# olasanni1/ETOL

Hardware: AMD Instinct MI355X
Metric: collocation-node constraint+Jacobian evals/sec, 6-state VGP N=1024 (higher is better)
Workload: dtype f64

## Files before the change

### etol_amd/_lib.py

```python
import ctypes as C
import os

import torch

_HERE = os.path.dirname(os.path.abspath(__file__))
LIB_PATH = os.path.join(_HERE, "lib", "libemi355x.so")

EMI_OK = 0
STATUS = {0: "EMI_OK", 1: "EMI_ERR_ARG", 2: "EMI_ERR_STATE", 3: "EMI_ERR_HIP",
          4: "EMI_ERR_NO_DEVICE", 5: "EMI_ERR_UNSUPPORTED", 6: "EMI_ERR_COMM"}

MODEL_POINTMASS2D, MODEL_QUADROTOR2D, MODEL_FIXEDWING12 = 0, 1, 2
MODEL_SOURCE = 100
PATH_ELLIPSE, PATH_DISC, PATH_TRACK = 0, 1, 2
PATH_REC = 8
EVAL_NODES, EVAL_DEFECT, EVAL_ALL, EVAL_NOJAC = 1, 2, 3, 4
EVAL_KEEP_INVARIANT = 8


class EmiError(RuntimeError):
    pass


class Layout(C.Structure):
# ... 41 lines not shown

class IpmRung(C.Structure):
    _fields_ = [("M", C.c_int), ("bd", IpmBounds), ("recs", _D), ("opt", IpmOptions), ("repair", C.c_int)]


class IpmRefine(C.Structure):
    _fields_ = [("ode_tol", C.c_double), ("first_check", C.c_int), ("ul", _D), ("uu", _D)]


class IpmRefineResult(C.Structure):
    _fields_ = [("rung", C.c_int), ("verdict", C.c_int), ("rungs_solved", C.c_int), ("err", C.c_double)]


class Start(C.Structure):
    _fields_ = [("kind", C.c_int), ("nsets", C.c_int), ("xa", _D), ("xb", _D), ("box", _D), ("bend", C.c_double), ("clearance", C.c_double),
                ("grid", C.c_int), ("repair", C.c_int)]


class IpmRestart(C.Structure):
    _fields_ = [("nstarts", C.c_int), ("starts", C.POINTER(Start)), ("patience", _I), ("retry_mask", C.c_int), ("flags", C.c_int)]


class IpmRestartResult(C.Structure):
    _fields_ = [("attempt", C.c_int), ("attempts", C.c_int), ("level", C.c_int), ("refine", IpmRefineResult)]


START_LINE, START_BEND, START_PLANNED = range(3)
RESTART_DROP_FAILED = 1
REFINE_MET, REFINE_NOT_MET, REFINE_FELL_BACK, REFINE_FAILED = range(4)
IPM_RULE_RESIDUAL = 1
IPM_CONVERGED, IPM_ACCEPTABLE, IPM_MAX_ITER, IPM_LINE_SEARCH, IPM_INFEASIBLE, IPM_FACTOR, IPM_NOT_FINITE = range(7)

_PT, _DU, _ST, _EL, _BD = (C.POINTER(t) for t in (IpmPoint, IpmDuals, IpmStep, IpmElim, IpmBounds))

SYMBOLS = {
    "emi_abi_version": (C.c_int, []),
    "emi_status_string": (C.c_char_p, [C.c_int]),
    "emi_device_count": (C.c_int, [_I]),
    "emi_lgl": (C.c_int, [C.c_int, _D, _D, _D]),
    "emi_model_dims": (C.c_int, [C.c_int, _I, _I, _I]),
    "emi_edge_ellipse": (C.c_int, [C.c_double] * 4 + [_D]),
    "emi_track_centres": (C.c_int, [C.c_int, _D, _D, _D, C.c_int, _D, _D, _D]),
    "emi_create": (C.c_int, [C.c_int, C.POINTER(_P)]),
    "emi_create_f32": (C.c_int, [C.c_int, C.POINTER(_P)]),
    "emi_destroy": (C.c_int, [_P]),
    "emi_last_error": (C.c_char_p, [_P]),
    "emi_set_stream": (C.c_int, [_P, _P]),
    "emi_get_stream": (C.c_int, [_P, C.POINTER(_P)]),
    "emi_synchronize": (C.c_int, [_P]),
    "emi_set_mesh": (C.c_int, [_P, C.c_int, _D, _D, _D, C.c_double, C.c_double]),
    "emi_set_model": (C.c_int, [_P, C.c_int, _D, C.c_int, C.c_int]),
    "emi_set_model_source": (C.c_int, [_P, C.c_char_p, C.c_char_p, C.c_int, C.c_int, C.c_int, _I, C.c_int, _D, C.c_int, C.c_int]),
    "emi_check_model_source": (C.c_int, [C.c_char_p, C.c_char_p, C.c_int, C.c_int, C.c_int, C.c_int, C.c_int, C.c_char_p, C.c_size_t]),
    "emi_kkt_factor": (C.c_int, [_P, _D, _D, C.POINTER(C.c_ubyte), C.c_double, C.POINTER(C.c_int)]),
    "emi_kkt_factor_dev": (C.c_int, [_P, _P, _P, _P, C.c_double, C.POINTER(C.c_int)]),
    "emi_kkt_blocks_rows": (C.c_int, [_P, C.c_int, _I, _I, _I]),
    "emi_kkt_blocks_dev": (C.c_int, [_P, _P, _P, _P, _P, _P, C.c_double, _P, _P, C.c_int, _P, _P, _P, _P, _P]),
    "emi_kkt_blocks_host": (C.c_int, [_P, _D, _D, _D, _D, C.POINTER(C.c_ubyte), C.c_double, _D, _D, C.c_int, _I, _I, _D, _D, _D]),
    "emi_kkt_solve": (C.c_int, [_P, _D, C.c_int]),
    "emi_kkt_solve_dev": (C.c_int, [_P, _P, C.c_int]),
    "emi_ipm_reduce_dev": (C.c_int, [_P, _PT, _DU, _P, _P, _P, _BD, _P, _P, _P, _EL, _P]),
    "emi_ipm_expand_dev": (C.c_int, [_P, _PT, _DU, _P, _BD, _P, _EL, _P, _ST, _P]),
    "emi_ipm_trial_dev": (C.c_int, [_P, _PT, _ST, _P, _PT]),
    "emi_ipm_merit_dev": (C.c_int, [_P, _PT, _P, _P, _BD, _P, _P, C.c_int, _P]),
    "emi_ipm_accept_dev": (C.c_int, [_P, _PT, _PT, _DU, _ST, _BD, _P, _P, _P, _P]),
    "emi_ipm_error_dev": (C.c_int, [_P, _PT, _DU, _P, _P, _BD, _P, _P]),
    "emi_ipm_reduce_host": (C.c_int, [_P, _PT, _DU, _P, _P, _P, _BD, _P, _P, _P, _EL, _P]),
    "emi_ipm_expand_host": (C.c_int, [_P, _PT, _DU, _P, _BD, _P, _EL, _P, _ST, _P]),
    "emi_ipm_trial_host": (C.c_int, [_P, _PT, _ST, _P, _PT]),
    "emi_ipm_merit_host": (C.c_int, [_P, _PT, _P, _P, _BD, _P, _P, C.c_int, _P]),
    "emi_ipm_accept_host": (C.c_int, [_P, _PT, _PT, _DU, _ST, _BD, _P, _P, _P, _P]),
    "emi_ipm_error_host": (C.c_int, [_P, _PT, _DU, _P, _P, _BD, _P, _P]),
    "emi_ipm_start_dev": (C.c_int, [_P, C.c_int, _PT, _DU, _P, _BD, _P, C.c_double, C.c_double, _P, _P]),
    "emi_ipm_error_parts_dev": (C.c_int, [_P, _PT, _DU, _P, _P, _BD, _P, _P]),
    "emi_ipm_error_parts_host": (C.c_int, [_P, _PT, _DU, _P, _P, _BD, _P, _P]),
    "emi_ipm_keep_dev": (C.c_int, [_P, _PT, _DU, _PT, _DU, _P, C.c_int]),
    "emi_ipm_keep_host": (C.c_int, [_P, _PT, _DU, _PT, _DU, _P, C.c_int]),
    "emi_ipm_solve_shard_dev": (C.c_int, [_P, _P, _P, _BD, C.POINTER(IpmOptions), _P, _P, C.POINTER(IpmResult)]),
    "emi_ipm_solve_shard_host": (C.c_int, [_P, _P, _P, _BD, C.POINTER(IpmOptions), _P, _P, C.POINTER(IpmResult)]),
    "emi_prolong_matrix": (C.c_int, [C.c_int, _D, _D, C.c_int, _D, _D]),
    "emi_prolong_dev": (C.c_int, [_P, C.c_int, C.c_int, _P, _P, C.c_int, _P]),
    "emi_repair_guess_dev": (C.c_int, [_P, _P]),
    "emi_ipm_solve_ladder_dev": (C.c_int, [_P, C.c_int, C.POINTER(IpmRung), C.c_double, C.c_double, _P, _P, _P, _P, _P, _P, C.POINTER(IpmResult)]),
    "emi_ipm_solve_ladder_host": (C.c_int, [_P, C.c_int, C.POINTER(IpmRung), C.c_double, C.c_double, _P, _P, _P, _P, _P, _P, C.POINTER(IpmResult)]),
    "emi_ode_error_operator": (C.c_int, [C.c_int, _D, _D, _D, _D, _D]),
    "emi_interp_dev": (C.c_int, [_P, C.c_int, C.c_int, C.c_int, _P, _P, C.c_int, C.c_int, _P]),
    "emi_ode_error_dev": (C.c_int, [_P, _P, _P, _D, _D, _P, _P]),
    "emi_ode_error_host": (C.c_int, [_P, _P, _P, _D, _D, _P, _P]),
    "emi_ode_error_delay_operator": (C.c_int, [C.c_int, _D, _D, C.c_double, C.c_double, C.c_double, _D]),
    "emi_ode_error_total_dev": (C.c_int, [_P, _P, _P, _D, _D, _P, _P]),
    "emi_ode_error_total_host": (C.c_int, [_P, _P, _P, _D, _D, _P, _P]),
    "emi_ipm_refine_decide": (C.c_int, [C.c_int, C.c_double, C.c_double, C.c_int, C.c_int, _I]),
    "emi_prolong_rows_dev": (C.c_int, [_P, C.c_int, C.c_int, _P, _P, C.c_int, _P, _P]),
    "emi_shard_move_dev": (C.c_int, [_P, C.c_int, _P, _P, C.c_int, _I, C.POINTER(_P), _I, C.POINTER(_P), _I, C.c_int]),
    "emi_ipm_solve_refine_dev": (C.c_int, [_P, C.c_int, C.POINTER(IpmRung), C.c_double, C.c_double, C.POINTER(IpmRefine), _P, _P, C.c_int,
                                           _P, _P, _P, _P, C.POINTER(IpmResult), _D, C.POINTER(IpmRefineResult)]),
    "emi_ipm_solve_refine_host": (C.c_int, [_P, C.c_int, C.POINTER(IpmRung), C.c_double, C.c_double, C.POINTER(IpmRefine), _P, _P, C.c_int,
                                            _P, _P, _P, _P, C.POINTER(IpmResult), _D, C.POINTER(IpmRefineResult)]),
    "emi_ipm_restart_decide": (C.c_int, [C.c_int, C.c_int]),
    "emi_ipm_solve_restart_dev": (C.c_int, [_P, C.c_int, C.POINTER(IpmRung), C.c_double, C.c_double, C.POINTER(IpmRefine), C.POINTER(IpmRestart),
                                            _P, _P, C.c_int, _P, _P, _P, _P, C.POINTER(IpmResult), _D, C.POINTER(IpmRestartResult)]),
    "emi_ipm_solve_restart_host": (C.c_int, [_P, C.c_int, C.POINTER(IpmRung), C.c_double, C.c_double, C.POINTER(IpmRefine), C.POINTER(IpmRestart),
                                             _P, _P, C.c_int, _P, _P, _P, _P, C.POINTER(IpmResult), _D, C.POINTER(IpmRestartResult)]),
    "emi_plan_route": (C.c_int, [C.c_int, _D, _D, _D, C.c_double, C.c_int, C.c_int, _D, _D, _D, _I, _D, _I, _I]),
    "emi_start_guess_dev": (C.c_int, [_P, C.POINTER(Start), _P, _P]),
    "emi_start_guess_host": (C.c_int, [_P, C.POINTER(Start), _P, _P]),
    "emi_kkt_last_regularisation": (C.c_int, [_P, _D, _D]),
    "emi_kkt_factor_batch": (C.c_int, [C.c_int, C.POINTER(_P), C.POINTER(_D), C.POINTER(_D), C.POINTER(C.POINTER(C.c_ubyte)), _D, _I]),
    "emi_kkt_solve_batch": (C.c_int, [C.c_int, C.POINTER(_P), C.POINTER(_D)]),
    "emi_kkt_is_schur": (C.c_int, [_P]),
    "emi_kkt_solve_refined": (C.c_int, [_P, _D, C.c_double, C.c_int, _D, _I, _I, _I]),
    "emi_kkt_solve_refined_batch": (C.c_int, [C.c_int, C.POINTER(_P), C.POINTER(_D), _D, C.c_int, _D, _I, _I, _I]),
    "emi_kkt_lowrank": (C.c_int, [_P, C.c_int, C.POINTER(C.c_int), _D, _D, C.POINTER(C.c_int)]),
    "emi_kkt_factor_shard_dev": (C.c_int, [_P, _P, _P, _P, _D, C.POINTER(C.c_ubyte), _I]),
    "emi_kkt_lowrank_shard_dev": (C.c_int, [_P, C.c_int, _P, _P, _P, _P, C.POINTER(C.c_ubyte), _I]),
    "emi_kkt_solve_shard_dev": (C.c_int, [_P, _P, C.POINTER(C.c_ubyte)]),
    "emi_kkt_solve_refined_shard_dev": (C.c_int, [_P, _P, C.POINTER(C.c_ubyte), _D, C.c_int, _D, _I, _I, _I]),
    "emi_set_batch": (C.c_int, [_P, C.c_int]),
    "emi_set_path": (C.c_int, [_P, C.c_int, C.c_int, _D, C.c_int, C.c_int]),
    "emi_set_tracks": (C.c_int, [_P, C.c_int, C.c_int, _D, _D]),
    "emi_set_track_waypoints": (C.c_int, [_P, C.c_int, C.c_int, C.c_int, _I, _D, _D, _D]),
    "emi_tracks_from_waypoints_dev": (C.c_int, [_P, C.c_int, _P]),
    "emi_get_tracks": (C.c_int, [_P, _D, _D]),
    "emi_get_layout": (C.c_int, [_P, C.POINTER(Layout)]),
    "emi_jac_structure": (C.c_int, [_P, _I, _I]),
    "emi_invariant_rows": (C.c_int, [C.c_int, C.c_int, C.POINTER(C.c_ubyte), _I]),
    "emi_dev_alloc": (C.c_int, [_P, C.c_size_t, C.POINTER(_P)]),
    "emi_dev_free": (C.c_int, [_P, _P]),
    "emi_h2d": (C.c_int, [_P, _P, _P, C.c_size_t]),
    "emi_d2h": (C.c_int, [_P, _P, _P, C.c_size_t]),
    "emi_eval_dev": (C.c_int, [_P, _P, _P, _P, _P, _P, C.c_uint]),
    "emi_eval_host": (C.c_int, [_P, _D, _D, _D, _D, _D, C.c_uint]),
    "emi_hess_dev": (C.c_int, [_P, _P, _P, _P, _P, C.c_double, _P]),
    "emi_hess_host": (C.c_int, [_P, _D, _D, _D, _D, C.c_double, _D]),
    "emi_lagr_grad_dev": (C.c_int, [_P, _P, _P, _P, C.c_double, _P]),
    "emi_lagr_grad_host": (C.c_int, [_P, _D, _D, _D, C.c_double, _D]),
    "emi_kkt_certificate_dev": (C.c_int, [_P, _P, _P, _P, _P, _P, _P, C.c_double, _P, _P, C.c_int, _D, _D, _P, _P]),
    "emi_kkt_certificate_host": (C.c_int, [_P, _D, _D, _D, _D, C.c_double, _D, _D, C.c_int, _D, _D, _D, _D]),
    "emi_lagr_grad_total_dev": (C.c_int, [_P, _P, _P, _P, C.c_double, _P, _P]),
    "emi_lagr_grad_total_host": (C.c_int, [_P, _D, _D, _D, C.c_double, _D, _D]),
    "emi_kkt_certificate_total_dev": (C.c_int, [_P, _P, _P, _P, _P, _P, _P, C.c_double, _P, _P, C.c_int, _D, _D, _P, _P, _P]),
    "emi_kkt_certificate_total_host": (C.c_int, [_P, _D, _D, _D, _D, C.c_double, _D, _D, C.c_int, _D, _D, _D, _D, _D]),
    "emi_timer_start": (C.c_int, [_P]),
    "emi_timer_stop": (C.c_int, [_P, C.POINTER(C.c_float)]),
    "emi_profile_enable": (C.c_int, [_P, C.c_int]),
    "emi_profile_read": (C.c_int, [_P, C.POINTER(C.c_float), _I, C.POINTER(C.c_float), _I, C.POINTER(C.c_float), _I]),
    "emi_set_option": (C.c_int, [_P, C.c_char_p, C.c_int]),
    "emi_last_path": (C.c_int, [_P, _I]),
    "emi_plan_pass": (C.c_int, [_P, C.c_int, C.POINTER(PassPlan)]),
    "emi_plan_pass_residency": (C.c_int, [_P, C.c_int, _I]),
    "emi_last_defect_kernel": (C.c_char_p, [_P]),
    "emi_debug_pass_roles": (C.c_int, [C.c_int, C.c_int, C.c_int, C.POINTER(C.c_int), C.c_int]),
    "emi_debug_tile_order": (C.c_int, [C.c_int, C.c_int, C.c_int, C.c_int, C.c_int, C.POINTER(C.c_int), C.c_int, C.POINTER(C.c_int), C.POINTER(C.c_int), C.POINTER(C.c_int)]),
    "emi_set_delays": (C.c_int, [_P, C.c_int, C.c_int, C.c_double]),
    "emi_get_delays": (C.c_int, [_P, _I, _I, _I]),
    "emi_delay_matrix": (C.c_int, [C.c_int, C.POINTER(C.c_double), C.POINTER(C.c_double), C.c_double, C.c_double, C.c_double, C.POINTER(C.c_double)]),
    "emi_debug_operator_fragments": (C.c_int, [C.c_int, C.POINTER(C.c_double), C.POINTER(C.c_double)]),
    "emi_debug_tile_order2": (C.c_int, [C.c_int] * 7 + [C.POINTER(C.c_int), C.c_int, C.POINTER(C.c_int), C.POINTER(C.c_int), C.POINTER(C.c_int)]),
    "emi_comm_unique_id": (C.c_int, [_P]),
    "emi_comm_create": (C.c_int, [C.c_int, C.c_int, C.c_int, _P, C.POINTER(_P)]),
    "emi_comm_gather": (C.c_int, [_P, _P, _P, C.c_size_t, C.c_int, _P]),
    "emi_comm_destroy": (C.c_int, [_P]),
    "emi_comm_last_error": (C.c_char_p, [_P]),
}

_lib = None


def load():
    global _lib
    if _lib is not None:
        return _lib
    if not os.path.exists(LIB_PATH):
        raise EmiError(f"{LIB_PATH} is missing: run `python -c 'import __graft_entry__ as g; g.build()'` "
                       "(or `make lib`) first; there is no CPU fallback")
    lib = C.CDLL(LIB_PATH, mode=C.RTLD_GLOBAL)
    for name, (res, args) in SYMBOLS.items():
        fn = getattr(lib, name)
        fn.restype = res
        fn.argtypes = args
    _lib = lib
    return lib


def check(status, ctx=None, what=""):
    if status == EMI_OK:
        return
    lib = load()
    msg = lib.emi_status_string(status).decode()
    if ctx:
        detail = lib.emi_last_error(ctx).decode()
        if detail:
            msg += ": " + detail
    raise EmiError(f"{what or 'libemi355x'}: {STATUS.get(status, status)} ({msg})")
```

### etol_amd/csrc/emi_api_pass.hip

```cpp
#include "emi_ctx.hpp"

using namespace emi_api;

namespace {

emi::PassPolicyIn policy_in(emi_ctx_t c) {
    emi::PassPolicyIn in;
    in.ns = c->ns;
    in.M = c->M;
    in.real_bytes = c->f32 ? 4 : 8;
    in.rows = nres_of(c) + nvals_of(c);
    if (c->model == EMI_MODEL_SOURCE) in.model_class = emi::rtc_has_symdefect(c->rtc) ? emi::PASS_MODEL_RTC : emi::PASS_MODEL_NONE;
    else in.model_class = emi::pass_model_supported(c->model) ? emi::PASS_MODEL_BUILTIN : emi::PASS_MODEL_NONE;
    in.rtc_sw_large = emi::rtc_pass_sw_large(c->rtc);
    in.f32 = c->f32;
    in.symmetric = c->symmetric;
    in.has_dfrag = c->has_dfrag;
    in.allow_fused = c->allow_fused;
    in.overlap_mode = c->overlap_mode;
    in.sym_ct = c->sym_ct;
    in.sym_ksplit = c->sym_ksplit;
    in.sym_cpart = c->sym_cpart;
    in.sym_gblk = c->sym_gblk;
    in.sym_cx = c->sym_cx;
// ... 53 lines not shown

void delay_matrix(const std::vector<double>& tau, const std::vector<double>& w, double t0, double tf, double delay, double* W) {
    const int M = (int)tau.size();
    std::vector<double> lam(M);
    for (int j = 0; j < M; ++j) lam[j] = ((j & 1) ? -1.0 : 1.0) * std::sqrt(w[j]);
    const double hh = (tf - t0) / 2.0;
    for (int k = 0; k < M; ++k) {
        double ts = t0 + hh * (tau[k] + 1.0) - delay;
        if (ts < t0) ts = t0;
        const double x = (ts - t0) / hh - 1.0;
        double* row = W + (size_t)k * M;
        int hit = -1;
        for (int j = 0; j < M; ++j)
            if (x == tau[j]) hit = j;
        if (ts <= t0) hit = 0;
        if (hit >= 0) {
            for (int j = 0; j < M; ++j) row[j] = j == hit ? 1.0 : 0.0;
            continue;
        }
        double den = 0.0;
        for (int j = 0; j < M; ++j) {
            row[j] = lam[j] / (x - tau[j]);
            den += row[j];
        }
        for (int j = 0; j < M; ++j) row[j] /= den;
    }
}

int extend_controls(emi_ctx_t c, const void* dX, const void* dU_free, const void** dU_ext) {
    if (c->f32) return fail(c, EMI_ERR_UNSUPPORTED, "delayed values: f64 contexts only");
    if (c->points_only) return fail(c, EMI_ERR_STATE, "delayed values need a collocation mesh (this context holds a points-only mesh)");
    const int M = c->M, ncf = c->nc - c->nch;
    HIP_TRY(c, hipSetDevice(c->device));
    if (!c->attr_set) {
        HIP_TRY(c, emi::defect_f64_set_attr());
        c->attr_set = true;
    }
    int st;
    if ((st = ensure_delay_matrices(c))) return st;
    const size_t row = (size_t)M * 8;
    if ((st = ensure(c, c->d_uext, (size_t)c->B * c->nc * row))) return st;
    HIP_TRY(c, hipMemsetAsync(c->d_uext.p, 0, (size_t)c->B * c->nc * row, c->stream));
    HIP_TRY(c, hipMemcpy2DAsync(c->d_uext.p, (size_t)c->nc * row, dU_free, (size_t)ncf * row, (size_t)ncf * row, c->B, hipMemcpyDeviceToDevice, c->stream));
    double* base = (double*)c->d_uext.p + (size_t)ncf * M;
    for (int i = 1; i < c->xh; ++i) {
        emi::DefectArgs a{(const double*)dX, (const double*)c->d_W.p + (size_t)(i - 1) * M * M, base + (size_t)(i - 1) * c->ns * M,
                          c->B * c->ns, M, c->ns, c->nc};
        HIP_TRY(c, emi::launch_defect_f64(a, c->stream));
    }
    base += (size_t)std::max(c->xh - 1, 0) * c->ns * M;
    for (int i = 1; i <= c->uh; ++i) {
        emi::DefectArgs a{(const double*)dU_free, (const double*)c->d_W.p + (size_t)(i - 1) * M * M, base + (size_t)(i - 1) * ncf * M,
                          c->B * ncf, M, ncf, c->nc};
        HIP_TRY(c, emi::launch_defect_f64(a, c->stream));
    }
    *dU_ext = c->d_uext.p;
    return EMI_OK;
}

enum class Form {
    PassF64,
    TwoKernelF64,
    PassF32,
    TwoStreamF32,
    Sequential,
};
struct FormChoice {
    Form form = Form::Sequential;
    bool small = false;
    emi::PassPlan plan;
    bool overlapped() const { return form == Form::PassF64 || form == Form::TwoKernelF64; }
};

FormChoice choose_form(emi_ctx_t c, Launch L, unsigned flags) {
    const bool nodes = flags & EMI_EVAL_NODES, defect = flags & EMI_EVAL_DEFECT, jac = !(flags & EMI_EVAL_NOJAC);
    FormChoice ch;
    const emi::PassPolicyIn in = policy_in(c);
    ch.small = defect && !c->f32 && L.B > 0 && L.B * c->ns <= in.small_rows && emi::defect_small_supported(L.B * c->ns) &&
               !(nodes && jac && emi::pass_takes_small_batches(in));
    if (nodes && defect && !ch.small && emi::pass_overlapped(in)) {
        ch.plan = emi::plan_pass(in, L.B, jac);
        ch.form = ch.plan.one_launch ? Form::PassF64 : Form::TwoKernelF64;
    } else if (c->f32 && nodes && defect && jac && !c->rtc && c->allow_fused) {
        if ((c->overlap_mode == 3 || (c->overlap_mode == 0 && c->f32_one_launch)) && emi::pass_f32_supported(c->model, L.B * c->ns, c->M, L.B))
            ch.form = Form::PassF32;
        else if (c->overlap_mode == 2 && emi::defect_f32_mfma_supported(c->M))
            ch.form = Form::TwoStreamF32;
    }
    return ch;
}

int next_prof_record(emi_ctx_t c, ProfEvents** out) {
    if (c->prof_used == c->prof.size()) c->prof.emplace_back();
    ProfEvents& pe = c->prof[c->prof_used];
    for (hipEvent_t& e : pe.ev)
        if (!e) HIP_TRY(c, hipEventCreate(&e));
    ++c->prof_used;
    *out = &pe;
    return EMI_OK;
}

constexpr unsigned AT1 = 1u << 1, AT2 = 1u << 2, AT3 = 1u << 3, AT_ANY = AT1 | AT2 | AT3;
int prof_mark(emi_ctx_t c, ProfEvents* pe, ProfMark which, unsigned levels, hipStream_t s) {
    if (pe && pe->level > 0 && ((levels >> pe->level) & 1u)) HIP_TRY(c, hipEventRecord(pe->ev[which], s));
    return EMI_OK;
}

const char* const NAME_PASS_F32 = "emi_pass_f32_kernel (MFMA + node roles, one launch)";
const char* const NAME_RING1_F64 = "emi_symdefect_ring_f64_kernel";
const char* name_defect_f32(emi_ctx_t c, bool mfma) {
    return !mfma ? "emi_defect_f32_kernel" : (c->f32_ring ? "emi_defect_f32_ring_kernel" : "emi_defect_f32_mfma_kernel");
}
const char* name_defect_f64(bool small) { return small ? "emi_defect_small_f64_kernel" : "emi_defect_f64_kernel"; }
std::string name_pass_f64(const emi::SymPlan& plan) {
    return "emi_pass_f64_kernel<SW=" + std::to_string(plan.sw) + "> (MFMA + node roles, one launch" +
           (plan.ks > 1 ? ", " + std::to_string(plan.ks) + " K slices per tile" : "") + ")" +
           (plan.bk == 16 ? " [K tiles of 16]" : "") + (plan.ct == 2 ? " [128-column tiles]" : "") + (plan.hs == 2 ? " [K range in two halves per workgroup]" : "") +
           (plan.dop ? " [De/Do from L2]" : "");
}
std::string name_symdefect(emi_ctx_t c, const emi::SymPlan& plan, bool in_kernel_combine) {
    if (plan.ring1) return c->sym_ct == 1 || c->sym_ct == 2 ? "emi_symdefect_f64_kernel" : NAME_RING1_F64;
    return "emi_symdefect_ring2_f64_kernel<SW=" + std::to_string(plan.sw) + ">" +
           (plan.ks > 1 ? " x" + std::to_string(plan.ks) + (in_kernel_combine ? " K slices (in-kernel combine)" : " K slices + emi_symdefect_combine_kernel") : "");
}

emi::SymDefectArgs sym_defect_args(emi_ctx_t c, Launch L, const PassIO& io) {
    emi::SymDefectArgs sa;
    sa.X = (const double*)io.X;
    sa.U = (const double*)io.U;
    sa.RES = (double*)io.RES;
    sa.node_t = (const double*)c->d_t.p;
    sa.De = (const double*)c->d_De.p;
    sa.Do = (const double*)c->d_Do.p;
    sa.Dfrag = c->has_dfrag ? (const double*)c->d_Dfrag.p : nullptr;
    sa.M = c->M;
    sa.B = L.B;
    sa.nres = nres_of(c);
    sa.h = (c->tf - c->t0) / 2.0;
    sa.order = c->sym_order;
    sa.ablate = c->sym_ablate;
    sa.ksplit = 1;
    sa.slab = nullptr;
    sa.tile_ticket = nullptr;
    sa.cpart = sa.cx = 0;
    sa.mfma_first = 0;
    for (int i = 0; i < EMI_MAX_PARAMS; ++i) sa.P.p[i] = c->params[i];
    return sa;
}

emi::DefectArgsF32 defect_args_f32(emi_ctx_t c, Launch L, const PassIO& io) {
    return emi::DefectArgsF32{(const float*)io.X, (const float*)c->d_D.p, (float*)io.RES, L.B * c->ns, c->M, c->ns, nres_of(c)};
}

int form_pass_f64(emi_ctx_t c, Launch L, const PassIO& io, const emi::PassPlan& pp, ProfEvents* pe) {
    const emi::SymPlan& plan = pp.sym;
    emi::SymDefectArgs sa = sym_defect_args(c, L, io);
    emi::NodeArgs<double> na;
    fill_node_args(c, L, na, io);
    sa.mfma_first = pp.mfma_first;
    sa.cpart = plan.cpart;
    sa.cx = plan.cx;
    if (plan.ks > 1) {
        EMI_TRY(ensure(c, c->d_slab, plan.slab_bytes));
        EMI_TRY(ensure_zeroed(c, c->d_tile_ticket, (size_t)plan.tiles * 4, c->stream));
        sa.ksplit = plan.ks;
        sa.slab = (double*)c->d_slab.p;
        sa.tile_ticket = (unsigned*)c->d_tile_ticket.p;
    }
    EMI_TRY(ensure_zeroed(c, c->d_ticket, (size_t)L.B * 4, c->stream));
    na.cost_ticket = (unsigned*)c->d_ticket.p;
    EMI_TRY(prof_mark(c, pe, K0, AT_ANY, c->stream));
    if (c->rtc) HIP_TRY(c, emi::rtc_launch_pass(c->rtc, sa, na, plan.sw, c->stream));
    else HIP_TRY(c, emi::launch_pass(c->model, sa, na, c->stream, plan));
    EMI_TRY(prof_mark(c, pe, K1, AT_ANY, c->stream));
    if (pe) pe->level = -1;
    c->last_defect_kernel = name_pass_f64(plan);
    return EMI_OK;
}

int launch_symdefect_f64(emi_ctx_t c, Launch L, emi::SymDefectArgs& sa, hipStream_t s) {
    if (c->rtc) {
        HIP_TRY(c, emi::rtc_launch_symdefect(c->rtc, sa, s));
        c->last_defect_kernel = NAME_RING1_F64;
        return EMI_OK;
    }
    const emi::SymPlan plan = emi::plan_symdefect(c->ns, L.B, c->M, c->sym_ct, c->sym_ksplit, c->sym_cpart, c->sym_gblk, c->sym_cx);
    if (plan.slab_bytes) EMI_TRY(ensure(c, c->d_slab, plan.slab_bytes));
    sa.ksplit = plan.ring1 ? 1 : plan.ks;
    sa.slab = (double*)c->d_slab.p;
    sa.cpart = plan.cpart;
    sa.cx = plan.cx;
    if (sa.ksplit > 1 && c->sym_combine) {
        EMI_TRY(ensure_zeroed(c, c->d_tile_ticket, (size_t)plan.tiles * 4, s));
        sa.tile_ticket = (unsigned*)c->d_tile_ticket.p;
    }
    const unsigned bit = 1u << c->sym_ct;
    HIP_TRY(c, emi::launch_symdefect(c->model, sa, s, !(c->fused_attr_mask & bit), c->sym_ct, plan));
    c->fused_attr_mask |= bit;
    c->last_defect_kernel = name_symdefect(c, plan, sa.tile_ticket != nullptr);
    return EMI_OK;
}

int form_two_kernel_f64(emi_ctx_t c, Launch L, const PassIO& io, bool jac, ProfEvents* pe) {
    emi::SymDefectArgs sa = sym_defect_args(c, L, io);
    emi::NodeArgs<double> na;
    fill_node_args(c, L, na, io);
    const bool two = c->overlap_mode != 1;
    const bool split = two && c->cu_split > 0;
    if (two && !split) EMI_TRY(need_stream2(c));
    hipStream_t s1 = split ? c->s_mfma : c->stream;
    hipStream_t s2 = split ? c->s_node : (two ? c->stream2 : c->stream);
    if (two) {
        HIP_TRY(c, hipEventRecord(c->ev_fork, c->stream));
        HIP_TRY(c, hipStreamWaitEvent(s2, c->ev_fork, 0));
        if (split) HIP_TRY(c, hipStreamWaitEvent(s1, c->ev_fork, 0));
    }
    EMI_TRY(prof_mark(c, pe, K0, AT1 | AT2, s1));
    EMI_TRY(launch_symdefect_f64(c, L, sa, s1));
    EMI_TRY(prof_mark(c, pe, K1, AT1 | AT2, s1));
    if (c->cost_in_kernel) {
        EMI_TRY(ensure_zeroed(c, c->d_ticket, (size_t)L.B * 4, s2));
        na.cost_ticket = (unsigned*)c->d_ticket.p;
    }
    EMI_TRY(prof_mark(c, pe, K2, AT1 | AT3, s2));
    if (c->rtc && jac && na.store_mode == 2 && c->M % 2 == 0) HIP_TRY(c, emi::rtc_launch_nodes_nt(c->rtc, na, s2));
    else if (c->rtc) HIP_TRY(c, emi::rtc_launch_nodes<double>(c->rtc, na, jac, false, s2));
    else HIP_TRY(c, emi::launch_nodes<double>(c->model, na, jac, false, s2));
    EMI_TRY(prof_mark(c, pe, K3, AT1 | AT3, s2));
    if (!c->cost_in_kernel) HIP_TRY(c, emi::launch_cost_finish<double>(na.cost_part, na.cost, L.B, emi::node_chunks(c->M), na.sgn * na.h, s2));
    if (two) {
        HIP_TRY(c, hipEventRecord(c->ev_join, s2));
        HIP_TRY(c, hipStreamWaitEvent(c->stream, c->ev_join, 0));
        if (split) {
            HIP_TRY(c, hipEventRecord(c->ev_join2, s1));
            HIP_TRY(c, hipStreamWaitEvent(c->stream, c->ev_join2, 0));
        }
    }
    EMI_TRY(prof_mark(c, pe, E1, AT1, c->stream));
    EMI_TRY(prof_mark(c, pe, E2, AT1, c->stream));
    return EMI_OK;
}

int form_pass_f32(emi_ctx_t c, Launch L, const PassIO& io, ProfEvents* pe) {
    emi::NodeArgs<float> na;
    fill_node_args(c, L, na, io);
    const size_t rowb = (size_t)c->M * 4;
    HIP_TRY(c, hipMemset2DAsync(io.RES, (size_t)nres_of(c) * rowb, 0, (size_t)c->ns * rowb, L.B, c->stream));
    EMI_TRY(ensure_zeroed(c, c->d_ticket, (size_t)L.B * 4, c->stream));
    na.cost_ticket = (unsigned*)c->d_ticket.p;
    EMI_TRY(prof_mark(c, pe, K0, AT_ANY, c->stream));
    HIP_TRY(c, emi::launch_pass_f32(c->model, defect_args_f32(c, L, io), na, c->pass_order >= 0 ? c->pass_order : 0, c->stream));
    EMI_TRY(prof_mark(c, pe, K1, AT_ANY, c->stream));
    if (pe) { pe->level = -1; pe->fused = true; }
    c->last_defect_kernel = NAME_PASS_F32;
    return EMI_OK;
}

int form_two_stream_f32(emi_ctx_t c, Launch L, const PassIO& io, ProfEvents* pe) {
    emi::NodeArgs<float> pre, full;
    PassIO values_only = io;
    values_only.VALS = nullptr;
    fill_node_args(c, L, pre, values_only);
    fill_node_args(c, L, full, io);
    EMI_TRY(ensure(c, c->d_cost_part2, (size_t)L.B * emi::node_chunks(c->M) * 4));
    EMI_TRY(need_stream2(c));
    pre.cost_part = (float*)c->d_cost_part2.p;
    pre.np = 0;
    const bool fork_late = c->f32_ring_wgs == 1;
    if (!fork_late) {
        HIP_TRY(c, hipEventRecord(c->ev_fork, c->stream));
        HIP_TRY(c, hipStreamWaitEvent(c->stream2, c->ev_fork, 0));
    }
    HIP_TRY(c, emi::launch_nodes<float>(c->model, pre, false, true, c->stream));
    if (fork_late) {
        HIP_TRY(c, hipEventRecord(c->ev_fork, c->stream));
        HIP_TRY(c, hipStreamWaitEvent(c->stream2, c->ev_fork, 0));
    }
    EMI_TRY(prof_mark(c, pe, K0, AT1 | AT2, c->stream));
    HIP_TRY(c, emi::launch_defect_f32_mfma(defect_args_f32(c, L, io), c->stream, c->f32_ring, c->f32_ring_wgs));
    EMI_TRY(prof_mark(c, pe, K1, AT1 | AT2, c->stream));
    c->last_defect_kernel = name_defect_f32(c, true);
    EMI_TRY(prof_mark(c, pe, K2, AT1 | AT3, c->stream2));
    HIP_TRY(c, emi::launch_nodes<float>(c->model, full, true, false, c->stream2));
    EMI_TRY(prof_mark(c, pe, K3, AT1 | AT3, c->stream2));
    HIP_TRY(c, emi::launch_cost_finish<float>(full.cost_part, full.cost, L.B, emi::node_chunks(c->M), full.sgn * full.h, c->stream2));
    HIP_TRY(c, hipEventRecord(c->ev_join, c->stream2));
    HIP_TRY(c, hipStreamWaitEvent(c->stream, c->ev_join, 0));
    if (pe) pe->fused = true;
    EMI_TRY(prof_mark(c, pe, E1, AT1, c->stream));
    EMI_TRY(prof_mark(c, pe, E2, AT1, c->stream));
    return EMI_OK;
}

template <typename T>
int launch_nodes_alone(emi_ctx_t c, Launch L, const PassIO& io, bool jac) {
    emi::NodeArgs<T> a;
    fill_node_args(c, L, a, io);
    if (c->rtc) HIP_TRY(c, emi::rtc_launch_nodes<T>(c->rtc, a, jac, true, c->stream));
    else HIP_TRY(c, emi::launch_nodes<T>(c->model, a, jac, true, c->stream));
    HIP_TRY(c, emi::launch_cost_finish<T>(a.cost_part, a.cost, L.B, emi::node_chunks(c->M), a.sgn * a.h, c->stream));
    return EMI_OK;
}

int form_sequential(emi_ctx_t c, Launch L, const PassIO& io, unsigned flags, bool small, ProfEvents* pe) {
    const bool jac = !(flags & EMI_EVAL_NOJAC);
    if (flags & EMI_EVAL_NODES) EMI_TRY(c->f32 ? launch_nodes_alone<float>(c, L, io, jac) : launch_nodes_alone<double>(c, L, io, jac));
    EMI_TRY(prof_mark(c, pe, E1, AT_ANY, c->stream));
    if ((flags & EMI_EVAL_DEFECT) && c->f32) {
        const bool mfma = emi::defect_f32_mfma_supported(c->M) && c->allow_fused;
        if (mfma) HIP_TRY(c, emi::launch_defect_f32_mfma(defect_args_f32(c, L, io), c->stream, c->f32_ring, c->f32_ring_wgs));
        else HIP_TRY(c, emi::launch_defect_f32(defect_args_f32(c, L, io), c->stream));
        c->last_defect_kernel = name_defect_f32(c, mfma);
    } else if (flags & EMI_EVAL_DEFECT) {
        emi::DefectArgs a{(const double*)io.X, (const double*)c->d_D.p, (double*)io.RES, L.B * c->ns, c->M, c->ns, nres_of(c)};
        if (small) HIP_TRY(c, emi::launch_defect_small_f64(a, c->stream));
        else HIP_TRY(c, emi::launch_defect_f64(a, c->stream));
        c->last_defect_kernel = name_defect_f64(small);
    }
    EMI_TRY(prof_mark(c, pe, E2, AT1 | AT2, c->stream));
    return EMI_OK;
}

int eval_launch(emi_ctx_t c, Launch L, const PassIO& io, unsigned flags) {
    const bool nodes = flags & EMI_EVAL_NODES, defect = flags & EMI_EVAL_DEFECT;
    const bool jac = !(flags & EMI_EVAL_NOJAC);
    if (!nodes && !defect) return fail(c, EMI_ERR_ARG, "emi_eval: empty flags");
// ... 32 lines not shown
    const int M = c->M, nd = std::max(c->xh - 1, c->uh);
    std::vector<double> W((size_t)nd * M * M);
    for (int d = 0; d < nd; ++d) delay_matrix(c->h_tau, c->h_w, c->t0, c->tf, (d + 1) * c->delay_dt, W.data() + (size_t)d * M * M);
    EMI_TRY(upload_real(c, c->d_W, W.data(), W.size()));
    c->delay_dirty = false;
    return EMI_OK;
}

int emi_api::need_stream2(emi_ctx_t c) {
    if (c->stream2) return EMI_OK;
    if (hipStreamCreateWithFlags(&c->stream2, hipStreamNonBlocking) != hipSuccess) {
        c->stream2 = nullptr;
        return fail(c, EMI_ERR_HIP, "cannot create the second stream of the two-stream pass");
    }
    return EMI_OK;
}

extern "C" {

int emi_delay_matrix(int M, const double* tau, const double* w, double t0, double tf, double delay, double* W) {
    if (M < 2 || !tau || !w || !W || !(tf > t0) || delay < 0) return EMI_ERR_ARG;
    delay_matrix(std::vector<double>(tau, tau + M), std::vector<double>(w, w + M), t0, tf, delay, W);
    return EMI_OK;
}

int emi_eval_dev(emi_ctx_t c, const void* dX, const void* dU, void* dRES, void* dVALS, void* dCOST,
                 unsigned flags) {
    int st = ready(c);
    if (st) return st;
    if (c->nch > 0 && dX && dU && (st = extend_controls(c, dX, dU, &dU))) return st;
    int piece = 0;
    const emi::PassPolicyIn in = policy_in(c);
    if (!c->profile && (flags & EMI_EVAL_ALL) == EMI_EVAL_ALL && emi::pass_overlapped(in) && dX && dU && dRES && dCOST &&
        (dVALS || (flags & EMI_EVAL_NOJAC)))
        piece = emi::plan_piece(in, c->B);
    const PassIO io{dX, dU, dRES, dVALS, dCOST};
    const emi::KeepRecord::Pass kp = c->keep.begin_pass((flags & EMI_EVAL_NODES) && !(flags & EMI_EVAL_NOJAC),
                                                        flags & EMI_EVAL_KEEP_INVARIANT, dVALS);
    flags &= ~(unsigned)EMI_EVAL_KEEP_INVARIANT;
    if (piece <= 0) st = eval_launch(c, Launch{0, c->B, kp.keep}, io, flags);
    for (int first = 0; piece > 0 && first < c->B && st == EMI_OK; first += piece)
        st = eval_launch(c, Launch{first, std::min(piece, c->B - first), kp.keep}, io_at(c, io, first), flags);
    c->keep.end_pass(kp, dVALS, st == EMI_OK);
    return st;
}

int emi_eval_host(emi_ctx_t c, const double* X, const double* U, double* RES, double* VALS,
                  double* COST, unsigned flags) {
    int st = ready(c);
    if (st) return st;
    if (!X || !U) return fail(c, EMI_ERR_ARG, "emi_eval_host: null input");
    const size_t rb = c->f32 ? 4 : 8;
    const size_t nX = (size_t)c->B * c->ns * c->M, nU = (size_t)c->B * (c->nc - c->nch) * c->M;
    const size_t nR = (size_t)c->B * nres_of(c) * c->M, nV = (size_t)c->B * nvals_of(c) * c->M;
    if ((st = upload_real(c, c->s_X, X, nX))) return st;
    if ((st = upload_real(c, c->s_U, U, nU))) return st;
    if ((st = ensure(c, c->s_RES, nR * rb))) return st;
    if ((st = ensure_vals_staging(c, nV * rb))) return st;
    if ((st = ensure(c, c->s_COST, (size_t)c->B * rb))) return st;
    if (!(flags & EMI_EVAL_NODES)) {
        if (!RES) return fail(c, EMI_ERR_ARG, "emi_eval_host: defect-only needs RES in/out");
        if ((st = upload_real(c, c->s_RES, RES, nR))) return st;
    }
    if ((st = emi_eval_dev(c, c->s_X.p, c->s_U.p, c->s_RES.p, c->s_VALS.p, c->s_COST.p, flags | EMI_EVAL_KEEP_INVARIANT))) return st;
    if ((st = download_real(c, RES, c->s_RES.p, nR))) return st;
    if (!(flags & EMI_EVAL_NOJAC) && (flags & EMI_EVAL_NODES))
        if ((st = download_real(c, VALS, c->s_VALS.p, nV))) return st;
    if (flags & EMI_EVAL_NODES)
        if ((st = download_real(c, COST, c->s_COST.p, c->B))) return st;
    HIP_TRY(c, hipStreamSynchronize(c->stream));
    return EMI_OK;
}

int emi_hess_dev(emi_ctx_t c, const void* dX, const void* dU, const void* dLamF, const void* dLamC,
                 double sigma, void* dH) {
    int st = ready(c);
    if (st) return st;
    if (!dX || !dU || !dLamF || !dH || (np_total(c) > 0 && !dLamC))
        return fail(c, EMI_ERR_ARG, "emi_hess: null device pointer");
    HIP_TRY(c, hipSetDevice(c->device));
    if (c->nch > 0 && (st = extend_controls(c, dX, dU, &dU))) return st;
    auto fill = [&](auto& a) {
        using T = typename std::remove_reference<decltype(a.h)>::type;
        a.X = (const T*)dX; a.U = (const T*)dU; a.lamF = (const T*)dLamF; a.lamC = (const T*)dLamC;
        a.H = (T*)dH; a.w = (const T*)c->d_w.p; a.node_t = (const T*)c->d_t.p;
        a.path = (const T*)c->d_path.p;
        a.M = c->M; a.B = c->B; a.np = np_total(c); a.path_sets = c->path_sets; a.px = c->px; a.py = c->py;
        a.h = (T)((c->tf - c->t0) / 2.0); a.sgn = c->maximize ? T(-1) : T(1); a.sigma = (T)sigma;
        for (int i = 0; i < EMI_MAX_PARAMS; ++i) a.P.p[i] = (T)c->params[i];
    };
    if (c->f32) {
        emi::HessArgs<float> a;
        fill(a);
        if (c->rtc) HIP_TRY(c, emi::rtc_launch_hess<float>(c->rtc, a, c->stream));
        else HIP_TRY(c, emi::launch_hess<float>(c->model, a, c->stream));
    } else {
        emi::HessArgs<double> a;
        fill(a);
        if (c->rtc) HIP_TRY(c, emi::rtc_launch_hess<double>(c->rtc, a, c->stream));
        else HIP_TRY(c, emi::launch_hess<double>(c->model, a, c->stream));
    }
    return EMI_OK;
}

int emi_hess_host(emi_ctx_t c, const double* X, const double* U, const double* LamF,
                  const double* LamC, double sigma, double* H) {
    int st = ready(c);
    if (st) return st;
    if (!X || !U || !LamF || !H || (np_total(c) > 0 && !LamC)) return fail(c, EMI_ERR_ARG, "emi_hess_host: null pointer");
    const size_t rb = c->f32 ? 4 : 8;
    const size_t nX = (size_t)c->B * c->ns * c->M, nU = (size_t)c->B * (c->nc - c->nch) * c->M;
    const size_t nC = (size_t)c->B * np_total(c) * c->M, nH = (size_t)c->B * nhess_of(c) * c->M;
    if ((st = upload_real(c, c->s_X, X, nX))) return st;
    if ((st = upload_real(c, c->s_U, U, nU))) return st;
    if ((st = upload_real(c, c->s_LF, LamF, nX))) return st;
    if (nC && (st = upload_real(c, c->s_LC, LamC, nC))) return st;
    if ((st = ensure(c, c->s_H, nH * rb))) return st;
    if ((st = emi_hess_dev(c, c->s_X.p, c->s_U.p, c->s_LF.p, c->s_LC.p, sigma, c->s_H.p))) return st;
    return download_real(c, H, c->s_H.p, nH);
}

int emi_plan_pass(emi_ctx_t c, int B, emi_pass_plan_t* out) {
    if (!c || !out || B < 1) return EMI_ERR_ARG;
    if (c->M <= 0 || c->model < 0) return fail(c, EMI_ERR_STATE, "emi_plan_pass: mesh and model must be set");
    memset(out, 0, sizeof *out);
    emi::report_pass(policy_in(c), B, out);
    return EMI_OK;
}

int emi_plan_pass_residency(emi_ctx_t c, int B, int* res) {
    if (!c || !res || B < 1) return EMI_ERR_ARG;
    if (c->M <= 0 || c->model < 0) return fail(c, EMI_ERR_STATE, "emi_plan_pass_residency: mesh and model must be set");
    emi_pass_plan_t plan;
    memset(&plan, 0, sizeof plan);
    emi::report_pass(policy_in(c), B, &plan, nullptr, res);
    return EMI_OK;
}

int emi_last_path(emi_ctx_t c, int* fused) {
    if (!c || !fused) return EMI_ERR_ARG;
    *fused = choose_form(c, Launch{0, c->B}, EMI_EVAL_ALL).overlapped() ? 1 : 0;
    return EMI_OK;
}

int emi_debug_pass_roles(int nm, int nn, int order, int* out_role, int out_cap) {
    if (nm < 0 || nn < 0 || nm + nn < 1 || !out_role || out_cap < nm + nn) return EMI_ERR_ARG;
    for (int j = 0; j < nm + nn; ++j) {
        const emi::PassRole r = emi::pass_role_of(j, nm, nn, order);
        out_role[j] = r.mfma ? r.index : -1 - r.index;
    }
    return EMI_OK;
}

int emi_debug_tile_order(int ns, int B, int M, int sym_ct, int sym_cpart, int* out_tile, int out_cap, int* ntiles_total, int* cpart,
                         int* cx) {
    return emi_debug_tile_order2(ns, B, M, sym_ct, sym_cpart, 0, 0, out_tile, out_cap, ntiles_total, cpart, cx);
}

int emi_debug_tile_order2(int ns, int B, int M, int sym_ct, int sym_cpart, int sym_gblk, int sym_cx, int* out_tile, int out_cap,
                          int* ntiles_total, int* cpart, int* cx) {
    if (ns < 1 || B < 1 || M < 128 || M % 128 != 0 || !ntiles_total) return EMI_ERR_ARG;
    const emi::SymPlan p = emi::plan_symdefect(ns, B, M, sym_ct, 1, sym_cpart, sym_gblk, sym_cx);
    if (p.ring1 || p.sw < 1) return EMI_ERR_UNSUPPORTED;
    const int ntiles = (M / 2) / 64, ngrp = ((B + 15) / 16) * (ns / p.sw), total = ntiles * ngrp;
    *ntiles_total = total;
    if (cpart) *cpart = p.cpart;
    if (cx) *cx = p.cx;
    for (int t = 0; t < total && t < out_cap && out_tile; ++t) {
        const emi::RingTile rt = emi::ring_tile_of(t, ntiles, ngrp, p.cpart, p.cx, ns / p.sw);
        out_tile[t] = rt.ntile + ntiles * rt.grp;
    }
    return EMI_OK;
}

int emi_debug_operator_fragments(int M, const double* D, double* out) {
    if (M < 128 || M % 128 != 0 || !D || !out) return EMI_ERR_ARG;
    std::vector<double> De, Do;
    if (!even_odd_halves(M, D, De, Do)) return EMI_ERR_UNSUPPORTED;
    emi::operator_fragments(M, De.data(), Do.data(), out);
    return EMI_OK;
}

const char* emi_last_defect_kernel(emi_ctx_t c) {
    if (!c) return "";
    return c->last_defect_kernel.c_str();
}

}
```

### etol_amd/csrc/emi_args.hpp

```cpp
#pragma once
#ifdef __HIPCC_RTC__
#define EMI_PATH_ELLIPSE 0
#define EMI_PATH_DISC 1
#define EMI_PATH_TRACK 2
#define EMI_PATH_REC 8
#else
#include <hip/hip_runtime.h>
#include <stddef.h>
#include "emi355x.h"
#endif

#define EMI_NODE_THREADS 256

#ifdef EMI_TICKET_ACQ_REL
#define EMI_TICKET_ORDER __ATOMIC_ACQ_REL
#else
#define EMI_TICKET_ORDER __ATOMIC_RELAXED
#endif
#ifdef EMI_NO_M0_NOP
#define EMI_M0_NOP ""
#else
#define EMI_M0_NOP "s_nop 0\n\t"
#endif

#define DEF_TM 96
#define DEF_TN 128
#define DEF_BK 16

#define FUSED_TI 16
#define FUSED_BK 16

#include "emi_models.hpp"

namespace emi {

template <typename T> struct NodeArgs {
    const T* X;
    const T* U;
    T* RES;
    T* VALS;
    T* cost_part;
    T* cost;
    unsigned* cost_ticket;
    const T* w;
    const T* node_t;
    const T* Ddiag;
    const T* path;
    const T* track_x;
    const T* track_y;
    int M, B, np, nres, nvals;
    int path_sets, track_sets, ntracks;
    int px, py;
    int store_mode;
    int keep;
    T h, sgn;
    ModelParams<T> P;
};

template <typename T> struct HessArgs {
    const T* X;
    const T* U;
    const T* lamF;
    const T* lamC;
    T* H;
    const T* w;
    const T* node_t;
    const T* path;
    int M, B, np, path_sets, px, py;
    T h, sgn, sigma;
    ModelParams<T> P;
};

template <typename T> struct OdeResidArgs {
    const T* Zs;
    const T* Zc;
    const T* tq;
    const T* scale;
    const T* ul;
    const T* uu;
    T* eta;
    int M, B, lds, ldc;
    T h;
    ModelParams<T> P;
};

template <typename T> struct OdeResidDelayArgs {
    const T* Zs;
    const T* Zc;
    const T* tq;
    const T* scale;
    const T* ul;
    const T* uu;
    T* eta;
    int M, B, lds, ldc;
    int ncf, ns, xh, uh;
    T h;
    ModelParams<T> P;
};

struct SymDefectArgs {
    const double* X;
    const double* U;
    double* RES;
    const double* node_t;
    const double* De;
    const double* Do;
    int M, B, nres;
    int order;
    int ablate;
    int ksplit;
    double* slab;
    unsigned* tile_ticket;
    int mfma_first;
    int cpart, cx;
    double h;
    ModelParams<double> P;
    const double* Dfrag;
};

struct DefectArgs {
    const double* X;
    const double* D;
    double* RES;
    int R, M, ns, nres;
};
struct DefectArgsF32 {
    const float* X;
    const float* D;
    float* RES;
    int R, M, ns, nres;
};
struct RingTile { int ntile, grp; };
#if defined(__HIPCC__)
__host__ __device__
#endif
inline RingTile ring_tile_of(int tl, int ntiles, int ngrp, int cpart, int cx, int nsg = 1) {
    RingTile t;
    if (cpart > 0) {
        const int per_xcd = ngrp * ntiles / 8;
        const int x = tl / per_xcd, m = tl - x * per_xcd;
        const int pc = x % cpart, pg = x / cpart;
        const int ncol = ntiles / cpart, ng = ngrp / (8 / cpart);
        const int cb = m / (ng * cx), r = m - cb * ng * cx;
        t.grp = pg * ng + r / cx;
        t.ntile = pc * ncol + cb * cx + r % cx;
    } else if (cpart < 0) {
        const int G = -cpart, per_xcd = ngrp * ntiles / 8;
        const int x = tl / per_xcd, m = tl - x * per_xcd;
        const int per_sb = G * nsg * ntiles, sb = m / per_sb, r = m - sb * per_sb;
        const int per_cb = G * nsg * cx, cb = r / per_cb, r2 = r - cb * per_cb;
        const int g = r2 / (nsg * cx), r3 = r2 - g * (nsg * cx);
        const int mt = x * (ngrp / nsg / 8) + sb * G + g;
        t.grp = mt * nsg + r3 / cx;
        t.ntile = cb * cx + r3 % cx;
    } else {
        t.ntile = tl % ntiles;
        t.grp = tl / ntiles;
    }
    return t;
}
struct PassRole { int mfma, index; };
#if defined(__HIPCC__)
__host__ __device__
#endif
inline PassRole pass_role_of(int j, int nm, int nn, int order) {
    const long long t = (long long)nm + nn;
    long long m0, m1;
    const long long d = order >= 100 ? order : 100;
    if (order == 1 || d * nm > 100 * t) {
        m0 = j < nm ? j : nm;
        m1 = j < nm ? j + 1 : nm;
    } else {
        m0 = ((long long)j * nm * d) / (100 * t);
        m1 = ((long long)(j + 1) * nm * d) / (100 * t);
        if (m0 > nm) m0 = nm;
        if (m1 > nm) m1 = nm;
    }
    PassRole r;
    r.mfma = m1 > m0;
    r.index = (int)(r.mfma ? m0 : j - m0);
    return r;
}
struct PassArgs {
    SymDefectArgs s;
    NodeArgs<double> n;
    int nm8, nn8;
    int nm, nn;
    int nbx;
};

}
```

### etol_amd/csrc/emi_ctx.hpp

```cpp
#pragma once
#include <hip/hip_runtime.h>

#include <algorithm>
#include <cstdarg>
#include <cstdio>
#include <cstring>
#include <string>
#include <vector>

#include "emi355x.h"
#include "emi_device_array.hpp"
#include "emi_keep_record.hpp"
#include "emi_kernels.hpp"

namespace emi_api {

using DevBuf = emi::DeviceArray<unsigned char>;

enum ProfMark { E0, E1, E2, K0, K1, K2, K3, PROF_MARKS };
struct ProfEvents {
    hipEvent_t ev[PROF_MARKS] = {};
    bool has_node = false, has_defect = false, fused = false;
    int level = 0;
};

}
using emi_api::DevBuf, emi_api::ProfEvents;

struct emi_ctx_s {
    int device = 0;
    bool f32 = false;
    hipStream_t stream = nullptr;
    bool own_stream = false;
    hipStream_t stream2 = nullptr;
    hipEvent_t ev_fork = nullptr, ev_join = nullptr, ev_join2 = nullptr;
    int cu_split = 0;
    hipStream_t s_mfma = nullptr, s_node = nullptr;
    std::string err;
    std::string last_defect_kernel;

    int M = 0;
    double t0 = 0, tf = 0;
    DevBuf d_w, d_t, d_Ddiag, d_D, d_De, d_Do;
    bool symmetric = false;
    DevBuf d_Dfrag;
    bool has_dfrag = false;
    bool points_only = false;
    int allow_fused = 1;
    int sym_ct = 0;
    int sym_order = 1;
    int sym_ablate = 0;
    int small_rows = 24;
    int overlap_mode = 0;
    int node_store = -1;
    unsigned fused_attr_mask = 0;
    std::vector<double> h_tau, h_w;
    int model = -1, ns = 0, nc = 0, maximize = 0;
    double params[EMI_MAX_PARAMS] = {0};
    emi::KktWorkspace* kkt = nullptr;
    std::vector<emi::KktWorkspace*> kkt_shard;
    int kkt_method = 1;
    emi::RtcModel* rtc = nullptr;
    int B = 0;
    int np = 0, path_sets = 0, px = 0, py = 1;
    int np_model = 0;
    std::vector<int> pvars;
    DevBuf d_path;
    int ntracks = 0, track_sets = 0;
    DevBuf d_trkx, d_trky;
    int wp_ntracks = 0, wp_sets = 0, wp_ld = 0;
    emi::DeviceArray<double> d_wp;
    emi::DeviceArray<int> d_wp_cnt;
    emi::DeviceArray<double> d_wp_nt;
    bool wp_nt_dirty = true;
    DevBuf d_cost_part;
    DevBuf d_slab;
    DevBuf d_tile_ticket;
    DevBuf d_cost_part2;
    DevBuf d_ticket;
    int cost_in_kernel = 1;
    int sym_nst = 3;
    int sym_hs = 0;
    int sym_ctc = 0;
    int sym_bk = 0;
    int sym_dop = 0;
    int sym_res = 0;
    int xh = 0, uh = 0, nch = 0;
    double delay_dt = 0.0;
    bool delay_dirty = true;
    DevBuf d_W;
    bool adjw_dirty = true;
    DevBuf d_adjWT;
    DevBuf d_adj_Gx;
    int adj_fold_tile = 0;
    DevBuf d_uext;
    int f32_ring_wgs = 2;
    int f32_ring = 1;
    int f32_one_launch = 0;
    int slice = 0;
    int sym_ksplit = 0;
    int sym_cpart = 0;
    int sym_gblk = 0, sym_cx = 0;
    int pass_order = -1;
    int sym_combine = 1;
    emi::KeepRecord keep;
    DevBuf s_X, s_U, s_RES, s_VALS, s_COST, s_LF, s_LC, s_H;
    std::vector<DevBuf> host_stage;
    DevBuf d_adjDT;
    bool adj_dirty = true;
    DevBuf d_adj_pvars;
    std::vector<int> adj_pvars;
    DevBuf d_adj_c;
    DevBuf d_adj_G;
    DevBuf d_adj_op;
    DevBuf s_G, s_cert, s_zl, s_zu, s_Gdel;
    bool ode_dirty = true;
    emi::DeviceArray<double> d_ode_op;
    emi::DeviceArray<double> d_ode_tq;
    emi::DeviceArray<double> d_ode_ub;
    emi::DeviceArray<double> d_ode_ws;
    bool odel_dirty = true;
    emi::DeviceArray<double> d_odel_ops;
    emi::DeviceArray<double> d_odel_opc;
    bool blk_rows_set = false;
    std::vector<int> blk_row_ptr, blk_var, blk_entry;
    std::vector<int> blk_key;
    emi::DeviceArray<int> blk_term_ptr, blk_term_row, blk_term_ea, blk_term_eb, blk_flag, blk_list, blk_nflag, blk_cnt;
    emi::DeviceArray<double> blk_tdelta, blk_tvec, blk_tworst;
    int blk_generic = 0;
    std::vector<int> ipm_key;
    emi::DeviceArray<int> ipm_lists;
    int ipm_npairs = 0;
    std::vector<double> ipm_crow_h;
    emi::DeviceArray<double> ipm_crow, ipm_part;
    emi::IpmSolveWs* ipm_solve = nullptr;
    emi::IpmLadderWs* ipm_ladder = nullptr;
    emi::StartGuessWs* start_guess = nullptr;
    bool path_has_track = false;
    hipEvent_t t_start = nullptr, t_stop = nullptr;
    int profile = 0;
    std::vector<ProfEvents> prof;
    size_t prof_used = 0;
    bool attr_set = false;

    ~emi_ctx_s() {
        (void)hipSetDevice(device);
        if (stream) (void)hipStreamSynchronize(stream);
        for (ProfEvents& pe : prof)
            for (hipEvent_t e : pe.ev)
                if (e) (void)hipEventDestroy(e);
        for (hipStream_t s : {stream2, s_mfma, s_node})
            if (s) { (void)hipStreamSynchronize(s); (void)hipStreamDestroy(s); }
        for (hipEvent_t e : {ev_join2, ev_fork, ev_join, t_start, t_stop})
            if (e) (void)hipEventDestroy(e);
        if (own_stream && stream) (void)hipStreamDestroy(stream);
        emi::rtc_destroy(rtc);
        emi::kkt_destroy(kkt);
        for (emi::KktWorkspace* w : kkt_shard) emi::kkt_destroy(w);
        emi::ipm_solve_destroy(ipm_solve);
        emi::ipm_ladder_destroy(ipm_ladder);
        emi::start_guess_destroy(start_guess);
    }
};

#define HIP_TRY(c, call)                                                                                                                  \
    do {                                                                                                                                  \
        hipError_t e_ = (call);                                                                                                           \
        if (e_ != hipSuccess) return emi_api::fail((c), EMI_ERR_HIP, "%s failed: %s (%s:%d)", #call, hipGetErrorString(e_), __FILE__, __LINE__); \
    } while (0)
#define HIP_TRY_AS(c, who, call)                                                                                        \
    do {                                                                                                                \
        const hipError_t e_ = (call);                                                                                   \
        if (e_ != hipSuccess) return emi_api::fail((c), EMI_ERR_HIP, "%s: %s failed: %s", who, #call, hipGetErrorString(e_)); \
    } while (0)

#define EMI_TRY(call)              \
    do {                           \
        const int st_ = (call);    \
        if (st_) return st_;       \
    } while (0)

namespace emi_api {

int fail(emi_ctx_t c, int code, const char* fmt, ...);
inline int ensure(emi_ctx_t c, DevBuf& b, size_t bytes) {
    HIP_TRY(c, b.reserve(bytes));
    return EMI_OK;
}
inline int ensure_zeroed(emi_ctx_t c, DevBuf& b, size_t bytes, hipStream_t s) {
    if (b.bytes() >= bytes) return EMI_OK;
    EMI_TRY(ensure(c, b, bytes));
    HIP_TRY(c, hipMemsetAsync(b.p, 0, bytes, s));
    return EMI_OK;
}
int upload_bytes(emi_ctx_t c, DevBuf& b, const void* src, size_t bytes);
int upload_real(emi_ctx_t c, DevBuf& b, const double* src, size_t n);
int download_real(emi_ctx_t c, double* dst, const void* dsrc, size_t n);
bool even_odd_halves(int M, const double* D, std::vector<double>& De, std::vector<double>& Do);
int ensure_vals_staging(emi_ctx_t c, size_t bytes);

inline int np_total(emi_ctx_t c) { return c->np + c->np_model; }
inline int nvals_of(emi_ctx_t c) { return c->ns * (c->ns + c->nc) + 2 * c->np + c->np_model * (int)c->pvars.size() + (c->ns + c->nc); }
inline int nres_of(emi_ctx_t c) { return c->ns + np_total(c); }
inline int nhess_of(emi_ctx_t c) { const int nv = c->ns + c->nc; return nv * (nv + 1) / 2; }
inline int ready(emi_ctx_t c) {
    if (!c) return EMI_ERR_ARG;
    if (c->M <= 0) return fail(c, EMI_ERR_STATE, "emi_set_mesh has not been called");
    if (c->model < 0) return fail(c, EMI_ERR_STATE, "emi_set_model has not been called");
    if (c->B <= 0) return fail(c, EMI_ERR_STATE, "emi_set_batch has not been called");
    if (c->np > 0 && c->path_sets != 1 && c->path_sets != c->B)
        return fail(c, EMI_ERR_STATE, "path table has %d sets, batch is %d", c->path_sets, c->B);
    if (c->ntracks > 0 && c->track_sets != 1 && c->track_sets != c->B)
        return fail(c, EMI_ERR_STATE, "track table has %d sets, batch is %d", c->track_sets, c->B);
    return EMI_OK;
}

struct HostStager {
    emi_ctx_t c;
    size_t slot = 0;
    int status = EMI_OK;
    struct Out { void* host; void* dev; size_t bytes; };
    std::vector<Out> outs;
    explicit HostStager(emi_ctx_t c_) : c(c_) {}
    void* place(const void* host, size_t bytes, bool in, bool out);
    int finish();
};
#define HOST_STAGED_TRY(s, call)                                                          \
    if ((s).status) { (void)hipStreamSynchronize((s).c->stream); return (s).status; }     \
    if (const int st_ = (call)) { (void)hipStreamSynchronize((s).c->stream); return st_; }

int ensure_delay_matrices(emi_ctx_t c);
int need_stream2(emi_ctx_t c);
int path_row_list(emi_ctx_t c, const char* what, std::vector<int>& ptr, std::vector<int>& var, std::vector<int>& ent);
int shard_check(emi_ctx_t c, const char* what);
int ctx_ipm_launch(emi_ctx_t c, int what, const emi_ipm_bounds_t* bd, const void* dPar, emi::IpmArgs& a);

}
```

### etol_amd/csrc/emi_kernels.hpp

```cpp
#pragma once
#include <hip/hip_runtime.h>
#include <stddef.h>

#include <string>

#include "emi355x.h"
#include "emi_args.hpp"
#include "emi_pass_plan.hpp"

static_assert(EMI_PATH_ELLIPSE == 0 && EMI_PATH_DISC == 1 && EMI_PATH_TRACK == 2 && EMI_PATH_REC == 8,
              "emi_args.hpp and emi355x.h disagree");

namespace emi {

static_assert(PASS_TI == FUSED_TI, "emi_pass_plan.hpp and emi_args.hpp disagree");

int node_chunks(int M);
bool invariant_rows(int model, int np, unsigned char* mask);
template <typename T>
hipError_t launch_nodes(int model, const NodeArgs<T>& a, bool jac, bool defect_rows, hipStream_t s);
template <typename T> hipError_t launch_hess(int model, const HessArgs<T>& a, hipStream_t s);
hipError_t launch_defect_f64(const DefectArgs& a, hipStream_t s);
bool defect_small_supported(int R);
hipError_t launch_defect_small_f64(const DefectArgs& a, hipStream_t s);
hipError_t launch_defect_f32(const DefectArgsF32& a, hipStream_t s);
bool defect_f32_mfma_supported(int M);
hipError_t launch_defect_f32_mfma(const DefectArgsF32& a, hipStream_t s, int ring = 0, int wgs_per_cu = 2);
bool pass_f32_supported(int model, int R, int M, int B);
hipError_t launch_pass_f32(int model, const DefectArgsF32& d, const NodeArgs<float>& n, int order, hipStream_t s);
hipError_t defect_f64_set_attr();
template <typename T>
hipError_t launch_cost_finish(const T* part, T* cost, int B, int nchunks, T scale, hipStream_t s);
bool fused_supported(int model, int M, int ct);
hipError_t launch_symdefect(int model, const SymDefectArgs& a, hipStream_t s, bool set_attr, int ct, const SymPlan& plan);
inline void operator_fragments(int M, const double* De, const double* Do, double* out) {
    const int Hh = M / 2, nkt = Hh / 16;
    for (int ct = 0; ct < Hh / 64; ++ct)
        for (int w = 0; w < 4; ++w)
            for (int kt = 0; kt < nkt; ++kt)
                for (int q = 0; q < 4; ++q)
                    for (int lane = 0; lane < 64; ++lane) {
                        const double* row = ((q & 1) ? Do : De) + (size_t)(64 * ct + 16 * w + (lane & 15)) * Hh + 16 * kt + 8 * (q >> 1) + 2 * (lane >> 4);
                        double* o = out + ((((size_t)(ct * 4 + w) * nkt + kt) * 4 + q) * 64 + lane) * 2;
                        o[0] = row[0];
                        o[1] = row[1];
                    }
}

bool pass_model_supported(int model);
hipError_t launch_pass(int model, const SymDefectArgs& sa, const NodeArgs<double>& na, hipStream_t s, const SymPlan& plan);

struct AdjointArgs {
    const double* VALS;
    const double* lamF;
    const double* lamC;
    const double* DT;
    const int* pvars;
    double* G;
    int B, M, ldt, ns, nc, np_table, np_traced, pw, px, py, nvals;
    int add_op;
    double sigma;
};
struct CertArgs {
    const double *X, *U, *RES, *VALS, *lamF, *lamC, *G;
    const double *zl, *zu;
    const double *cl, *cu;
    double* cert;
    int B, M, ns, nc, np, nres, nvals, nsets;
    int ncg;
    double sigma;
};
struct AdjointOpArgs {
    const double* A;
    const double* Bop;
    const double* add;
    double* out;
    int R, rpi, M, ldt, nseg, ldb;
    int a_inst, a_row0, a_seg, out_inst, out_row0, add_inst, add_row0;
};
hipError_t launch_adjoint_transpose(const double* dSrc, double* dDst, int M, int ldt, int ld_dst, int nseg, bool keep_diag, hipStream_t s);
bool adjoint_side_by_side(int B, int ns, int M);
hipError_t launch_adjoint_op(const AdjointArgs& a, hipStream_t s);
hipError_t launch_adjoint_product(const AdjointOpArgs& a, int tile, hipStream_t s);
hipError_t launch_adjoint_nodes(const AdjointArgs& a, hipStream_t s);
hipError_t launch_adjoint_add(const double* dGop, double* dG, int B, int ns, int nv, int M, hipStream_t s);
hipError_t launch_kkt_certificate(const CertArgs& a, hipStream_t s);

struct InterpOpArgs {
    const double* V;
    const double* OP;
    double* out;
    int R, K, N, ldk, ldo;
};
hipError_t launch_interp_op(const InterpOpArgs& a, hipStream_t s);
hipError_t launch_ode_copy_D(const double* D, double* dst, int M, int ldk, hipStream_t s);
hipError_t launch_ode_resid(int model, const OdeResidArgs<double>& a, hipStream_t s);
struct RtcModel;
hipError_t rtc_launch_ode_resid(RtcModel* m, const OdeResidArgs<double>& a, hipStream_t s);
hipError_t launch_ode_resid_delay(int model, const OdeResidDelayArgs<double>& a, hipStream_t s);
hipError_t rtc_launch_ode_resid_delay(RtcModel* m, const OdeResidDelayArgs<double>& a, hipStream_t s);
struct OdeFinishArgs {
    const double* X;
    const double* Zs;
    const double* eta;
    double* err;
    int B, M, ns, lds, dcol;
    double h;
};
hipError_t launch_ode_finish(const OdeFinishArgs& a, hipStream_t s);

struct BlocksArgs {
    const double *H, *VALS, *Sigma, *SigT;
    const unsigned char* fixed;
    double dw_shift;
    double *Qexact, *Q;
    int max_mods;
    int* count;
    int* node;
    double *delta, *vec, *worst;
    int B, M, nv, np, nvals;
    int generic;
    const int *term_ptr, *term_row, *term_ea, *term_eb;
    int *flag, *list, *nflag, *cnt;
    double *tdelta, *tvec, *tworst;
};
hipError_t launch_kkt_blocks(const BlocksArgs& a, hipStream_t s);

struct IpmArgs {
    int B, M, ns, nc, np, nvals, nsets, reset;
    double *X, *U, *S, *E1, *E2;
    double *tX, *tU, *tS, *tE1, *tE2;
    double *LF, *Y, *ZL, *ZU, *VL, *VU, *W1, *W2;
    double *DZ, *DS, *DY, *DE1, *DE2, *DZL, *DZU, *DVL, *DVU, *DW1, *DW2;
    double *Sigma, *SigT, *SigS, *RhatS, *Rt, *Rhs;
    const double *RES, *VALS, *G, *COST, *DefRes, *RowRes, *rs;
    const double *zl, *zu;
    const double* crow;
    const double *par, *apr, *adu;
    const unsigned char* mask;
    const int *vptr, *vrow, *vent;
    const int *rptr, *rvar, *rent;
    double *part, *out;
    unsigned char* fixedb;
    double* LamC;
    double push, frac;
};
enum { IPM_REDUCE, IPM_EXPAND, IPM_TRIAL, IPM_MERIT, IPM_ACCEPT, IPM_ERROR, IPM_ERROR_PARTS, IPM_START_PUSH, IPM_START_ROWS, IPM_RESET_W, IPM_LAMC };
constexpr int IPM_MAX_PARTIALS = 9;
int ipm_chunks(int M);
hipError_t launch_ipm(int what, const IpmArgs& a, hipStream_t s);

struct RtcModel;
int rtc_check(bool f32, const char* struct_name, const char* source, int ns, int nc, int npath, int pw, std::string* log);
int rtc_build(bool f32, const char* struct_name, const char* source, int ns, int nc, int npath, int pw, RtcModel** out, std::string* log);
void rtc_destroy(RtcModel* m);
bool rtc_has_symdefect(const RtcModel* m);
template <typename T>
hipError_t rtc_launch_nodes(RtcModel* m, const NodeArgs<T>& a, bool jac, bool defect_rows, hipStream_t s);
template <typename T> hipError_t rtc_launch_hess(RtcModel* m, const HessArgs<T>& a, hipStream_t s);
hipError_t rtc_launch_symdefect(RtcModel* m, const SymDefectArgs& a, hipStream_t s);
int rtc_pass_sw_large(const RtcModel* m);
hipError_t rtc_launch_pass(RtcModel* m, const SymDefectArgs& sa, const NodeArgs<double>& na, int sw, hipStream_t s);
hipError_t rtc_launch_nodes_nt(RtcModel* m, const NodeArgs<double>& a, hipStream_t s);

struct KktWorkspace;
int kkt_factor(KktWorkspace** w, hipStream_t stream, const double* dD, int M, int ns, int nv, const double* Qblk,
               const double* Jblk, const unsigned char* fixed, double dc, int method, int* info, std::string* err,
               bool blocks_on_device = false);
int kkt_solve(KktWorkspace* w, hipStream_t stream, int nz, double* rhs, int nrhs, std::string* err,
              bool rhs_on_device = false);
bool kkt_set_option(const char* name, int value);
int kkt_lowrank(KktWorkspace* w, hipStream_t stream, int nz, int r, const int* node, const double* vec, const double* delta,
                int* exact, std::string* err);
void kkt_destroy(KktWorkspace* w);
void kkt_last_regularisation(const KktWorkspace* w, double* dc, double* dw);
void kkt_mesh_changed(KktWorkspace* w);
bool kkt_is_schur(const KktWorkspace* w);
struct KktShardSrc {
    const double* Q;
    const double* VALS;
    const unsigned char* fixed;
    size_t vals_stride;
    const int* inst;
};
int kkt_factor_batch(int n, KktWorkspace** const* pws, hipStream_t stream, const double* const* dD, int M, int ns, int nv,
                     const double* const* Qblk, const double* const* Jblk, const unsigned char* const* fixed, const double* dc, int* info,
                     std::string* err, const KktShardSrc* src = nullptr);
int kkt_solve_batch(int n, KktWorkspace* const* ws, hipStream_t stream, int nz, double* const* rhs, std::string* err,
                    bool rhs_on_device = false);
int kkt_solve_refined_batch(int n, KktWorkspace* const* ws, hipStream_t stream, double* const* rhs, const double* dc_nominal, int max_steps,
                            double* rel, int* nsolve, int* reverted, int* status, std::string* err, bool rhs_on_device = false);
int kkt_holds(const KktWorkspace* w, int M, int ns, int nv);
int kkt_lowrank_shard(int n, KktWorkspace* const* ws, hipStream_t stream, int max_mods, const int* inst, const int* count, const int* dNode,
                      const double* dDelta, const double* dVec, int* exact, std::string* err);
void kkt_forget_ladder(KktWorkspace* w);

struct IpmSolveWs;
void ipm_solve_destroy(IpmSolveWs* w);
int ipm_solve_shard(emi_ctx_t c, void* dX, void* dU, const emi_ipm_bounds_t* bd, const emi_ipm_options_t& opt, void* dLamF, void* dLamC,
                    emi_ipm_result_t* results);

struct IpmKeepArgs {
    double* live[13];
    double* kept[13];
    const unsigned char* mask;
    int B, M, ns, nc, np, restore;
};
hipError_t launch_ipm_keep(const IpmKeepArgs& a, hipStream_t s);

hipError_t launch_prolong_rows(const double* PT, const double* Vc, const int* map, int group, double* Vf, int Mc, int Mf, int R, hipStream_t s);
struct RepairArgs {
    double* X;
    const double *recs, *trkx, *trky;
    int B, ns, M, np, path_sets, px, py, ntracks, track_sets;
};
hipError_t launch_repair_guess(const RepairArgs& a, hipStream_t s);
struct TrackWaypointArgs {
    const double *t, *x, *y, *node_t;
    const int *cnt, *map;
    void *xc, *yc;
    int n, ntracks, ld, M, first;
};
template <typename T> hipError_t launch_track_waypoints(TrackWaypointArgs a, hipStream_t s);
struct IpmLadderWs;
void ipm_ladder_destroy(IpmLadderWs* w);
struct StartArgs {
    double* X;
    int* level;
    const double *recs, *par, *tau, *sine;
    double *cost, *dist, *extra;
    int* cells;
    unsigned char* bits;
    int B, ns, M, np, path_sets, px, py, nsets, kind, N, has_box;
    double bend, clearance;
};
struct StartGuessWs;
void start_guess_destroy(StartGuessWs* w);
int start_guess(emi_ctx_t c, const emi_start_t& st, void* dX, void* dLevel);
int ipm_solve_ladder(emi_ctx_t c, int nrungs, const emi_ipm_rung_t* rungs, double t0, double tf, const void* dX0, const void* dU0, void* dX,
                     void* dU, void* dLamF, void* dLamC, emi_ipm_result_t* results);
constexpr int SHARD_MOVE_ARRAYS = 4;
struct ShardMoveArgs {
    const double* src[SHARD_MOVE_ARRAYS];
    double* dst[SHARD_MOVE_ARRAYS];
    int rows[SHARD_MOVE_ARRAYS], sld[SHARD_MOVE_ARRAYS], dld[SHARD_MOVE_ARRAYS];
    const int *sidx, *didx;
    int n, narrays, len, first;
};
hipError_t launch_shard_move(ShardMoveArgs a, hipStream_t s);
int ipm_solve_refine(emi_ctx_t c, int nrungs, const emi_ipm_rung_t* rungs, double t0, double tf, const emi_ipm_refine_t& rf, const void* dX0,
                     const void* dU0, int ldm, void* dX, void* dU, void* dLamF, void* dLamC, emi_ipm_result_t* results, double* err,
                     emi_ipm_refine_result_t* out);
int ipm_solve_restart(emi_ctx_t c, int nrungs, const emi_ipm_rung_t* rungs, double t0, double tf, const emi_ipm_refine_t* rf,
                      const emi_ipm_restart_t& rs, const void* dX0, const void* dU0, int ldm, void* dX, void* dU, void* dLamF, void* dLamC,
                      emi_ipm_result_t* results, double* err, emi_ipm_restart_result_t* out);

}
```

### etol_amd/csrc/emi_pass_plan.hpp

```cpp
#pragma once
#include <stddef.h>

#include <algorithm>
#include <climits>

#include "emi355x.h"

namespace emi {

constexpr int PASS_TI = 16;

struct SymPlan {
    bool ring1 = false;
    int sw = 0;
    int ks = 1;
    int nst = 3;
    int bk = 8;
    int hs = 1;
    int ct = 1;
    bool dop = false;
    int res = 2;
    size_t slab_bytes = 0;
    int cpart = 0, cx = 0;
    int tiles = 0;
};

inline bool symdefect_shape_ok(int M, int ct) {
    if (ct == 0 || (ct >= 4 && ct <= 8)) return M >= 128 && M % 128 == 0;
    const int w = ct == 2 ? 2 : 1;
    return ct >= 1 && ct <= 3 && M >= 128 * w && M % (128 * w) == 0;
}

inline int legal_ks(int nkt, int ks) {
    while (ks > 1 && (nkt % ks != 0 || nkt / ks < 2 || (nkt / ks) % 2 != 0)) ks >>= 1;
    return ks < 1 ? 1 : ks;
}

inline int symdefect_sw(int ns, int tiles, int ct) {
    if (ct == 0 || ct == 4) {
        if (tiles >= 448) return (ns % 2 == 0 && ns > 2) ? 2 : ns;
        if (tiles >= 320) return ns;
        if (tiles >= 192) return 0;
        return (tiles <= 96 || ns % 2 != 0 || ns <= 2) ? 1 : 2;
    }
    if (ct < 5 || ct > 8) return 0;
    const int sw = ct == 5 ? ns : (ct == 6 ? 2 : (ct == 8 ? 3 : 1));
    return ns % sw != 0 ? 1 : sw;
}
inline int symdefect_ct_of(int ns, int sw) { return sw == ns ? 5 : (sw == 2 ? 6 : (sw == 3 ? 8 : 7)); }

inline SymPlan plan_symdefect(int ns, int B, int M, int ct, int ksplit_opt, int cpart_opt = 0, int gblk_opt = 0, int cx_opt = 0, int bk_opt = 8,
                              int ct_cols = 1) {
    SymPlan p;
    p.bk = bk_opt == 16 ? 16 : 8;
    const int mtiles = (B + PASS_TI - 1) / PASS_TI;
    const int tiles = mtiles * ((M / 2) / 64);
    p.sw = symdefect_sw(ns, tiles, ct);
    if (p.sw == 0) {
        p.ring1 = true;
        return p;
    }
    if (ksplit_opt > 0) p.ks = legal_ks((M / 2) / p.bk, ksplit_opt);
    p.ct = (ct_cols == 2 && p.sw == 2 && p.ks == 1 && M % 256 == 0) ? 2 : 1;
    p.tiles = (tiles / p.ct) * (ns / p.sw);
    {
        const int ntiles = (M / 2) / (64 * p.ct), ngrp = mtiles * (ns / p.sw);
        const int target_cols = std::max(1, 4096 / M / p.ct);
        auto valid = [&](int cp) { return cp >= 1 && cp <= 8 && ntiles % cp == 0 && ngrp % (8 / cp) == 0 && (ngrp * ntiles) % 8 == 0; };
        int cp = 0;
        if (cpart_opt > 0) cp = valid(cpart_opt) ? cpart_opt : 0;
        else if (cpart_opt == 0 && tiles >= 192)
            for (int c = 1; c <= 8 && !cp; c *= 2)
                if (valid(c) && (ntiles / c <= target_cols || c == 8 || !valid(2 * c))) cp = c;
        if (gblk_opt > 0 && mtiles % (8 * gblk_opt) == 0 && (ngrp * ntiles) % 8 == 0) {
            int cxg = cx_opt > 0 ? cx_opt : 2;
            while (cxg > 1 && ntiles % cxg != 0) --cxg;
            p.cpart = -gblk_opt;
            p.cx = cxg;
        } else if (cp > 0) {
            p.cpart = cp;
            p.cx = 1;
            for (int d = 1; d <= std::min(ntiles / cp, target_cols); ++d)
                if ((ntiles / cp) % d == 0) p.cx = d;
            if (cp == 1 && p.cx == ntiles) p.cpart = p.cx = 0;
        }
    }
    if (p.ks > 1) p.slab_bytes = (size_t)p.tiles * p.ks * (2 * p.sw * 4) * 256 * sizeof(double);
    return p;
}

enum PassSwClass { SWC_NS = 0, SWC_1 = 1, SWC_2 = 2, SWC_3 = 3, SWC_LARGE = 4  };
constexpr bool pass_class_applies(int cls, int ns) {
    return cls == SWC_2 ? (ns > 2 && ns % 2 == 0) : (cls == SWC_3 ? (ns > 3 && ns % 3 == 0) : true);
}
constexpr int pass_class_sw(int cls, int ns) { return cls == SWC_NS ? ns : (cls == SWC_LARGE ? ((ns % 2 == 0 && ns > 2) ? 2 : 1) : cls); }

#define EMI_PASS_FORMS(X)                   \
    X(SWC_NS, 3, 8, 1, 1, false, true, -1)  \
    X(SWC_2, 3, 8, 1, 2, false, false, -1)  \
    X(SWC_2, 3, 16, 1, 2, false, false, -1) \
    X(SWC_2, 3, 8, 2, 1, false, false, -1)  \
    X(SWC_2, 3, 16, 2, 1, false, false, -1) \
    X(SWC_2, 3, 16, 1, 1, true, false, -1)  \
    X(SWC_2, 3, 16, 1, 1, false, false, -1) \
    X(SWC_2, 4, 8, 1, 1, false, true, -1)   \
    X(SWC_2, 3, 8, 1, 1, false, true, -1)   \
    X(SWC_3, 3, 8, 1, 1, false, true, -1)   \
    X(SWC_1, 3, 8, 1, 2, false, false, -1)  \
    X(SWC_1, 3, 16, 1, 2, false, false, -1) \
    X(SWC_1, 3, 16, 1, 1, true, false, -1)  \
    X(SWC_1, 3, 16, 1, 1, false, false, -1) \
    X(SWC_1, 4, 8, 1, 1, false, true, -1)   \
    X(SWC_1, 3, 8, 1, 1, false, true, -1)
#define EMI_PASS_FORMS_RTC(X)             \
    X(SWC_1, 3, 8, 1, 1, false, true, 0)  \
    X(SWC_LARGE, 3, 8, 1, 1, false, true, 2)

struct PassForm {
    int cls, nst, bk, ct, hs;
    bool dop, slices;
    int stores;
};
#define EMI_PASS_FORM_ROW(CLS, NST, BK, CT, HS, DOP, SLICES, STORES) {CLS, NST, BK, CT, HS, DOP, SLICES, STORES},
inline constexpr PassForm PASS_FORMS[] = {EMI_PASS_FORMS(EMI_PASS_FORM_ROW)};
inline constexpr PassForm PASS_FORMS_RTC[] = {EMI_PASS_FORMS_RTC(EMI_PASS_FORM_ROW)};
#undef EMI_PASS_FORM_ROW
constexpr int N_PASS_FORMS = sizeof PASS_FORMS / sizeof PASS_FORMS[0], N_PASS_FORMS_RTC = sizeof PASS_FORMS_RTC / sizeof PASS_FORMS_RTC[0];

enum PassModelClass { PASS_MODEL_NONE = 0, PASS_MODEL_BUILTIN = 1, PASS_MODEL_RTC = 2 };
struct PassShape {
    int ns = 0, M = 0;
    int model_class = PASS_MODEL_NONE;
    bool has_dfrag = false;
    int store_mode = 0;
};
struct PassWants {
    int sw = 0, ks = 1, nst = 3, bk = 8, ct = 1, hs = 1;
    bool dop = false;
    int res = 2;
};
constexpr int pass_form_max_res(const PassForm& f) { return f.dop ? 3 : 2; }
struct PassResolved {
    const PassForm* row = nullptr;
    int sw = 0, ks = 1;
    int res = 2;
    explicit operator bool() const { return row != nullptr; }
};

inline bool form_fits(const PassForm& f, const PassShape& s) {
    if (f.ct == 2 && s.M % 256 != 0) return false;
    if (f.hs == 2 && ((s.M / 2) / f.bk) % 4 != 0) return false;
    if (f.dop && !s.has_dfrag) return false;
    if (f.stores >= 0 && (f.stores == 2) != (s.store_mode == 2)) return false;
    return true;
}

inline const PassForm* find_form(const PassShape& s, int sw, bool sliced, int nst, int bk, int ct, int hs, bool dop) {
    const bool rtc = s.model_class == PASS_MODEL_RTC;
    const PassForm* rows = rtc ? PASS_FORMS_RTC : PASS_FORMS;
    const int n = s.model_class == PASS_MODEL_NONE ? 0 : (rtc ? N_PASS_FORMS_RTC : N_PASS_FORMS);
    if (sw < 1 || s.M < 128 || s.M % 128 != 0 || s.ns % sw != 0) return nullptr;
    for (int i = 0; i < n; ++i) {
        const PassForm& f = rows[i];
        if (pass_class_applies(f.cls, s.ns) && pass_class_sw(f.cls, s.ns) == sw && f.nst == nst && f.bk == bk && f.ct == ct && f.hs == hs && f.dop == dop &&
            (f.slices || !sliced) && form_fits(f, s))
            return &f;
    }
    return nullptr;
}

inline PassResolved resolve_form(const PassWants& w, const PassShape& s) {
    PassResolved r;
    const bool sliced = w.ks > 1;
    int nst = 3, bk = 8, ct = 1, hs = 1;
    bool dop = false;
    if (!find_form(s, w.sw, sliced, nst, bk, ct, hs, dop)) return r;
    if (w.nst == 4 && find_form(s, w.sw, sliced, 4, bk, ct, hs, dop)) nst = 4;
    if (w.bk == 16 && find_form(s, w.sw, sliced, nst, 16, ct, hs, dop)) bk = 16;
    if (w.ct == 2 && find_form(s, w.sw, sliced, nst, bk, 2, hs, dop)) ct = 2;
    if (w.hs == 2 && find_form(s, w.sw, sliced, nst, bk, ct, 2, dop)) hs = 2;
    if (w.dop && find_form(s, w.sw, sliced, nst, bk, ct, hs, true)) dop = true;
    r.row = find_form(s, w.sw, sliced, nst, bk, ct, hs, dop);
    r.sw = w.sw;
    r.ks = w.ks;
    r.res = (w.res == 3 && r.row && pass_form_max_res(*r.row) >= 3) ? 3 : 2;
    return r;
}

struct PassPolicyIn {
    int ns = 0, M = 0;
    int real_bytes = 8;
    int rows = 0;
    int model_class = PASS_MODEL_NONE;
    int rtc_sw_large = 0;
    bool f32 = false, symmetric = false, has_dfrag = false;
    int allow_fused = 1, overlap_mode = 0, sym_ct = 0, sym_ksplit = 0, sym_cpart = 0, sym_gblk = 0, sym_cx = 0, sym_nst = 3, sym_hs = 0, sym_ctc = 0,
        sym_bk = 0, sym_dop = 0, sym_res = 0, pass_order = -1, node_store = -1, slice = 0, small_rows = 24;
};

inline bool pass_overlapped(const PassPolicyIn& in) {
    if (in.f32 || !in.allow_fused || !in.symmetric || in.M <= 0 || in.model_class == PASS_MODEL_NONE) return false;
    if (in.model_class == PASS_MODEL_RTC) return in.M % 128 == 0;
    return symdefect_shape_ok(in.M, in.sym_ct);
}

inline int pass_tiles16(const PassPolicyIn& in, int B) { return ((B + 15) / 16) * (in.M / 128); }

inline int store_mode_for(const PassPolicyIn& in, int B) {
    if (in.node_store >= 0) return in.node_store;
    if ((size_t)B * in.rows * in.M * in.real_bytes > ((size_t)230 << 20)) return 2;
    const int tiles16 = pass_tiles16(in, B);
    if (tiles16 > 16 && tiles16 <= 32) return 0;
    return (in.model_class != PASS_MODEL_RTC && !in.f32) ? 1 : 0;
}

enum PassBandNeeds : unsigned {
    BAND_EVEN_NS = 1u,
    BAND_FREE_KS = 2u,
    BAND_FREE_DEPTH = 4u,
    BAND_FREE_ORDER = 8u,
    BAND_DEFAULT = 16u,
    BAND_FREE_RES = 32u,
};
enum PassKsRule {
    KS_UNSPLIT,
    KS_BY_WORKGROUPS,
};
struct PassBand {
    int lo, hi;
    unsigned needs;
    int sw_ct;
    PassKsRule ks;
    int bk;
    int dop;
    int order;
    int res = 2;
};
constexpr unsigned BAND_DEEP = BAND_DEFAULT | BAND_FREE_DEPTH;
inline constexpr PassBand PASS_BANDS[] = {
    {33, 48, BAND_DEEP | BAND_FREE_KS | BAND_EVEN_NS, 7, KS_UNSPLIT, 16, 1, 1},
    {80, 80, BAND_DEEP | BAND_FREE_KS | BAND_EVEN_NS | BAND_FREE_RES, 6, KS_UNSPLIT, 16, 2, 1, 3},
    {49, 127, BAND_DEEP | BAND_FREE_KS | BAND_EVEN_NS, 6, KS_UNSPLIT, 16, 1, 1},
    {144, 207, BAND_DEEP | BAND_FREE_ORDER | BAND_EVEN_NS, 6, KS_BY_WORKGROUPS, 16, 1, 150},
    {208, 215, BAND_DEEP | BAND_FREE_ORDER, 6, KS_BY_WORKGROUPS, 16, 1, 125},
    {512, 1024, BAND_DEEP | BAND_FREE_ORDER | BAND_EVEN_NS | BAND_FREE_RES, 6, KS_BY_WORKGROUPS, 16, 2, 110, 3},
    {216, 383, BAND_DEEP | BAND_FREE_ORDER, 6, KS_BY_WORKGROUPS, 16, 2, 125},
    {384, 767, BAND_DEEP | BAND_FREE_ORDER, 6, KS_BY_WORKGROUPS, 16, 2, 110},
    {768, 1024, BAND_DEEP | BAND_FREE_ORDER, 6, KS_BY_WORKGROUPS, 16, 2, 0},
    {0, 127, 0, 7, KS_BY_WORKGROUPS, 8, 1, 1},
    {128, 207, 0, 6, KS_BY_WORKGROUPS, 8, 1, 1},
    {208, 383, 0, 6, KS_BY_WORKGROUPS, 8, 1, 125},
    {384, 767, 0, 6, KS_BY_WORKGROUPS, 8, 1, 110},
    {768, INT_MAX, 0, 6, KS_BY_WORKGROUPS, 8, 1, 0},
};

struct PassLargeBatch { int above, whole; int gblk, ct, cx; };
inline constexpr PassLargeBatch PASS_LARGE_BATCH = {2048, 256, 2, 2, 1};

inline const PassBand& band_for(const PassPolicyIn& in, int tiles16, bool auto_ct) {
    unsigned met = 0;
    if (in.ns % 2 == 0 && in.ns > 2) met |= BAND_EVEN_NS;
    if (in.sym_ksplit == 0) met |= BAND_FREE_KS;
    if (in.sym_bk == 0 && in.sym_nst == 3) met |= BAND_FREE_DEPTH;
    if (in.pass_order < 0) met |= BAND_FREE_ORDER;
    if (in.sym_res == 0 && in.sym_dop != 1 && in.sym_hs <= 1 && in.sym_ctc <= 1 && in.sym_ksplit <= 1) met |= BAND_FREE_RES;
    if (auto_ct && in.model_class == PASS_MODEL_BUILTIN) met |= BAND_DEFAULT;
    const PassBand* b = PASS_BANDS;
    while (!(tiles16 >= b->lo && tiles16 <= b->hi && (b->needs & ~met) == 0)) ++b;
    return *b;
}

struct PassPlan {
    bool one_launch = false;
    SymPlan sym;
    int tiles16 = 0;
    int store_mode = 0;
    int mfma_first = 0;
};

inline SymPlan plan_tiles(const PassPolicyIn& in, int B, const PassWants& w, const PassResolved& r, int gblk, int band_cx) {
    const PassForm& f = *r.row;
    const bool wide_order = f.ct == 2 || (in.model_class == PASS_MODEL_BUILTIN && w.ct == 2 && r.sw == 2 && r.ks == 1 && w.nst == 3 && in.M % 256 == 0);
    const int cx = in.sym_cx ? in.sym_cx : (wide_order ? band_cx : 0);
    SymPlan p = plan_symdefect(in.ns, B, in.M, symdefect_ct_of(in.ns, r.sw), r.ks, in.sym_cpart, gblk, cx, 8, wide_order ? 2 : 1);
    p.tiles = p.tiles * p.ct / f.ct;
    p.nst = f.nst;
    p.bk = f.bk;
    p.ct = f.ct;
    p.hs = f.hs;
    p.dop = f.dop;
    p.res = r.res;
    return p;
}

inline PassPlan plan_pass(const PassPolicyIn& in, int B, bool jac) {
    PassPlan p;
    p.tiles16 = pass_tiles16(in, B);
    p.store_mode = store_mode_for(in, B);
    const bool auto_mode = in.overlap_mode == 0, rtc = in.model_class == PASS_MODEL_RTC;
    if (!((in.overlap_mode == 3 || auto_mode) && jac) || in.M % 128 != 0) return p;
    const bool auto_ct = auto_mode && (in.sym_ct == 0 || in.sym_ct == 4);
    const PassBand& band = band_for(in, p.tiles16, auto_ct);
    const bool large = B > PASS_LARGE_BATCH.above && B % PASS_LARGE_BATCH.whole == 0 && in.sym_cpart == 0;
    const bool wide_large = auto_ct && large && in.sym_ctc == 0;
    const int ct_code = rtc ? ((p.store_mode == 2 && in.rtc_sw_large == 2) ? 6 : 7) : (auto_ct ? band.sw_ct : in.sym_ct);
    PassWants w;
    w.sw = symdefect_sw(in.ns, p.tiles16, ct_code);
    if (w.sw == 0) w.sw = in.ns;
    w.ks = in.sym_ksplit;
    if (w.ks == 0 && auto_ct && band.ks == KS_BY_WORKGROUPS) {
        const int wgs = p.tiles16 * (in.ns / w.sw);
        w.ks = wgs * 4 <= 256 ? 4 : (wgs * 2 <= 512 ? 2 : 1);
    }
    w.ks = legal_ks((in.M / 2) / 8, w.ks);
    w.nst = in.sym_nst;
    w.bk = in.sym_bk ? in.sym_bk : band.bk;
    w.ct = in.sym_ctc ? in.sym_ctc : (wide_large ? PASS_LARGE_BATCH.ct : 1);
    w.hs = in.sym_hs ? in.sym_hs : 1;
    w.dop = (in.sym_dop ? in.sym_dop : band.dop) == 2;
    w.res = (in.sym_res ? in.sym_res : band.res) == 3 ? 3 : 2;
    const int gblk = (large && in.sym_gblk == 0 && (rtc || (auto_ct && w.ks == 1))) ? PASS_LARGE_BATCH.gblk : in.sym_gblk;
    PassShape s;
    s.ns = in.ns;
    s.M = in.M;
    s.model_class = in.model_class;
    s.has_dfrag = in.has_dfrag;
    s.store_mode = p.store_mode;
    const PassResolved r = resolve_form(w, s);
    if (!r) return p;
    p.sym = plan_tiles(in, B, w, r, gblk, wide_large ? PASS_LARGE_BATCH.cx : 0);
    p.mfma_first = in.pass_order >= 0 ? in.pass_order : band.order;
    p.one_launch = true;
    return p;
}

inline bool pass_takes_small_batches(const PassPolicyIn& in) {
    if (!pass_overlapped(in) || (in.overlap_mode != 0 && in.overlap_mode != 3) || in.M % 128 != 0) return false;
    PassShape s;
    s.ns = in.ns;
    s.M = in.M;
    s.model_class = in.model_class;
    PassWants w;
    w.sw = 1;
    return (bool)resolve_form(w, s);
}

inline int plan_piece(const PassPolicyIn& in, int B) {
    const long long cap = ((0xFFFFFFFFLL / ((long long)in.ns * in.M * 8)) / 256) * 256;
    int piece = 0;
    if (in.slice > 0) { if (B > 2 * in.slice) piece = in.slice; }
    else if (B > 2048) piece = (int)std::min<long long>(cap > 0 ? cap : 256, B - B % 256);
    return piece >= B ? 0 : piece;
}

inline void report_pass(const PassPolicyIn& in, int B, emi_pass_plan_t* out, bool* dop = nullptr, int* res = nullptr) {
    if (dop) *dop = false;
    if (res) *res = 0;
    if (!pass_overlapped(in)) return;
    const int piece = plan_piece(in, B);
    out->piece = piece;
    out->tail = piece > 0 ? B % piece : 0;
    const PassPlan p = plan_pass(in, piece > 0 ? piece : B, true);
    out->one_launch = p.one_launch ? 1 : 0;
    out->sw = p.sym.sw;
    out->ksplit = p.sym.ks;
    out->ring_stages = p.sym.nst;
    out->k_tile = p.sym.bk;
    out->column_tiles = p.sym.ct;
    out->k_halves = p.sym.hs;
    out->cpart = p.sym.cpart;
    out->cx = p.sym.cx;
    out->mfma_workgroups = p.sym.tiles * p.sym.ks;
    out->store_mode = p.store_mode;
    out->block_order = p.mfma_first;
    out->tiles16 = p.tiles16;
    if (dop) *dop = p.sym.dop;
    if (res) *res = p.one_launch ? p.sym.res : 0;
}

}
```

### etol_amd/csrc/emi_rtc.hip

```cpp
#include <hip/hip_runtime.h>
#include <hip/hiprtc.h>

#include <cstdio>
#include <cstring>
#include <map>
#include <mutex>
#include <string>
#include <vector>

#include "emi_kernels.hpp"
#include "emi_rtc_sources.inc"

namespace emi {

struct RtcModel {
    hipModule_t mod = nullptr;
    hipFunction_t nodes[2][2][2] = {};
    hipFunction_t hess = nullptr;
    hipFunction_t ode_resid = nullptr;
    hipFunction_t ode_resid_delay = nullptr;
    hipFunction_t ring = nullptr;
    hipFunction_t pass[N_PASS_FORMS_RTC] = {};
    hipFunction_t node_nt = nullptr;
    bool f32 = false;
// ... 91 lines not shown
    hiprtcGetProgramLogSize(p, &ls);
    std::string l(ls, '\0');
    if (ls) hiprtcGetProgramLog(p, &l[0]);
    while (!l.empty() && l.back() == '\0') l.pop_back();
    if (r != HIPRTC_SUCCESS) {
        if (log) *log = std::string("model program does not compile (") + hiprtcGetErrorString(r) + "):\n" + l;
        hiprtcDestroyProgram(&p);
        return EMI_ERR_ARG;
    }
    if (log) *log = l;
    lowered->clear();
    for (const std::string* s : order) {
        const char* low = nullptr;
        if (hiprtcGetLoweredName(p, s->c_str(), &low) != HIPRTC_SUCCESS || !low) {
            if (log) *log = "no lowered name for " + *s;
            hiprtcDestroyProgram(&p);
            return EMI_ERR_HIP;
        }
        lowered->push_back(low);
    }
    size_t cs = 0;
    hiprtcGetCodeSize(p, &cs);
    code->resize(cs);
    hiprtcGetCode(p, code->data());
    hiprtcDestroyProgram(&p);
    *has_ring = with_ring;
    return EMI_OK;
}

hipError_t launch(hipFunction_t f, dim3 grid, dim3 block, size_t lds, hipStream_t s, const void* args, size_t bytes) {
    if (!f) return hipErrorInvalidDeviceFunction;
    void* config[] = {HIP_LAUNCH_PARAM_BUFFER_POINTER, const_cast<void*>(args), HIP_LAUNCH_PARAM_BUFFER_SIZE, &bytes,
                      HIP_LAUNCH_PARAM_END};
    return hipModuleLaunchKernel(f, grid.x, grid.y, grid.z, block.x, block.y, block.z, (unsigned)lds, s, nullptr,
                                 config);
}

}

int rtc_check(bool f32, const char* struct_name, const char* source, int ns, int nc, int npath, int pw, std::string* log) {
    std::vector<char> code;
    std::vector<std::string> low;
    bool ring = false;
    return compile(f32, struct_name, source, ns, nc, npath, pw, &code, &low, &ring, log);
}

namespace {
struct CachedProgram {
    std::vector<char> code;
    std::vector<std::string> lowered;
    bool ring = false;
};
std::mutex g_cache_mutex;
std::map<std::string, CachedProgram> g_cache;
}

int rtc_build(bool f32, const char* struct_name, const char* source, int ns, int nc, int npath, int pw, RtcModel** out,
              std::string* log) {
    *out = nullptr;
    std::vector<char> code;
    std::vector<std::string> low;
    bool ring = false;
    const std::string key = std::string(f32 ? "f32|" : "f64|") + (struct_name ? struct_name : "") + "|" + std::to_string(ns) + "|" +
                            std::to_string(nc) + "|" + std::to_string(npath) + "|" + (source ? source : "");
    bool hit = false;
    {
        std::lock_guard<std::mutex> lk(g_cache_mutex);
        auto it = g_cache.find(key);
        if (it != g_cache.end()) {
            code = it->second.code;
            low = it->second.lowered;
            ring = it->second.ring;
            hit = true;
        }
    }
    if (!hit) {
        const int st = compile(f32, struct_name, source, ns, nc, npath, pw, &code, &low, &ring, log);
        if (st) return st;
        std::lock_guard<std::mutex> lk(g_cache_mutex);
        CachedProgram& cp = g_cache[key];
        cp.code = code;
        cp.lowered = low;
        cp.ring = ring;
    }
    RtcModel* m = new RtcModel();
    m->f32 = f32;
    m->ns = ns;
    m->nc = nc;
    hipError_t e = hipModuleLoadData(&m->mod, code.data());
    size_t i = 0;
    for (int v = 0; v < 2 && e == hipSuccess; ++v)
        for (int j = 0; j < 2 && e == hipSuccess; ++j)
            for (int d = 0; d < 2 && e == hipSuccess; ++d) e = hipModuleGetFunction(&m->nodes[v][j][d], m->mod, low[i++].c_str());
    if (e == hipSuccess) e = hipModuleGetFunction(&m->hess, m->mod, low[i++].c_str());
    if (e == hipSuccess && !f32) e = hipModuleGetFunction(&m->ode_resid, m->mod, low[i++].c_str());
    if (e == hipSuccess && !f32) e = hipModuleGetFunction(&m->ode_resid_delay, m->mod, low[i++].c_str());
    if (e == hipSuccess && ring) {
        e = hipModuleGetFunction(&m->ring, m->mod, low[i++].c_str());
        m->ring_lds = ring_lds_bytes(ns);
        for (int k = 0; k < N_PASS_FORMS_RTC && e == hipSuccess; ++k) e = hipModuleGetFunction(&m->pass[k], m->mod, low[i++].c_str());
        if (e == hipSuccess) e = hipModuleGetFunction(&m->node_nt, m->mod, low[i++].c_str());
    }
    if (e != hipSuccess) {
        if (log) *log = std::string("loading the model code object failed: ") + hipGetErrorString(e);
        rtc_destroy(m);
        return EMI_ERR_HIP;
    }
    *out = m;
    return EMI_OK;
}

void rtc_destroy(RtcModel* m) {
    if (!m) return;
    if (m->mod) (void)hipModuleUnload(m->mod);
    delete m;
}

bool rtc_has_symdefect(const RtcModel* m) { return m && m->ring; }

template <typename T>
hipError_t rtc_launch_nodes(RtcModel* m, const NodeArgs<T>& a, bool jac, bool defect_rows, hipStream_t s) {
    const bool vec2 = a.M % 2 == 0;
    const int per_block = EMI_NODE_THREADS * (vec2 ? 2 : 1);
    dim3 grid((a.M + per_block - 1) / per_block, a.B), block(EMI_NODE_THREADS);
    return launch(m->nodes[vec2][jac][defect_rows], grid, block, 0, s, &a, sizeof a);
}
template hipError_t rtc_launch_nodes<double>(RtcModel*, const NodeArgs<double>&, bool, bool, hipStream_t);
template hipError_t rtc_launch_nodes<float>(RtcModel*, const NodeArgs<float>&, bool, bool, hipStream_t);

template <typename T> hipError_t rtc_launch_hess(RtcModel* m, const HessArgs<T>& a, hipStream_t s) {
    dim3 grid((a.M + EMI_NODE_THREADS - 1) / EMI_NODE_THREADS, a.B), block(EMI_NODE_THREADS);
    return launch(m->hess, grid, block, 0, s, &a, sizeof a);
}
template hipError_t rtc_launch_hess<double>(RtcModel*, const HessArgs<double>&, hipStream_t);
template hipError_t rtc_launch_hess<float>(RtcModel*, const HessArgs<float>&, hipStream_t);

hipError_t rtc_launch_ode_resid(RtcModel* m, const OdeResidArgs<double>& a, hipStream_t s) {
    dim3 grid((a.M - 1 + EMI_NODE_THREADS - 1) / EMI_NODE_THREADS, a.B), block(EMI_NODE_THREADS);
    return launch(m->ode_resid, grid, block, 0, s, &a, sizeof a);
}

hipError_t rtc_launch_ode_resid_delay(RtcModel* m, const OdeResidDelayArgs<double>& a, hipStream_t s) {
    dim3 grid((a.M - 1 + EMI_NODE_THREADS - 1) / EMI_NODE_THREADS, a.B), block(EMI_NODE_THREADS);
    return launch(m->ode_resid_delay, grid, block, 0, s, &a, sizeof a);
}

hipError_t rtc_launch_symdefect(RtcModel* m, const SymDefectArgs& a, hipStream_t s) {
    const int mtiles = (a.B + FUSED_TI - 1) / FUSED_TI, ntiles = (a.M / 2) / 64;
    return launch(m->ring, dim3(mtiles * ntiles), dim3(256), m->ring_lds, s, &a, sizeof a);
}

int rtc_pass_sw_large(const RtcModel* m) { return m ? pass_class_sw(SWC_LARGE, m->ns) : 0; }

hipError_t rtc_launch_pass(RtcModel* m, const SymDefectArgs& sa, const NodeArgs<double>& na, int sw, hipStream_t s) {
    PassShape shape;
    shape.ns = m->ns;
    shape.M = sa.M;
    shape.model_class = PASS_MODEL_RTC;
    shape.store_mode = na.store_mode;
    const PassForm* f = find_form(shape, sw, sa.ksplit > 1, 3, 8, 1, 1, false);
    if (!f || !m->pass[f - PASS_FORMS_RTC]) return hipErrorInvalidDeviceFunction;
    PassArgs a;
    a.s = sa;
    a.n = na;
    const int mtiles = (sa.B + FUSED_TI - 1) / FUSED_TI, ntiles = (sa.M / 2) / 64;
    const int nm = mtiles * ntiles * (m->ns / sw) * (sa.ksplit > 1 ? sa.ksplit : 1);
    a.nbx = (na.M + 2 * EMI_NODE_THREADS - 1) / (2 * EMI_NODE_THREADS);
    const int nn = a.nbx * na.B;
    a.nm = nm;
    a.nn = nn;
    a.nm8 = (nm + 7) / 8;
    a.nn8 = (nn + 7) / 8;
    const size_t lds = (size_t)f->nst * ((2 * sw * FUSED_TI + 2 * 64 + 63) / 64 * 64) * f->bk * sizeof(double);
    return launch(m->pass[f - PASS_FORMS_RTC], dim3(8 * (a.nm8 + a.nn8)), dim3(256), lds, s, &a, sizeof a);
}

hipError_t rtc_launch_nodes_nt(RtcModel* m, const NodeArgs<double>& a, hipStream_t s) {
    if (!m->node_nt || a.M % 2) return hipErrorInvalidDeviceFunction;
    dim3 grid((a.M + 2 * EMI_NODE_THREADS - 1) / (2 * EMI_NODE_THREADS), a.B), block(EMI_NODE_THREADS);
    return launch(m->node_nt, grid, block, 0, s, &a, sizeof a);
}

}
```

### etol_amd/csrc/emi_symdefect.hip

```cpp
#include <hip/hip_runtime.h>

#include <type_traits>

#include "emi_kernels.hpp"
#include "emi_models.hpp"
#include "emi_symdefect_kernels.hpp"

namespace emi {

template <class Model>
static hipError_t launch_symdefect_ring_model(const SymDefectArgs& a, hipStream_t s, bool set_attr) {
    constexpr int NS = Model::NS;
    const int mtiles = (a.B + FUSED_TI - 1) / FUSED_TI, ntiles = (a.M / 2) / 64;
    const size_t lds = (size_t)3 * (2 * NS * FUSED_TI + 2 * 64) * 16 * sizeof(double);
    if (set_attr) {
        hipError_t e = hipFuncSetAttribute((const void*)emi_symdefect_ring_f64_kernel<Model>,
                                           hipFuncAttributeMaxDynamicSharedMemorySize, (int)lds);
        if (e != hipSuccess) return e;
    }
    dim3 grid(mtiles * ntiles), block(256);
    hipLaunchKernelGGL((emi_symdefect_ring_f64_kernel<Model>), grid, block, lds, s, a);
    return hipGetLastError();
}

template <class Model, int CT>
static hipError_t launch_symdefect_model(const SymDefectArgs& a, hipStream_t s, bool set_attr) {
    constexpr int NS = Model::NS, TN = 64 * CT;
    const int mtiles = (a.B + FUSED_TI - 1) / FUSED_TI, ntiles = (a.M / 2) / TN;
    const size_t lds = (size_t)2 * (2 * NS * FUSED_TI + 2 * TN) * (FUSED_BK + 2) * sizeof(double);
    if (set_attr) {
        hipError_t e = hipFuncSetAttribute((const void*)emi_symdefect_f64_kernel<Model, CT>,
                                           hipFuncAttributeMaxDynamicSharedMemorySize, (int)lds);
        if (e != hipSuccess) return e;
    }
    dim3 grid(mtiles * ntiles), block(256);
    hipLaunchKernelGGL((emi_symdefect_f64_kernel<Model, CT>), grid, block, lds, s, a);
    return hipGetLastError();
}

template <class Model, int SW>
static hipError_t launch_ring2_model(const SymDefectArgs& a, hipStream_t s) {
    constexpr int NS = Model::NS;
    const int mtiles = (a.B + FUSED_TI - 1) / FUSED_TI, ntiles = (a.M / 2) / 64;
    const size_t lds = (size_t)3 * ((2 * SW * FUSED_TI + 2 * 64 + 63) / 64 * 64) * 8 * sizeof(double);
    static bool attr_done = false;
    if (!attr_done) {
        hipError_t e = hipFuncSetAttribute((const void*)emi_symdefect_ring2_f64_kernel<Model, SW>,
                                           hipFuncAttributeMaxDynamicSharedMemorySize, (int)lds);
        if (e != hipSuccess) return e;
        attr_done = true;
    }
    const int tiles = mtiles * ntiles * (NS / SW), ks = a.ksplit > 1 ? a.ksplit : 1;
    hipLaunchKernelGGL((emi_symdefect_ring2_f64_kernel<Model, SW>), dim3(tiles * ks), dim3(256), lds, s, a);
    if (ks > 1 && a.tile_ticket == nullptr) hipLaunchKernelGGL((emi_symdefect_combine_kernel<Model, SW>), dim3(tiles), dim3(256), 0, s, a);
    return hipGetLastError();
}

template <class Model>
static hipError_t launch_ring2_planned(const SymDefectArgs& a, hipStream_t s, const SymPlan& p) {
    constexpr int NS = Model::NS;
    if (p.sw == NS) return launch_ring2_model<Model, NS>(a, s);
    if constexpr (NS > 2 && NS % 2 == 0) {
        if (p.sw == 2) return launch_ring2_model<Model, 2>(a, s);
    }
    if constexpr (NS > 3 && NS % 3 == 0) {
        if (p.sw == 3) return launch_ring2_model<Model, 3>(a, s);
    }
    return launch_ring2_model<Model, 1>(a, s);
}

template <class Model, int SW, int NST, int BK = 8, int CT = 1, int HS = 1, bool DOP = false>
static hipError_t launch_pass_model(const SymDefectArgs& sa, const NodeArgs<double>& na, hipStream_t s, int res) {
    constexpr int NS = Model::NS;
    PassArgs a;
    a.s = sa;
    a.n = na;
    const int mtiles = (sa.B + FUSED_TI - 1) / FUSED_TI, ntiles = (sa.M / 2) / (64 * CT);
    const int nm = mtiles * ntiles * (NS / SW) * (sa.ksplit > 1 ? sa.ksplit : 1);
    a.nbx = (na.M + 2 * EMI_NODE_THREADS - 1) / (2 * EMI_NODE_THREADS);
    const int nn = a.nbx * na.B;
    a.nm = nm;
    a.nn = nn;
    a.nm8 = (nm + 7) / 8;
    a.nn8 = ((nn + HS - 1) / HS + 7) / 8;
    const size_t lds = DOP ? (size_t)NST * (2 * SW * FUSED_TI) * BK * sizeof(double)
                           : (size_t)HS * NST * ((2 * SW * FUSED_TI + 2 * 64 * CT + 63) / 64 * 64) * BK * sizeof(double);
    if (DOP && (!sa.Dfrag || sa.ksplit > 1)) return hipErrorInvalidValue;
    const int st = (na.store_mode >= 0 && na.store_mode <= 3) ? na.store_mode : 0;
    constexpr bool HAS_KEEP = NST == 3 && HS == 1;
    const bool keep = HAS_KEEP && na.keep;
    const bool res3 = DOP && res == 3;
    auto pick = [&](auto keep_c, auto res_c) {
        constexpr bool K = decltype(keep_c)::value;
        constexpr int R = decltype(res_c)::value;
        return st == 2 ? emi_pass_f64_kernel<Model, SW, 2, 2, NST, BK, CT, HS, K, DOP, R>
             : (st == 1 ? emi_pass_f64_kernel<Model, SW, 2, 1, NST, BK, CT, HS, K, DOP, R>
                        : (st == 3 ? emi_pass_f64_kernel<Model, SW, 2, 3, NST, BK, CT, HS, K, DOP, R> : emi_pass_f64_kernel<Model, SW, 2, 0, NST, BK, CT, HS, K, DOP, R>));
    };
    using res2_t = std::integral_constant<int, 2>;
    using res3_t = std::integral_constant<int, 3>;
    auto kern = pick(std::false_type{}, res2_t{});
    if constexpr (HAS_KEEP) {
        if (keep) kern = pick(std::true_type{}, res2_t{});
    }
    if constexpr (DOP) {
        if (res3) kern = pick(std::false_type{}, res3_t{});
        if constexpr (HAS_KEEP) {
            if (res3 && keep) kern = pick(std::true_type{}, res3_t{});
        }
    }
    static bool attr_done[2][2][4] = {};
    if (!attr_done[res3][keep][st]) {
        hipError_t e = hipFuncSetAttribute((const void*)kern, hipFuncAttributeMaxDynamicSharedMemorySize, (int)lds);
        if (e != hipSuccess) return e;
        attr_done[res3][keep][st] = true;
    }
    hipLaunchKernelGGL(kern, dim3(8 * (a.nm8 + a.nn8)), dim3(256 * HS), lds, s, a);
    return hipGetLastError();
}

template <class Model>
static hipError_t launch_pass_planned(const SymDefectArgs& sa, const NodeArgs<double>& na, hipStream_t s, const SymPlan& p) {
    constexpr int NS = Model::NS;
#define EMI_PASS_FORM_LAUNCH(CLS, NST, BK, CT, HS, DOP, SLICES, STORES)                                                                   \
    if constexpr (pass_class_applies(CLS, NS)) {                                                                                          \
        if (p.sw == pass_class_sw(CLS, NS) && p.nst == NST && p.bk == BK && p.ct == CT && p.hs == HS && p.dop == DOP && (SLICES || p.ks == 1)) \
            return launch_pass_model<Model, pass_class_sw(CLS, NS), NST, BK, CT, HS, DOP>(sa, na, s, p.res);                             \
    }
    EMI_PASS_FORMS(EMI_PASS_FORM_LAUNCH)
#undef EMI_PASS_FORM_LAUNCH
    return hipErrorInvalidValue;
}

bool pass_model_supported(int model) { return model == EMI_MODEL_POINTMASS2D || model == EMI_MODEL_QUADROTOR2D; }

hipError_t launch_pass(int model, const SymDefectArgs& sa, const NodeArgs<double>& na, hipStream_t s, const SymPlan& p) {
    if (model == EMI_MODEL_POINTMASS2D) return launch_pass_planned<PointMass2D<double>>(sa, na, s, p);
    if (model == EMI_MODEL_QUADROTOR2D) return launch_pass_planned<Quadrotor2D<double>>(sa, na, s, p);
    return hipErrorInvalidValue;
}

bool fused_supported(int model, int M, int ct) {
    return pass_model_supported(model) && symdefect_shape_ok(M, ct);
}

hipError_t launch_symdefect(int model, const SymDefectArgs& a, hipStream_t s, bool set_attr, int ct, const SymPlan& plan) {
    if (!plan.ring1) {
        if (model == EMI_MODEL_POINTMASS2D) return launch_ring2_planned<PointMass2D<double>>(a, s, plan);
        if (model == EMI_MODEL_QUADROTOR2D) return launch_ring2_planned<Quadrotor2D<double>>(a, s, plan);
        return hipErrorInvalidValue;
    }
    if (ct == 0 || ct >= 4) {
        ct = 3;
        set_attr = true;
    }
    if (ct == 3) {
        if (model == EMI_MODEL_POINTMASS2D) return launch_symdefect_ring_model<PointMass2D<double>>(a, s, set_attr);
        if (model == EMI_MODEL_QUADROTOR2D) return launch_symdefect_ring_model<Quadrotor2D<double>>(a, s, set_attr);
        return hipErrorInvalidValue;
    }
    if (model == EMI_MODEL_POINTMASS2D)
        return ct == 1 ? launch_symdefect_model<PointMass2D<double>, 1>(a, s, set_attr)
                       : launch_symdefect_model<PointMass2D<double>, 2>(a, s, set_attr);
    if (model == EMI_MODEL_QUADROTOR2D)
        return ct == 1 ? launch_symdefect_model<Quadrotor2D<double>, 1>(a, s, set_attr)
                       : launch_symdefect_model<Quadrotor2D<double>, 2>(a, s, set_attr);
    return hipErrorInvalidValue;
}

}
```

### etol_amd/csrc/emi_symdefect_kernels.hpp

```cpp
#pragma once
#include "emi_args.hpp"
#include "emi_node_kernels.hpp"

namespace emi {

typedef double d4 __attribute__((ext_vector_type(4)));
typedef double d2 __attribute__((ext_vector_type(2)));
template <bool C, class A, class B> struct emi_pick { typedef A type; };
template <class A, class B> struct emi_pick<false, A, B> { typedef B type; };

template <class Model, int CT>
__global__ __launch_bounds__(256, CT == 1 ? 2 : 1) void emi_symdefect_f64_kernel(SymDefectArgs a) {
    constexpr int NS = Model::NS, NC = Model::NC, NV = Model::NV;
    constexpr int TI = FUSED_TI, TM = NS * TI, TN = 64 * CT, BK = FUSED_BK, LDK = BK + 2;
    constexpr int A_PASS = TM * (BK / 2) / 256;
    constexpr int B_PASS = TN * (BK / 2) / 256;
    static_assert(TM * (BK / 2) % 256 == 0 && TN * (BK / 2) % 256 == 0, "staging shape");
    static_assert(TN % 64 == 0 && TI == 16, "wave layout below assumes 16 instances x 64*CT columns");
    constexpr int STAGE = (2 * TM + 2 * TN) * LDK;

    extern __shared__ __attribute__((aligned(16))) double smem[];

    const int M = a.M, Hh = M >> 1, B = a.B;
    const int mtiles = (B + TI - 1) / TI;
// ... 260 lines not shown
        double* __restrict__ Rb = a.RES + (size_t)inst * a.nres * M;
#pragma unroll
        for (int side = 0; side < 2; ++side) {
            const int node = side == 0 ? node_f : node_m;
            double z[NV], f[NS];
#pragma unroll
            for (int v = 0; v < NS; ++v) z[v] = Xb[(size_t)v * M + node];
#pragma unroll
            for (int v = 0; v < NC; ++v) z[NS + v] = Ub[(size_t)v * M + node];
            Model::f(a.P, z, a.node_t[node], f);
#pragma unroll
            for (int s = 0; s < NS; ++s) {
                const double dx = side == 0 ? acc_a[s][i] + acc_b[s][i] : acc_b[s][i] - acc_a[s][i];
                Rb[(size_t)s * M + node] = dx - a.h * f[s];
            }
        }
    }
}

EMI_DEV constexpr int ring_swz(int r) { return (0 - (r >> 2)) & 3; }
#ifndef EMI_EPILOGUE_PREFETCH
#define EMI_EPILOGUE_PREFETCH 0
#endif
template <int BK> EMI_DEV constexpr int ring_swz_k(int r) { return BK == 8 ? ring_swz(r) : ((r >> 1) & 7); }

template <class Model>
EMI_DEV void ring_epilogue_load(const SymDefectArgs& a, double (&z)[2][Model::NV], int inst, int node_f) {
    constexpr int NS = Model::NS, NC = Model::NC;
    const int M = a.M, node_m = M - 1 - node_f;
    inst = inst < a.B ? inst : a.B - 1;
    const double* __restrict__ Xb = a.X + (size_t)inst * NS * M;
    const double* __restrict__ Ub = a.U + (size_t)inst * NC * M;
#pragma unroll
    for (int side = 0; side < 2; ++side) {
        const int node = side == 0 ? node_f : node_m;
#pragma unroll
        for (int v = 0; v < NS; ++v) z[side][v] = Xb[(size_t)v * M + node];
#pragma unroll
        for (int v = 0; v < NC; ++v) z[side][NS + v] = Ub[(size_t)v * M + node];
    }
}
template <class Model, int SW, int S0, bool PRE>
EMI_DEV void ring_epilogue_s0(const SymDefectArgs& a, const d4 (&acc_a)[SW], const d4 (&acc_b)[SW], int inst0, int i0,
                              int wid, int r16, int kq, const double (&zpre)[2][Model::NV]) {
    constexpr int NS = Model::NS, NC = Model::NC, NV = Model::NV;
    const int M = a.M, B = a.B;
    const int col = wid * 16 + r16;
    const int node_f = i0 + col, node_m = M - 1 - node_f;
    const double t_f = a.node_t[node_f], t_m = a.node_t[node_m];
    if constexpr (SW == 1) {
        if (a.ablate & 4) return;
        double zz[4][2][NV];
#pragma unroll
        for (int i = 0; i < 4; ++i) {
            int inst = inst0 + kq + 4 * i;
            inst = inst < B ? inst : B - 1;
            const double* __restrict__ Xb = a.X + (size_t)inst * NS * M;
            const double* __restrict__ Ub = a.U + (size_t)inst * NC * M;
#pragma unroll
            for (int side = 0; side < 2; ++side) {
                const int node = side == 0 ? node_f : node_m;
#pragma unroll
                for (int v = 0; v < NS; ++v) zz[i][side][v] = Xb[(size_t)v * M + node];
#pragma unroll
                for (int v = 0; v < NC; ++v) zz[i][side][NS + v] = Ub[(size_t)v * M + node];
            }
        }
#pragma unroll
        for (int i = 0; i < 4; ++i) {
            const int inst = inst0 + kq + 4 * i;
            if (inst >= B) continue;
            double* __restrict__ Rb = a.RES + (size_t)inst * a.nres * M;
#pragma unroll
            for (int side = 0; side < 2; ++side) {
                double f[NS];
                Model::f(a.P, zz[i][side], side == 0 ? t_f : t_m, f);
                const double dx = side == 0 ? acc_a[0][i] + acc_b[0][i] : acc_b[0][i] - acc_a[0][i];
                Rb[(size_t)S0 * M + (side == 0 ? node_f : node_m)] = dx - a.h * f[S0];
            }
        }
        return;
    }
    if (a.ablate & 4) return;
    auto load_z = [&](double (&z)[2][NV], int i) {
        int inst = inst0 + kq + 4 * i;
        inst = inst < B ? inst : B - 1;
        const double* __restrict__ Xb = a.X + (size_t)inst * NS * M;
        const double* __restrict__ Ub = a.U + (size_t)inst * NC * M;
#pragma unroll
        for (int side = 0; side < 2; ++side) {
            const int node = side == 0 ? node_f : node_m;
#pragma unroll
            for (int v = 0; v < NS; ++v) z[side][v] = Xb[(size_t)v * M + node];
#pragma unroll
            for (int v = 0; v < NC; ++v) z[side][NS + v] = Ub[(size_t)v * M + node];
        }
    };
    double zc[2][NV], zn[2][NV];
    if constexpr (PRE) {
#pragma unroll
        for (int side = 0; side < 2; ++side)
#pragma unroll
            for (int v = 0; v < NV; ++v) zc[side][v] = zpre[side][v];
    } else {
        load_z(zc, 0);
    }
#pragma unroll
    for (int i = 0; i < 4; ++i) {
        if (i < 3) load_z(zn, i + 1);
        const int inst = inst0 + kq + 4 * i;
        if (inst < B) {
            double* __restrict__ Rb = a.RES + (size_t)inst * a.nres * M;
            double hf[2][SW];
#pragma unroll
            for (int side = 0; side < 2; ++side) {
                double f[NS];
                Model::f(a.P, zc[side], side == 0 ? t_f : t_m, f);
#pragma unroll
                for (int s = 0; s < SW; ++s) hf[side][s] = a.h * f[S0 + s];
            }
#pragma unroll
            for (int side = 0; side < 2; ++side) {
                const int node = side == 0 ? node_f : node_m;
#pragma unroll
                for (int s = 0; s < SW; ++s) {
                    const double dx = side == 0 ? acc_a[s][i] + acc_b[s][i] : acc_b[s][i] - acc_a[s][i];
                    Rb[(size_t)(S0 + s) * M + node] = dx - hf[side][s];
                }
            }
        }
        if (i < 3) {
#pragma unroll
            for (int side = 0; side < 2; ++side)
#pragma unroll
                for (int v = 0; v < NV; ++v) zc[side][v] = zn[side][v];
        }
    }
}
template <class Model, int SW, bool PRE, int SG = 0>
EMI_DEV void ring_epilogue_pre(const SymDefectArgs& a, const d4 (&acc_a)[SW], const d4 (&acc_b)[SW], int inst0, int i0,
                               int s0, int wid, int r16, int kq, const double (&zpre)[2][Model::NV]) {
    if constexpr (SG * SW < Model::NS) {
        if (s0 == SG * SW) ring_epilogue_s0<Model, SW, SG * SW, PRE>(a, acc_a, acc_b, inst0, i0, wid, r16, kq, zpre);
        else ring_epilogue_pre<Model, SW, PRE, SG + 1>(a, acc_a, acc_b, inst0, i0, s0, wid, r16, kq, zpre);
    }
}
template <class Model, int SW>
EMI_DEV void ring_epilogue(const SymDefectArgs& a, const d4 (&acc_a)[SW], const d4 (&acc_b)[SW], int inst0, int i0,
                           int s0, int wid, int r16, int kq) {
    const double none[2][Model::NV] = {};
    ring_epilogue_pre<Model, SW, false>(a, acc_a, acc_b, inst0, i0, s0, wid, r16, kq, none);
}

template <class Model, int SW, int NST = 3, int BK = 8, int CT = 1, int HS = 1, bool DOP = false>
EMI_DEV void emi_ring2_body(const SymDefectArgs& a, const int bid ) {
    constexpr int NS = Model::NS;
    constexpr int TI = FUSED_TI, TM = SW * TI, TN = 64 * CT, CH = BK / 2, NSG = NS / SW;
    static_assert(CT == 1 || CT == 2, "one or two column sub-tiles per wave");
    constexpr int KH = BK / 8;
    constexpr int RPI = 64 / CH;
    static_assert(BK == 8 || BK == 16, "K tiles of 8 or 16");
    constexpr int LOOK = NST - 1;
    static_assert(!DOP || (SW <= 2 && NST == 3 && BK == 16 && CT == 1 && HS == 1), "De / Do from L2: the unsplit 16-deep form only");
    constexpr int ROWS = 2 * TM + (DOP ? 0 : 2 * TN);
    constexpr int ROWS_PAD = DOP ? (ROWS + 4 * RPI - 1) / (4 * RPI) * (4 * RPI) : (ROWS + 63) / 64 * 64;
    constexpr int STAGE = ROWS_PAD * BK;
    constexpr int L = ROWS_PAD * CH / 256;
    static_assert(NS % SW == 0, "states split evenly over workgroups");

    extern __shared__ __attribute__((aligned(16))) double smem_all[];
    static_assert(HS == 1 || HS == 2, "the K range whole or in two halves");
    const int half = HS > 1 ? __builtin_amdgcn_readfirstlane((int)(threadIdx.x >> 8)) : 0;
    double* const smem = smem_all + (size_t)half * NST * STAGE;

    const int M = a.M, Hh = M >> 1, B = a.B;
    const int ntiles = Hh / TN;
    const int KS = (HS == 1 && !DOP && a.ksplit > 1) ? a.ksplit : 1;
    const int kslice = bid % KS;
    const RingTile rt = ring_tile_of(bid / KS, ntiles, (B + TI - 1) / TI * NSG, a.cpart, a.cx, NSG);
    const int ntile = rt.ntile, grp = rt.grp;
    const int tile = grp * ntiles + ntile;
    const int sg = grp % NSG, mtile = grp / NSG;
    const int inst0 = mtile * TI, i0 = ntile * TN, s0 = sg * SW;

    const int tid = threadIdx.x & 255, lane = tid & 63;
    const int wid = __builtin_amdgcn_readfirstlane(tid >> 6);
    const int r16 = lane & 15, kq = lane >> 4;

    unsigned voff[L];
    unsigned long long gbase[L];
    int gstep[L];
#pragma unroll
    for (int t = 0; t < L; ++t) {
        const int row0 = (wid + 4 * t) * RPI;
        const int row = row0 + lane / CH, p = lane % CH;
        if (row0 < 2 * TM) {
            const bool mir = row0 >= TM;
            const int rr = row - (mir ? TM : 0);
            const int c = p ^ ring_swz_k<BK>(rr);
            int inst = inst0 + (rr & 15);
            inst = inst < B ? inst : B - 1;
            if (a.ablate & 8) inst &= 15;
            voff[t] = (unsigned)((((size_t)inst * NS + s0 + (rr >> 4)) * M + 2 * c) * sizeof(double));
            gbase[t] = (unsigned long long)(a.X + (mir ? M - BK : 0));
            gstep[t] = mir ? -(int)(BK * sizeof(double)) : (int)(BK * sizeof(double));
        } else if (row0 < ROWS) {
            const bool od = row0 >= 2 * TM + TN;
            const int rr = row - 2 * TM - (od ? TN : 0);
            const int c = p ^ ring_swz_k<BK>(rr);
            voff[t] = (unsigned)(((size_t)((a.ablate & 64) ? rr : i0 + rr) * Hh + 2 * c) * sizeof(double));
            gbase[t] = (unsigned long long)(od ? a.Do : a.De);
            gstep[t] = (int)(BK * sizeof(double));
        } else {
            voff[t] = (unsigned)(2 * p * sizeof(double));
            gbase[t] = (unsigned long long)a.De;
            gstep[t] = 0;
        }
    }
    const unsigned lds0 = (unsigned)(unsigned long)(emi_lds_ptr_t)smem;
    const int nkt = (Hh / BK) / KS / HS, kt0 = (kslice * HS + half) * nkt;
    unsigned long long gnext[L];
#pragma unroll
    for (int t = 0; t < L; ++t) gnext[t] = gbase[t] + (long long)gstep[t] * kt0;
    unsigned st_dma = 0, st_rd = 0;
    int nd = 0;
    auto issue_one = [&](int t) {
        const unsigned dst = lds0 + st_dma + (unsigned)(wid + 4 * t) * 1024u;
        asm volatile("s_mov_b32 m0, %2\n\t" EMI_M0_NOP "global_load_lds_dwordx4 %0, %1" ::"v"(voff[t]), "s"(gnext[t]), "s"(dst) : "memory", "m0");
        gnext[t] += (long long)gstep[t];
        if (t == L - 1) {
            st_dma = st_dma == (unsigned)((NST - 1) * STAGE * 8) ? 0u : st_dma + (unsigned)(STAGE * 8);
            ++nd;
        }
    };
    auto issue = [&]() {
#pragma unroll
        for (int t = 0; t < L; ++t) issue_one(t);
    };
    constexpr int ND = DOP ? 2 * KH : 0;
    unsigned long long fnext = 0;
    const unsigned foff = (unsigned)lane * 16u;
    if constexpr (DOP)
        fnext = (unsigned long long)(a.Dfrag + ((size_t)(((a.ablate & 64) ? 0 : ntile) * 4 + wid) * (Hh / BK) + kt0) * (ND * 64 * 2));

    d4 acc_a[SW][CT], acc_b[SW][CT];
#pragma unroll
    for (int s = 0; s < SW; ++s)
#pragma unroll
        for (int c = 0; c < CT; ++c) {
            acc_a[s][c] = d4{0.0, 0.0, 0.0, 0.0};
            acc_b[s][c] = d4{0.0, 0.0, 0.0, 0.0};
        }

    constexpr bool EPI_PRE = EMI_EPILOGUE_PREFETCH && SW >= 2 && SW <= 3 && HS == 1 && CT == 1;
    double zpre[2][Model::NV] = {};
    if constexpr (EPI_PRE) ring_epilogue_load<Model>(a, zpre, inst0 + kq, i0 + wid * 16 + r16);

#pragma unroll
    for (int t = 0; t < LOOK; ++t)
        if (t < nkt) issue();
    int off_b[CT][KH], off_f[SW][KH], off_m[SW][KH];
#pragma unroll
    for (int c = 0; c < CT; ++c) {
        const int rb = c * 64 + wid * 16 + r16;
#pragma unroll
        for (int h = 0; h < KH; ++h) off_b[c][h] = rb * BK + (((kq + 4 * h) ^ ring_swz_k<BK>(rb)) << 1);
    }
#pragma unroll
    for (int s = 0; s < SW; ++s) {
        const int r = s * 16 + r16;
#pragma unroll
        for (int h = 0; h < KH; ++h) {
            off_f[s][h] = r * BK + (((kq + 4 * h) ^ ring_swz_k<BK>(r)) << 1);
            off_m[s][h] = (TM + r) * BK + (((CH - 1 - kq - 4 * h) ^ ring_swz_k<BK>(r)) << 1);
        }
    }
    typedef typename emi_pick<DOP, d2, double2>::type BFrag;
    struct Frag {
        BFrag be[CT][KH], bo[CT][KH];
        double2 sp[SW][KH], dm[SW][KH];
    };
    double2 txf[SW][KH], txm[SW][KH];
    constexpr int NB = DOP ? 0 : 2 * CT;
    constexpr int NRH = NB + 2 * SW;
    constexpr int NR = NRH * KH, NM = 4 * SW * CT * KH;
    auto read_one = [&](Frag& f, const double* S, int r) {
        const int h = r / NRH, q = r % NRH;
        if (q < NB) {
            if constexpr (NB > 0) {
                if (q & 1) f.bo[q >> 1][h] = *reinterpret_cast<const double2*>(S + (2 * TM + TN) * BK + off_b[q >> 1][h]);
                else f.be[q >> 1][h] = *reinterpret_cast<const double2*>(S + 2 * TM * BK + off_b[q >> 1][h]);
            }
        } else if (q & 1) txm[(q - NB) >> 1][h] = *reinterpret_cast<const double2*>(S + off_m[(q - NB) >> 1][h]);
        else txf[(q - NB) >> 1][h] = *reinterpret_cast<const double2*>(S + off_f[(q - NB) >> 1][h]);
    };
    auto dload_one = [&](Frag& f, int q) {
        if constexpr (DOP) {
            d2& dst = (q & 1) ? f.bo[0][q >> 1] : f.be[0][q >> 1];
            if (q == 0) asm volatile("global_load_dwordx4 %0, %1, %2" : "=v"(dst) : "v"(foff), "s"(fnext) : "memory");
            if (q == 1) asm volatile("global_load_dwordx4 %0, %1, %2 offset:1024" : "=v"(dst) : "v"(foff), "s"(fnext) : "memory");
            if (q == 2) asm volatile("global_load_dwordx4 %0, %1, %2 offset:2048" : "=v"(dst) : "v"(foff), "s"(fnext) : "memory");
            if (q == 3) asm volatile("global_load_dwordx4 %0, %1, %2 offset:3072" : "=v"(dst) : "v"(foff), "s"(fnext) : "memory");
            if (q == ND - 1) fnext += (unsigned long long)(ND * 1024);
        }
    };
    auto wait_counted = [&](Frag& f) {
        if constexpr (DOP) asm volatile("s_waitcnt vmcnt(%4)" : "+v"(f.be[0][0]), "+v"(f.bo[0][0]), "+v"(f.be[0][1]), "+v"(f.bo[0][1]) : "n"(L * (LOOK - 1)) : "memory");
        else asm volatile("s_waitcnt vmcnt(%0)" ::"n"(L * (LOOK - 1)) : "memory");
    };
    auto wait_all = [&](Frag& f) {
        if constexpr (DOP) asm volatile("s_waitcnt vmcnt(0)" : "+v"(f.be[0][0]), "+v"(f.bo[0][0]), "+v"(f.be[0][1]), "+v"(f.bo[0][1]) :: "memory");
        else asm volatile("s_waitcnt vmcnt(0)" ::: "memory");
    };
    auto sums_one = [&](Frag& f, int s) {
#pragma unroll
        for (int h = 0; h < KH; ++h) {
            f.sp[s][h] = double2{txf[s][h].x + txm[s][h].y, txf[s][h].y + txm[s][h].x};
            f.dm[s][h] = double2{txf[s][h].x - txm[s][h].y, txf[s][h].y - txm[s][h].x};
        }
    };
    auto rd_stage = [&]() -> const double* {
        const double* S = smem + (st_rd >> 3);
        st_rd = st_rd == (unsigned)((NST - 1) * STAGE * 8) ? 0u : st_rd + (unsigned)(STAGE * 8);
        return S;
    };
    auto read_frag = [&](Frag& f) {
        const double* S = rd_stage();
#pragma unroll
        for (int r = 0; r < NR; ++r) read_one(f, S, r);
#pragma unroll
        for (int s = 0; s < SW; ++s) sums_one(f, s);
    };
    auto mfma_one = [&](const Frag& f, int i) {
// ... 6 lines not shown
    auto multiply = [&](const Frag& f) {
#pragma unroll
        for (int i = 0; i < NM; ++i) mfma_one(f, i);
    };
    if constexpr (SW <= 3) {
        constexpr int RPG = DOP ? NR / ND : (NR + (NM - L) - 1) / (NM - L);
        constexpr int GR = (NR + RPG - 1) / RPG;
        static_assert(NM > L && GR + L <= NM, "a gap for every DMA instruction after the reads");
        static_assert(!DOP || GR == ND, "a direct load in every gap that takes reads");
        struct Ahead { enum { drained = 0 }; };
        struct Tail { enum { drained = 1 }; };
        auto step = [&](Frag& cur, Frag& nxt, int kt, auto tail) {
            if constexpr (DOP) {
                if constexpr (decltype(tail)::drained) wait_all(cur);
                else wait_counted(cur);
            } else if (kt + LOOK < nkt) wait_counted(cur);
            else wait_all(cur);
            __builtin_amdgcn_s_waitcnt(0xC07F);
            asm volatile("s_barrier" ::: "memory");
            const bool more = nd < nkt;
            const double* S = rd_stage();
#pragma unroll
            for (int i = 0; i < NM; ++i) {
                mfma_one(cur, i);
                if (DOP && i < ND) dload_one(nxt, i);
                if (i < GR) {
#pragma unroll
                    for (int r = i * RPG; r < (i + 1) * RPG && r < NR; ++r) read_one(nxt, S, r);
                } else if (i < GR + L) {
                    if (more) issue_one(i - GR);
                }
                if (i >= NM - SW) sums_one(nxt, i - (NM - SW));
                __builtin_amdgcn_sched_barrier(0);
            }
        };
        Frag f0, f1;
        if constexpr (DOP) {
#pragma unroll
            for (int q = 0; q < ND; ++q) dload_one(f0, q);
            wait_all(f0);
        } else if (nkt > LOOK - 1) wait_counted(f0);
        else wait_all(f0);
        asm volatile("s_barrier" ::: "memory");
        if (LOOK < nkt) issue();
        __builtin_amdgcn_s_waitcnt(0xC07F);
        read_frag(f0);
        int kt = 0;
        for (; kt + 2 < nkt; kt += 2) {
            step(f0, f1, kt, Ahead{});
            step(f1, f0, kt + 1, Ahead{});
        }
        step(f0, f1, kt, Tail{});
        if constexpr (DOP) wait_all(f1);
        multiply(f1);
    } else {
        for (int kt = 0; kt < nkt; ++kt) {
            if (kt + LOOK - 1 < nkt) asm volatile("s_waitcnt vmcnt(%0)" ::"n"(L * (LOOK - 1)) : "memory");
            else                     asm volatile("s_waitcnt vmcnt(0)" ::: "memory");
            asm volatile("s_barrier" ::: "memory");
            if (kt + LOOK < nkt) issue();
            Frag f;
            read_frag(f);
            multiply(f);
        }
    }

    if (CT == 1 && KS > 1) {
        double* sl = a.slab + ((size_t)tile * KS + kslice) * (2 * SW * 4) * 256 + tid;
        if (a.tile_ticket == nullptr) {
#pragma unroll
            for (int s = 0; s < SW; ++s)
#pragma unroll
                for (int i = 0; i < 4; ++i) {
                    sl[(size_t)((2 * s) * 4 + i) * 256] = acc_a[s][0][i];
                    sl[(size_t)((2 * s + 1) * 4 + i) * 256] = acc_b[s][0][i];
                }
            return;
        }
#pragma unroll
        for (int s = 0; s < SW; ++s)
#pragma unroll
            for (int i = 0; i < 4; ++i) {
                __hip_atomic_store(sl + (size_t)((2 * s) * 4 + i) * 256, acc_a[s][0][i], __ATOMIC_RELAXED, __HIP_MEMORY_SCOPE_AGENT);
                __hip_atomic_store(sl + (size_t)((2 * s + 1) * 4 + i) * 256, acc_b[s][0][i], __ATOMIC_RELAXED, __HIP_MEMORY_SCOPE_AGENT);
            }
        asm volatile("s_waitcnt vmcnt(0)" ::: "memory");
        __syncthreads();
        unsigned* flag = reinterpret_cast<unsigned*>(smem);
        if (tid == 0) *flag = __hip_atomic_fetch_add(a.tile_ticket + tile, 1u, EMI_TICKET_ORDER, __HIP_MEMORY_SCOPE_AGENT);
        __syncthreads();
        if (*flag != (unsigned)KS - 1u) return;
#pragma unroll
        for (int s = 0; s < SW; ++s) {
            acc_a[s][0] = d4{0.0, 0.0, 0.0, 0.0};
            acc_b[s][0] = d4{0.0, 0.0, 0.0, 0.0};
        }
        for (int k = 0; k < KS; ++k) {
            const double* sk = a.slab + ((size_t)tile * KS + k) * (2 * SW * 4) * 256 + tid;
#pragma unroll
            for (int s = 0; s < SW; ++s)
#pragma unroll
                for (int i = 0; i < 4; ++i) {
                    acc_a[s][0][i] += __hip_atomic_load(sk + (size_t)((2 * s) * 4 + i) * 256, __ATOMIC_RELAXED, __HIP_MEMORY_SCOPE_AGENT);
                    acc_b[s][0][i] += __hip_atomic_load(sk + (size_t)((2 * s + 1) * 4 + i) * 256, __ATOMIC_RELAXED, __HIP_MEMORY_SCOPE_AGENT);
                }
        }
        if (tid == 0) __hip_atomic_store(a.tile_ticket + tile, 0u, __ATOMIC_RELAXED, __HIP_MEMORY_SCOPE_AGENT);
    }
    __builtin_amdgcn_s_setprio(0);
    if constexpr (HS == 2) {
        asm volatile("s_waitcnt lgkmcnt(0)" ::: "memory");
        __syncthreads();
        double* cb = smem_all + tid;
        if (half == 1) {
#pragma unroll
            for (int s2 = 0; s2 < SW; ++s2)
#pragma unroll
                for (int c = 0; c < CT; ++c)
#pragma unroll
                    for (int i = 0; i < 4; ++i) {
                        cb[(size_t)(((2 * s2) * CT + c) * 4 + i) * 256] = acc_a[s2][c][i];
                        cb[(size_t)(((2 * s2 + 1) * CT + c) * 4 + i) * 256] = acc_b[s2][c][i];
                    }
        }
        __syncthreads();
        if (half == 1) return;
#pragma unroll
        for (int s2 = 0; s2 < SW; ++s2)
#pragma unroll
            for (int c = 0; c < CT; ++c)
#pragma unroll
                for (int i = 0; i < 4; ++i) {
                    acc_a[s2][c][i] += cb[(size_t)(((2 * s2) * CT + c) * 4 + i) * 256];
                    acc_b[s2][c][i] += cb[(size_t)(((2 * s2 + 1) * CT + c) * 4 + i) * 256];
                }
    }
#pragma unroll
    for (int c = 0; c < CT; ++c) {
        d4 ea[SW], eb[SW];
#pragma unroll
        for (int s2 = 0; s2 < SW; ++s2) { ea[s2] = acc_a[s2][c]; eb[s2] = acc_b[s2][c]; }
        if (c == 0) ring_epilogue_pre<Model, SW, EPI_PRE>(a, ea, eb, inst0, i0, s0, wid, r16, kq, zpre);
        else ring_epilogue<Model, SW>(a, ea, eb, inst0, i0 + 64 * c, s0, wid, r16, kq);
    }
}

template <class Model, int SW>
__global__ __launch_bounds__(256, 2) void emi_symdefect_ring2_f64_kernel(SymDefectArgs a) {
    int bid = blockIdx.x;
    {
        const int nwg = gridDim.x, xcd = bid & 7, q = nwg >> 3, rr = nwg & 7;
        bid = (xcd < rr ? xcd * (q + 1) : rr * (q + 1) + (xcd - rr) * q) + (bid >> 3);
    }
    emi_ring2_body<Model, SW>(a, bid);
}

template <class Model, int SW>
__global__ __launch_bounds__(256) void emi_symdefect_combine_kernel(SymDefectArgs a) {
    constexpr int NS = Model::NS, TI = FUSED_TI, TN = 64, NSG = NS / SW;
    const int ntiles = (a.M >> 1) / TN, KS = a.ksplit;
    const int tile = blockIdx.x;
    const int ntile = tile % ntiles, grp = tile / ntiles;
    const int sg = grp % NSG, mtile = grp / NSG;
    const int tid = threadIdx.x, lane = tid & 63, wid = tid >> 6;
    d4 acc_a[SW], acc_b[SW];
#pragma unroll
    for (int s = 0; s < SW; ++s) {
        acc_a[s] = d4{0.0, 0.0, 0.0, 0.0};
        acc_b[s] = d4{0.0, 0.0, 0.0, 0.0};
    }
    for (int k = 0; k < KS; ++k) {
        const double* sl = a.slab + ((size_t)tile * KS + k) * (2 * SW * 4) * 256 + tid;
#pragma unroll
        for (int s = 0; s < SW; ++s)
#pragma unroll
            for (int i = 0; i < 4; ++i) {
                acc_a[s][i] += sl[(size_t)((2 * s) * 4 + i) * 256];
                acc_b[s][i] += sl[(size_t)((2 * s + 1) * 4 + i) * 256];
            }
    }
    ring_epilogue<Model, SW>(a, acc_a, acc_b, mtile * TI, ntile * TN, sg * SW, wid, lane & 15, lane >> 4);
}


#define EMI_STR2(x) #x
#define EMI_STR(x) EMI_STR2(x)
#ifndef EMI_PASS_WAVES_PER_EU
#define EMI_PASS_WAVES_PER_EU 0
#endif
#if EMI_PASS_WAVES_PER_EU > 0
#define EMI_PASS_OCC __attribute__((amdgpu_waves_per_eu(EMI_PASS_WAVES_PER_EU, EMI_PASS_WAVES_PER_EU)))
#elif EMI_PASS_WAVES_PER_EU < 0
#define EMI_PASS_OCC
#else
#define EMI_PASS_OCC __attribute__((amdgpu_waves_per_eu(SW > 3 ? 1 : 2, RES)))
#endif
template <class Model, int SW, int VEC, int ST, int NST = 3, int BK = 8, int CT = 1, int HS = 1, bool KEEP = false, bool DOP = false, int RES = 2>
__global__ __launch_bounds__(256 * HS) EMI_PASS_OCC void emi_pass_f64_kernel(PassArgs a) {
    static_assert(RES == 2 || (RES == 3 && DOP), "three resident workgroups per CU: direct-operator forms only");
#ifdef EMI_ENTRY_PAD_NOPS
    asm volatile(".rept " EMI_STR(EMI_ENTRY_PAD_NOPS) "\n\ts_nop 0\n\t.endr" ::: "memory");
#endif
    const int g = blockIdx.x, xcd = g & 7, j = g >> 3;
    const PassRole role = pass_role_of(j, a.nm8, a.nn8, a.s.mfma_first);
    if (a.s.ablate & (role.mfma ? 16 : 32)) return;
    if (role.mfma) {
        const int tid = xcd * a.nm8 + role.index;
        if (tid >= a.nm) return;
        __builtin_amdgcn_s_setprio(3);
        emi_ring2_body<Model, SW, NST, BK, CT, HS, DOP>(a.s, tid);
    } else {
        const int nid = (xcd * a.nn8 + role.index) * HS + (HS > 1 ? (int)(threadIdx.x >> 8) : 0);
        if (nid >= a.nn) return;
        emi_nodes_body<double, Model, VEC, true, false, ST, false, KEEP>(a.n, nid % a.nbx, nid / a.nbx, a.nbx);
    }
}

}
```

### etol_amd/evaluator.py

```python
import ctypes as C

import numpy as np
import torch

from . import _lib as L


def _dp(a):
    return a.ctypes.data_as(C.POINTER(C.c_double))


def lgl(M):
    lib = L.load()
    tau = np.empty(M)
    w = np.empty(M)
    D = np.empty((M, M))
    L.check(lib.emi_lgl(M, _dp(tau), _dp(w), _dp(D)), what="emi_lgl")
    return tau, w, D


def model_dims(model):
    lib = L.load()
    ns, nc, npar = C.c_int(), C.c_int(), C.c_int()
    L.check(lib.emi_model_dims(model, C.byref(ns), C.byref(nc), C.byref(npar)), what="emi_model_dims")
# ... 716 lines not shown
            g.grid, g.repair = int(d.get("grid", 0)), int(bool(d.get("repair")))
        return arr

    def ipm_solve_restart(self, rungs, t0, tf, starts, U0, X0=None, ode_tol=None, first_check=0, ul=None, uu=None, patience=None,
                          retry_mask=0, flags=0, ldm=None, out=None, dev=True):
        lay = self.layout
        B, ns, nc, npth = lay.B, lay.ns, lay.nc, lay.np
        keep = []
        arr = self._ipm_rungs(rungs, keep)
        ldm = int(ldm if ldm is not None else (out[0].shape[-1] if out is not None else max([int(r["M"]) for r in rungs] or [0])))
        if out is not None:
            X, U, LamF, LamC = out
        elif dev:
            kw = dict(dtype=torch.float64, device=U0.device)
            X, U, LamF, LamC = (torch.zeros((B, r, ldm), **kw) for r in (ns, nc, ns, npth))
        else:
            X, U, LamF, LamC = (np.zeros((B, r, ldm)) for r in (ns, nc, ns, npth))
        if not dev:
            assert all(a is None or (a.dtype == np.float64 and a.flags.c_contiguous) for a in (X0, U0, X, U, LamF, LamC))
        rf = None
        if ode_tol is not None:
            rf = L.IpmRefine()
            rf.ode_tol, rf.first_check = float(ode_tol), int(first_check)
            for f, a in (("ul", ul), ("uu", uu)):
                if a is not None:
                    a = np.ascontiguousarray(a, dtype=np.float64)
                    keep.append(a)
                    setattr(rf, f, _dp(a))
        rs = L.IpmRestart()
        rs.nstarts, rs.retry_mask, rs.flags = len(starts), int(retry_mask), int(flags)
        if len(starts):
            rs.starts = self._ipm_starts(starts, keep)
        nat = max(1, min(len(starts) + (X0 is not None), 8))
        if patience is not None:
            pat = np.ascontiguousarray(patience, dtype=np.int32)
            assert pat.size >= nat
            keep.append(pat)
            rs.patience = pat.ctypes.data_as(C.POINTER(C.c_int))
        nr = len(rungs)
        res = (L.IpmResult * max(1, nat * nr * B))()
        err = np.full((nat, max(1, nr), B), np.nan)
        summ = (L.IpmRestartResult * B)()
        A = self._ipm_addr
        fn = self.lib.emi_ipm_solve_restart_dev if dev else self.lib.emi_ipm_solve_restart_host
        st = fn(self.ctx, nr, arr, float(t0), float(tf), C.byref(rf) if rf is not None else None, C.byref(rs), A(X0), A(U0), ldm, A(X), A(U),
                A(LamF), A(LamC) if npth else None, res, _dp(err), summ)
        self._changed()
        self._trk_shape = self._wp_shape
        self._ck(st, fn.__name__)
        Ml = self.layout.M
        self.tau, self.w, self.D = lgl(Ml)
        self.node_t = t0 + (tf - t0) / 2.0 * (self.tau + 1.0)
        fields = [n for n, _ in L.IpmResult._fields_]
        results = [[[{n: getattr(res[(a * nr + r) * B + b], n) for n in fields} for b in range(B)] for r in range(nr)] for a in range(nat)]
        summary = [dict(attempt=q.attempt, attempts=q.attempts, level=q.level,
                        **{n: getattr(q.refine, n) for n, _ in L.IpmRefineResult._fields_}) for q in summ]
        return X, U, LamF, LamC, results, err[:, :nr], summary

    @staticmethod
    def ode_error_operator(M, mesh=None):
        lib = L.load()
        tau, w = (np.ascontiguousarray(a, dtype=np.float64) for a in (mesh if mesh is not None else lgl(M))[:2])
        n = 5 * (int(M) - 1)
        E, Ed, tq = np.empty((n, int(M))), np.empty((n, int(M))), np.empty(n)
        L.check(lib.emi_ode_error_operator(int(M), _dp(tau), _dp(w), _dp(E), _dp(Ed), _dp(tq)), what="emi_ode_error_operator")
        return E, Ed, tq

    def interp(self, OP, V, K=None, out=None):
        N, ldk = OP.shape
        K = int(ldk if K is None else K)
        assert V.shape[-1] == K and OP.is_contiguous() and V.is_contiguous()
        R = V.numel() // K
        if out is None:
            out = torch.empty(tuple(V.shape[:-1]) + (N,), dtype=torch.float64, device=V.device)
        assert out.is_contiguous() and out.numel() == R * out.shape[-1]
        self._ck(self.lib.emi_interp_dev(self.ctx, K, int(N), int(ldk), C.c_void_p(OP.data_ptr()), C.c_void_p(V.data_ptr()), int(R),
                                         int(out.shape[-1]), C.c_void_p(out.data_ptr())), "emi_interp_dev")
        return out

    def ode_error(self, X, U, ul=None, uu=None, eta=True, dev=True):
        lay = self.layout
        bd = [None if a is None else np.ascontiguousarray(a, dtype=np.float64) for a in (ul, uu)]
        pb = [None if a is None else _dp(a) for a in bd]
        if dev:
            kw = dict(dtype=torch.float64, device=X.device)
            err = torch.empty((lay.B,), **kw)
            Eta = torch.empty((lay.B, lay.ns, lay.M - 1), **kw) if eta else None
        else:
            assert all(a.dtype == np.float64 and a.flags.c_contiguous for a in (X, U))
            err, Eta = np.empty(lay.B), (np.empty((lay.B, lay.ns, lay.M - 1)) if eta else None)
        A = self._ipm_addr
        fn = self.lib.emi_ode_error_dev if dev else self.lib.emi_ode_error_host
        self._ck(fn(self.ctx, A(X), A(U), pb[0], pb[1], A(Eta), A(err)), fn.__name__)
        return err, Eta

    @staticmethod
    def ode_error_delay_operator(M, mesh=None, t0=0.0, tf=1.0, delay=0.0):
        lib = L.load()
        tau, w = (np.ascontiguousarray(a, dtype=np.float64) for a in (mesh if mesh is not None else lgl(M))[:2])
        Edel = np.empty((5 * (int(M) - 1), int(M)))
        L.check(lib.emi_ode_error_delay_operator(int(M), _dp(tau), _dp(w), float(t0), float(tf), float(delay), _dp(Edel)),
                what="emi_ode_error_delay_operator")
        return Edel

    def ode_error_total(self, X, U, ul=None, uu=None, eta=True, dev=True):
        lay = self.layout
        bd = [None if a is None else np.ascontiguousarray(a, dtype=np.float64) for a in (ul, uu)]
        pb = [None if a is None else _dp(a) for a in bd]
        if dev:
            kw = dict(dtype=torch.float64, device=X.device)
            err = torch.empty((lay.B,), **kw)
            Eta = torch.empty((lay.B, lay.ns, lay.M - 1), **kw) if eta else None
        else:
            assert all(a.dtype == np.float64 and a.flags.c_contiguous for a in (X, U))
            err, Eta = np.empty(lay.B), (np.empty((lay.B, lay.ns, lay.M - 1)) if eta else None)
        A = self._ipm_addr
        fn = self.lib.emi_ode_error_total_dev if dev else self.lib.emi_ode_error_total_host
        self._ck(fn(self.ctx, A(X), A(U), pb[0], pb[1], A(Eta), A(err)), fn.__name__)
        return err, Eta

    def timer_start(self):
        self._ck(self.lib.emi_timer_start(self.ctx), "emi_timer_start")

    def timer_stop(self):
        ms = C.c_float()
        self._ck(self.lib.emi_timer_stop(self.ctx, C.byref(ms)), "emi_timer_stop")
        return ms.value

    def profile(self, level):
        self._ck(self.lib.emi_profile_enable(self.ctx, int(level)), "emi_profile_enable")

    def profile_read(self):
        nm, dm, fm = C.c_float(), C.c_float(), C.c_float()
        nl, dl, fl = C.c_int(), C.c_int(), C.c_int()
        self._ck(self.lib.emi_profile_read(self.ctx, C.byref(nm), C.byref(nl), C.byref(dm), C.byref(dl), C.byref(fm),
                                           C.byref(fl)), "emi_profile_read")
        return dict(node_ms=nm.value, node_launches=nl.value, defect_ms=dm.value, defect_launches=dl.value,
                    pass_ms=fm.value, overlapped_passes=fl.value)

    def set_option(self, name, value):
        self._ck(self.lib.emi_set_option(self.ctx, name.encode(), int(value)), "emi_set_option")

    def plan(self, B=None):
        p = L.PassPlan()
        self._ck(self.lib.emi_plan_pass(self.ctx, int(B if B is not None else self.layout.B), C.byref(p)), "emi_plan_pass")
        return {n: getattr(p, n) for n, _ in L.PassPlan._fields_}

    def plan_residency(self, B=None):
        res = C.c_int(0)
        self._ck(self.lib.emi_plan_pass_residency(self.ctx, int(B if B is not None else self.layout.B), C.byref(res)), "emi_plan_pass_residency")
        return res.value

    @property
    def last_defect_kernel(self):
        return self.lib.emi_last_defect_kernel(self.ctx).decode()

    @property
    def uses_fused_kernel(self):
        f = C.c_int()
        self._ck(self.lib.emi_last_path(self.ctx, C.byref(f)), "emi_last_path")
        return bool(f.value)
```

### include/emi355x.h

```cpp
#ifndef EMI355X_H_
#define EMI355X_H_

#include <stddef.h>

#ifdef __cplusplus
extern "C" {
#endif

#define EMI_ABI_VERSION 2

typedef struct emi_ctx_s* emi_ctx_t;

enum {
    EMI_OK = 0,
    EMI_ERR_ARG = 1,
    EMI_ERR_STATE = 2,
    EMI_ERR_HIP = 3,
    EMI_ERR_NO_DEVICE = 4,
    EMI_ERR_UNSUPPORTED = 5,
    EMI_ERR_COMM = 6
};

enum {
    EMI_MODEL_POINTMASS2D = 0,
// ... 166 lines not shown
  int repair;
} emi_ipm_rung_t;
int emi_prolong_matrix(int Mc, const double* tau_c, const double* w_c, int Mf, const double* tau_f, double* P);
int emi_prolong_dev(emi_ctx_t ctx, int Mc, int Mf, const void* dPT, const void* dVc, int R, void* dVf);
int emi_repair_guess_dev(emi_ctx_t ctx, void* dX);
int emi_ipm_solve_ladder_dev(emi_ctx_t ctx, int nrungs, const emi_ipm_rung_t* rungs, double t0, double tf, const void* dX0,
                             const void* dU0, void* dX, void* dU, void* dLamF, void* dLamC, emi_ipm_result_t* results);
int emi_ipm_solve_ladder_host(emi_ctx_t ctx, int nrungs, const emi_ipm_rung_t* rungs, double t0, double tf, const double* X0,
                              const double* U0, double* X, double* U, double* LamF, double* LamC, emi_ipm_result_t* results);
int emi_ode_error_operator(int M, const double* tau, const double* w, double* E, double* Ed, double* tq);
int emi_interp_dev(emi_ctx_t ctx, int K, int N, int ldk, const void* dOP, const void* dV, int R, int ldo, void* dOut);
int emi_ode_error_dev(emi_ctx_t ctx, const void* dX, const void* dU, const double* ul, const double* uu, void* dEta, void* dErr);
int emi_ode_error_host(emi_ctx_t ctx, const double* X, const double* U, const double* ul, const double* uu, double* Eta, double* Err);
int emi_ode_error_delay_operator(int M, const double* tau, const double* w, double t0, double tf, double delay, double* Edel);
int emi_ode_error_total_dev(emi_ctx_t ctx, const void* dX, const void* dU, const double* ul, const double* uu, void* dEta, void* dErr);
int emi_ode_error_total_host(emi_ctx_t ctx, const double* X, const double* U, const double* ul, const double* uu, double* Eta, double* Err);
enum { EMI_REFINE_MET = 0, EMI_REFINE_NOT_MET = 1, EMI_REFINE_FELL_BACK = 2, EMI_REFINE_FAILED = 3 };
typedef struct emi_ipm_refine {
  double ode_tol;
  int first_check;
  const double *ul, *uu;
} emi_ipm_refine_t;
typedef struct emi_ipm_refine_result { int rung, verdict, rungs_solved; double err; } emi_ipm_refine_result_t;
int emi_ipm_refine_decide(int status, double err, double ode_tol, int has_good, int is_last, int* verdict);
int emi_prolong_rows_dev(emi_ctx_t ctx, int Mc, int Mf, const void* dPT, const void* dVc, int R, const void* dRowMap, void* dVf);
int emi_shard_move_dev(emi_ctx_t ctx, int n, const void* dSrcIdx, const void* dDstIdx, int narrays, const int* rows,
                       const void* const* src, const int* src_ld, void* const* dst, const int* dst_ld, int len);
int emi_ipm_solve_refine_dev(emi_ctx_t ctx, int nrungs, const emi_ipm_rung_t* rungs, double t0, double tf, const emi_ipm_refine_t* rf,
                             const void* dX0, const void* dU0, int ldm, void* dX, void* dU, void* dLamF, void* dLamC,
                             emi_ipm_result_t* results, double* err, emi_ipm_refine_result_t* out);
int emi_ipm_solve_refine_host(emi_ctx_t ctx, int nrungs, const emi_ipm_rung_t* rungs, double t0, double tf, const emi_ipm_refine_t* rf,
                              const double* X0, const double* U0, int ldm, double* X, double* U, double* LamF, double* LamC,
                              emi_ipm_result_t* results, double* err, emi_ipm_refine_result_t* out);
enum { EMI_START_LINE = 0, EMI_START_BEND = 1, EMI_START_PLANNED = 2 };
typedef struct emi_start {
  int kind;
  int nsets;
  const double* xa;
  const double* xb;
  const double* box;
  double bend;
  double clearance;
  int grid;
  int repair;
} emi_start_t;
int emi_plan_route(int np, const double* recs, const double ends[4], const double box[4], double clearance, int grid, int M,
                   const double* tau, double* xs, double* ys, int* level, double* cost, int* cells, int* ncells);
int emi_start_guess_dev(emi_ctx_t ctx, const emi_start_t* st, void* dX, void* dLevel);
int emi_start_guess_host(emi_ctx_t ctx, const emi_start_t* st, double* X, int* level);
enum { EMI_RESTART_DROP_FAILED = 1 };
typedef struct emi_ipm_restart {
  int nstarts;
  const emi_start_t* starts;
  const int* patience;
  int retry_mask;
  int flags;
} emi_ipm_restart_t;
typedef struct emi_ipm_restart_result {
  int attempt;
  int attempts;
  int level;
  emi_ipm_refine_result_t refine;
} emi_ipm_restart_result_t;
int emi_ipm_restart_decide(int verdict, int retry_mask);
int emi_ipm_solve_restart_dev(emi_ctx_t ctx, int nrungs, const emi_ipm_rung_t* rungs, double t0, double tf, const emi_ipm_refine_t* rf,
                              const emi_ipm_restart_t* rs, const void* dX0, const void* dU0, int ldm, void* dX, void* dU, void* dLamF,
                              void* dLamC, emi_ipm_result_t* results, double* err, emi_ipm_restart_result_t* out);
int emi_ipm_solve_restart_host(emi_ctx_t ctx, int nrungs, const emi_ipm_rung_t* rungs, double t0, double tf, const emi_ipm_refine_t* rf,
                               const emi_ipm_restart_t* rs, const double* X0, const double* U0, int ldm, double* X, double* U,
                               double* LamF, double* LamC, emi_ipm_result_t* results, double* err, emi_ipm_restart_result_t* out);
int emi_ipm_start_dev(emi_ctx_t ctx, int phase, const emi_ipm_point_t* pt, const emi_ipm_duals_t* du, const void* dRES,
                      const emi_ipm_bounds_t* bd, const void* dPar, double bound_push, double bound_frac, void* dFixed,
                      const void* dMask);
int emi_ipm_error_parts_dev(emi_ctx_t ctx, const emi_ipm_point_t* pt, const emi_ipm_duals_t* du, const void* dRES, const void* dG,
                            const emi_ipm_bounds_t* bd, const void* dPar, void* dOut);
int emi_ipm_error_parts_host(emi_ctx_t ctx, const emi_ipm_point_t* pt, const emi_ipm_duals_t* du, const double* RES, const double* G,
                             const emi_ipm_bounds_t* bd, const double* par, double* out);
int emi_ipm_keep_dev(emi_ctx_t ctx, const emi_ipm_point_t* pt, const emi_ipm_duals_t* du, const emi_ipm_point_t* kept_pt,
                     const emi_ipm_duals_t* kept_du, const void* dMask, int restore);
int emi_ipm_keep_host(emi_ctx_t ctx, const emi_ipm_point_t* pt, const emi_ipm_duals_t* du, const emi_ipm_point_t* kept_pt,
                      const emi_ipm_duals_t* kept_du, const unsigned char* mask, int restore);

typedef struct emi_pass_plan {
  int one_launch;
  int sw;
  int ksplit;
  int ring_stages;
  int cpart, cx;
  int mfma_workgroups;
  int store_mode;
  int block_order;
  int tiles16;
  int piece, tail;
  int k_tile;
  int column_tiles;
  int k_halves;
} emi_pass_plan_t;
int emi_plan_pass(emi_ctx_t ctx, int B, emi_pass_plan_t* out);
int emi_plan_pass_residency(emi_ctx_t ctx, int B, int* res);

int emi_jac_structure(emi_ctx_t ctx, int* rows, int* cols);
int emi_invariant_rows(int model, int np, unsigned char* mask, int* nvals);

int emi_dev_alloc(emi_ctx_t ctx, size_t bytes, void** dptr);
int emi_dev_free(emi_ctx_t ctx, void* dptr);
int emi_h2d(emi_ctx_t ctx, void* dst, const void* src, size_t bytes);
int emi_d2h(emi_ctx_t ctx, void* dst, const void* src, size_t bytes);

int emi_eval_dev(emi_ctx_t ctx, const void* dX, const void* dU, void* dRES,
                 void* dVALS, void* dCOST, unsigned flags);
int emi_eval_host(emi_ctx_t ctx, const double* X, const double* U, double* RES,
                  double* VALS, double* COST, unsigned flags);

int emi_hess_dev(emi_ctx_t ctx, const void* dX, const void* dU,
                 const void* dLamF, const void* dLamC, double sigma, void* dH);
int emi_hess_host(emi_ctx_t ctx, const double* X, const double* U,
                  const double* LamF, const double* LamC, double sigma,
                  double* H);

int emi_lagr_grad_dev(emi_ctx_t ctx, const void* dVALS, const void* dLamF, const void* dLamC, double sigma, void* dG);
int emi_lagr_grad_host(emi_ctx_t ctx, const double* VALS, const double* LamF, const double* LamC, double sigma, double* G);
int emi_kkt_certificate_dev(emi_ctx_t ctx, const void* dX, const void* dU, const void* dRES, const void* dVALS,
                            const void* dLamF, const void* dLamC, double sigma, const void* dZl, const void* dZu, int nsets,
                            const double* cl, const double* cu, void* dCert, void* dG);
int emi_kkt_certificate_host(emi_ctx_t ctx, const double* X, const double* U, const double* LamF, const double* LamC,
                             double sigma, const double* zl, const double* zu, int nsets, const double* cl, const double* cu,
                             double* cert, double* G);
int emi_lagr_grad_total_dev(emi_ctx_t ctx, const void* dVALS, const void* dLamF, const void* dLamC, double sigma, void* dG,
                            void* dGdel);
int emi_lagr_grad_total_host(emi_ctx_t ctx, const double* VALS, const double* LamF, const double* LamC, double sigma, double* G,
                             double* Gdel);
int emi_kkt_certificate_total_dev(emi_ctx_t ctx, const void* dX, const void* dU, const void* dRES, const void* dVALS,
                                  const void* dLamF, const void* dLamC, double sigma, const void* dZl, const void* dZu, int nsets,
                                  const double* cl, const double* cu, void* dCert, void* dG, void* dGdel);
int emi_kkt_certificate_total_host(emi_ctx_t ctx, const double* X, const double* U, const double* LamF, const double* LamC,
                                   double sigma, const double* zl, const double* zu, int nsets, const double* cl, const double* cu,
                                   double* cert, double* G, double* Gdel);

int emi_timer_start(emi_ctx_t ctx);
int emi_timer_stop(emi_ctx_t ctx, float* elapsed_ms);
int emi_profile_enable(emi_ctx_t ctx, int level);
int emi_profile_read(emi_ctx_t ctx, float* node_ms, int* node_launches,
                     float* defect_ms, int* defect_launches,
                     float* fused_ms, int* fused_launches);

int emi_set_option(emi_ctx_t ctx, const char* name, int value);
int emi_last_path(emi_ctx_t ctx, int* fused);
int emi_debug_tile_order(int ns, int B, int M, int sym_ct, int sym_cpart, int* out_tile, int out_cap, int* ntiles_total,
                         int* cpart, int* cx);
int emi_debug_tile_order2(int ns, int B, int M, int sym_ct, int sym_cpart, int sym_gblk, int sym_cx, int* out_tile, int out_cap,
                          int* ntiles_total, int* cpart, int* cx);
int emi_debug_operator_fragments(int M, const double* D, double* out);
int emi_debug_pass_roles(int nm, int nn, int order, int* out_role, int out_cap);
const char* emi_last_defect_kernel(emi_ctx_t ctx);

#define EMI_COMM_ID_BYTES 128
typedef struct emi_comm_s* emi_comm_t;
int emi_comm_unique_id(void* id );
int emi_comm_create(int device_id, int world, int rank, const void* id, emi_comm_t* out);
int emi_comm_gather(emi_comm_t comm, const void* dsend, void* drecv, size_t bytes, int root, void* hip_stream);
int emi_comm_destroy(emi_comm_t comm);
const char* emi_comm_last_error(emi_comm_t comm);

#ifdef __cplusplus
}
#endif
#endif
```

Measured before the change: 5.891 billion.

## Precompute one-launch pass work assignment into a cached device table

Replaces the per-workgroup role/tile decoding in the fused pass kernel (pass_role_of plus ring_tile_of index arithmetic) with a lookup into a host-built, device-resident table of packed work entries. The table is built per launch configuration key and kept in an 8-slot LRU cache on the context, so it is uploaded only when the configuration changes. This trims integer prologue work from each workgroup at the cost of one extra global load, an upload and possible stream sync on a cache miss, and more host-side bookkeeping. It also adds debug entry points to inspect the table and the upload count.

```diff
diff --git a/etol_amd/_lib.py b/etol_amd/_lib.py
--- a/etol_amd/_lib.py
+++ b/etol_amd/_lib.py
@@ -217,6 +217,8 @@
     "emi_last_defect_kernel": (C.c_char_p, [_P]),
     "emi_debug_pass_roles": (C.c_int, [C.c_int, C.c_int, C.c_int, C.POINTER(C.c_int), C.c_int]),
     "emi_debug_tile_order": (C.c_int, [C.c_int, C.c_int, C.c_int, C.c_int, C.c_int, C.POINTER(C.c_int), C.c_int, C.POINTER(C.c_int), C.POINTER(C.c_int), C.POINTER(C.c_int)]),
+    "emi_debug_pass_work": (C.c_int, [C.c_int] * 11 + [C.POINTER(C.c_int), C.c_int, C.POINTER(C.c_int)]),
+    "emi_debug_pass_work_uploads": (C.c_int, [_P, C.POINTER(C.c_ulonglong), _I]),
     "emi_set_delays": (C.c_int, [_P, C.c_int, C.c_int, C.c_double]),
     "emi_get_delays": (C.c_int, [_P, _I, _I, _I]),
     "emi_delay_matrix": (C.c_int, [C.c_int, C.POINTER(C.c_double), C.POINTER(C.c_double), C.c_double, C.c_double, C.c_double, C.POINTER(C.c_double)]),
diff --git a/etol_amd/csrc/emi_api_pass.hip b/etol_amd/csrc/emi_api_pass.hip
--- a/etol_amd/csrc/emi_api_pass.hip
+++ b/etol_amd/csrc/emi_api_pass.hip
@@ -229,6 +229,34 @@
     return emi::DefectArgsF32{(const float*)io.X, (const float*)c->d_D.p, (float*)io.RES, L.B * c->ns, c->M, c->ns, nres_of(c)};
 }
 
+int pass_work_table(emi_ctx_t c, const emi::PassWorkKey& key, const emi::PassWork** out) {
+    emi_api::PassWorkCache& pc = c->pass_work;
+    for (emi_api::PassWorkCache::Slot& sl : pc.slot)
+        if (sl.used && sl.key == key) {
+            sl.stamp = ++pc.clock;
+            *out = sl.dev.p;
+            return EMI_OK;
+        }
+    emi_api::PassWorkCache::Slot* lru = &pc.slot[0];
+    for (emi_api::PassWorkCache::Slot& sl : pc.slot)
+        if (lru->used && (!sl.used || sl.stamp < lru->stamp)) lru = &sl;
+    std::vector<emi::PassWork> table;
+    const char* why = "";
+    if (!emi::pass_work_build(key, table, &why))
+        return fail(c, EMI_ERR_UNSUPPORTED, "emi_eval: the launch does not fit the work table of the one-launch pass (%s)", why);
+    if (lru->used) HIP_TRY(c, hipStreamSynchronize(c->stream));
+    lru->used = false;
+    HIP_TRY(c, lru->dev.reserve(table.size()));
+    lru->host.swap(table);
+    HIP_TRY(c, hipMemcpyAsync(lru->dev.p, lru->host.data(), lru->host.size() * sizeof(emi::PassWork), hipMemcpyHostToDevice, c->stream));
+    lru->key = key;
+    lru->used = true;
+    lru->stamp = ++pc.clock;
+    ++pc.uploads;
+    *out = lru->dev.p;
+    return EMI_OK;
+}
+
 int form_pass_f64(emi_ctx_t c, Launch L, const PassIO& io, const emi::PassPlan& pp, ProfEvents* pe) {
     const emi::SymPlan& plan = pp.sym;
     emi::SymDefectArgs sa = sym_defect_args(c, L, io);
@@ -246,9 +274,12 @@
     }
     EMI_TRY(ensure_zeroed(c, c->d_ticket, (size_t)L.B * 4, c->stream));
     na.cost_ticket = (unsigned*)c->d_ticket.p;
+    const emi::PassWorkKey key = emi::pass_work_for(plan, c->ns, L.B, c->M, pp.mfma_first);
+    const emi::PassWork* work = nullptr;
+    EMI_TRY(pass_work_table(c, key, &work));
     EMI_TRY(prof_mark(c, pe, K0, AT_ANY, c->stream));
-    if (c->rtc) HIP_TRY(c, emi::rtc_launch_pass(c->rtc, sa, na, plan.sw, c->stream));
-    else HIP_TRY(c, emi::launch_pass(c->model, sa, na, c->stream, plan));
+    if (c->rtc) HIP_TRY(c, emi::rtc_launch_pass(c->rtc, sa, na, plan.sw, c->stream, key, work));
+    else HIP_TRY(c, emi::launch_pass(c->model, sa, na, c->stream, plan, key, work));
     EMI_TRY(prof_mark(c, pe, K1, AT_ANY, c->stream));
     if (pe) pe->level = -1;
     c->last_defect_kernel = name_pass_f64(plan);
@@ -587,6 +618,46 @@
     return EMI_OK;
 }
 
+int emi_debug_pass_work(int ns, int B, int M, int sw, int ctc, int ksplit, int hs, int sym_cpart, int sym_gblk, int sym_cx, int order, int* out,
+                        int out_cap, int* info) {
+    if (ns < 1 || B < 1 || M < 128 || M % 128 != 0 || sw < 1 || ns % sw != 0 || (ctc != 1 && ctc != 2) || ksplit < 1 || (hs != 1 && hs != 2) || !info)
+        return EMI_ERR_ARG;
+    emi::SymPlan p = emi::plan_symdefect(ns, B, M, emi::symdefect_ct_of(ns, sw), emi::legal_ks((M / 2) / 8, ksplit), sym_cpart, sym_gblk, sym_cx, 8, ctc);
+    if (p.ring1 || p.sw != sw || p.ct != ctc) return EMI_ERR_UNSUPPORTED;
+    p.hs = hs;
+    const emi::PassWorkKey key = emi::pass_work_for(p, ns, B, M, order);
+    std::vector<emi::PassWork> table;
+    if (!emi::pass_work_build(key, table)) return EMI_ERR_UNSUPPORTED;
+    const int vals[12] = {(int)key.blocks(), key.nm, key.nn, key.nm8, key.nn8, key.nbx, key.ntiles, key.ngrp, key.cpart, key.cx, key.ks, key.nsg};
+    for (int i = 0; i < 12; ++i) info[i] = vals[i];
+    for (int g = 0; out && g < (int)key.blocks() && 5 * (g + 1) <= out_cap; ++g) {
+        const emi::PassWork e = table[(size_t)emi::pass_work_index(g, key.per_xcd())];
+        int* o = out + 5 * (size_t)g;
+        o[0] = emi::pass_work_role(e);
+        o[1] = o[2] = o[3] = o[4] = 0;
+        if (o[0] == emi::PASS_WORK_MFMA) {
+            o[1] = emi::pass_work_ntile(e);
+            o[2] = emi::pass_work_grp(e);
+            o[3] = emi::pass_work_kslice(e);
+        } else if (o[0] == emi::PASS_WORK_NODE) {
+            o[1] = emi::pass_work_bx(e, 0);
+            o[2] = emi::pass_work_b(e, 0);
+            o[3] = hs == 2 && emi::pass_work_has_chunk(e, 1) ? emi::pass_work_bx(e, 1) : -1;
+            o[4] = hs == 2 && emi::pass_work_has_chunk(e, 1) ? emi::pass_work_b(e, 1) : -1;
+        }
+    }
+    return EMI_OK;
+}
+
+int emi_debug_pass_work_uploads(emi_ctx_t c, unsigned long long* uploads, int* tables) {
+    if (!c || !uploads) return EMI_ERR_ARG;
+    *uploads = c->pass_work.uploads;
+    int n = 0;
+    for (const emi_api::PassWorkCache::Slot& sl : c->pass_work.slot) n += sl.used ? 1 : 0;
+    if (tables) *tables = n;
+    return EMI_OK;
+}
+
 int emi_debug_tile_order(int ns, int B, int M, int sym_ct, int sym_cpart, int* out_tile, int out_cap, int* ntiles_total, int* cpart,
                          int* cx) {
     return emi_debug_tile_order2(ns, B, M, sym_ct, sym_cpart, 0, 0, out_tile, out_cap, ntiles_total, cpart, cx);
diff --git a/etol_amd/csrc/emi_args.hpp b/etol_amd/csrc/emi_args.hpp
--- a/etol_amd/csrc/emi_args.hpp
+++ b/etol_amd/csrc/emi_args.hpp
@@ -31,6 +31,7 @@
 #define FUSED_BK 16
 
 #include "emi_models.hpp"
+#include "emi_pass_work.hpp"
 
 namespace emi {
 
@@ -130,63 +131,13 @@
     float* RES;
     int R, M, ns, nres;
 };
-struct RingTile { int ntile, grp; };
-#if defined(__HIPCC__)
-__host__ __device__
-#endif
-inline RingTile ring_tile_of(int tl, int ntiles, int ngrp, int cpart, int cx, int nsg = 1) {
-    RingTile t;
-    if (cpart > 0) {
-        const int per_xcd = ngrp * ntiles / 8;
-        const int x = tl / per_xcd, m = tl - x * per_xcd;
-        const int pc = x % cpart, pg = x / cpart;
-        const int ncol = ntiles / cpart, ng = ngrp / (8 / cpart);
-        const int cb = m / (ng * cx), r = m - cb * ng * cx;
-        t.grp = pg * ng + r / cx;
-        t.ntile = pc * ncol + cb * cx + r % cx;
-    } else if (cpart < 0) {
-        const int G = -cpart, per_xcd = ngrp * ntiles / 8;
-        const int x = tl / per_xcd, m = tl - x * per_xcd;
-        const int per_sb = G * nsg * ntiles, sb = m / per_sb, r = m - sb * per_sb;
-        const int per_cb = G * nsg * cx, cb = r / per_cb, r2 = r - cb * per_cb;
-        const int g = r2 / (nsg * cx), r3 = r2 - g * (nsg * cx);
-        const int mt = x * (ngrp / nsg / 8) + sb * G + g;
-        t.grp = mt * nsg + r3 / cx;
-        t.ntile = cb * cx + r3 % cx;
-    } else {
-        t.ntile = tl % ntiles;
-        t.grp = tl / ntiles;
-    }
-    return t;
-}
-struct PassRole { int mfma, index; };
-#if defined(__HIPCC__)
-__host__ __device__
-#endif
-inline PassRole pass_role_of(int j, int nm, int nn, int order) {
-    const long long t = (long long)nm + nn;
-    long long m0, m1;
-    const long long d = order >= 100 ? order : 100;
-    if (order == 1 || d * nm > 100 * t) {
-        m0 = j < nm ? j : nm;
-        m1 = j < nm ? j + 1 : nm;
-    } else {
-        m0 = ((long long)j * nm * d) / (100 * t);
-        m1 = ((long long)(j + 1) * nm * d) / (100 * t);
-        if (m0 > nm) m0 = nm;
-        if (m1 > nm) m1 = nm;
-    }
-    PassRole r;
-    r.mfma = m1 > m0;
-    r.index = (int)(r.mfma ? m0 : j - m0);
-    return r;
-}
 struct PassArgs {
     SymDefectArgs s;
     NodeArgs<double> n;
     int nm8, nn8;
     int nm, nn;
     int nbx;
+    const PassWork* work;
 };
 
 }
diff --git a/etol_amd/csrc/emi_ctx.hpp b/etol_amd/csrc/emi_ctx.hpp
--- a/etol_amd/csrc/emi_ctx.hpp
+++ b/etol_amd/csrc/emi_ctx.hpp
@@ -22,6 +22,20 @@
     hipEvent_t ev[PROF_MARKS] = {};
     bool has_node = false, has_defect = false, fused = false;
     int level = 0;
+};
+
+struct PassWorkCache {
+    static constexpr int SLOTS = 8;
+    struct Slot {
+        bool used = false;
+        emi::PassWorkKey key;
+        std::vector<emi::PassWork> host;
+        emi::DeviceArray<emi::PassWork> dev;
+        unsigned long long stamp = 0;
+    };
+    Slot slot[SLOTS];
+    unsigned long long clock = 0;
+    unsigned long long uploads = 0;
 };
 
 }
@@ -103,6 +117,7 @@
     int sym_gblk = 0, sym_cx = 0;
     int pass_order = -1;
     int sym_combine = 1;
+    emi_api::PassWorkCache pass_work;
     emi::KeepRecord keep;
     DevBuf s_X, s_U, s_RES, s_VALS, s_COST, s_LF, s_LC, s_H;
     std::vector<DevBuf> host_stage;
diff --git a/etol_amd/csrc/emi_kernels.hpp b/etol_amd/csrc/emi_kernels.hpp
--- a/etol_amd/csrc/emi_kernels.hpp
+++ b/etol_amd/csrc/emi_kernels.hpp
@@ -48,7 +48,8 @@
 }
 
 bool pass_model_supported(int model);
-hipError_t launch_pass(int model, const SymDefectArgs& sa, const NodeArgs<double>& na, hipStream_t s, const SymPlan& plan);
+hipError_t launch_pass(int model, const SymDefectArgs& sa, const NodeArgs<double>& na, hipStream_t s, const SymPlan& plan, const PassWorkKey& key,
+                       const PassWork* work);
 
 struct AdjointArgs {
     const double* VALS;
@@ -160,7 +161,7 @@
 template <typename T> hipError_t rtc_launch_hess(RtcModel* m, const HessArgs<T>& a, hipStream_t s);
 hipError_t rtc_launch_symdefect(RtcModel* m, const SymDefectArgs& a, hipStream_t s);
 int rtc_pass_sw_large(const RtcModel* m);
-hipError_t rtc_launch_pass(RtcModel* m, const SymDefectArgs& sa, const NodeArgs<double>& na, int sw, hipStream_t s);
+hipError_t rtc_launch_pass(RtcModel* m, const SymDefectArgs& sa, const NodeArgs<double>& na, int sw, hipStream_t s, const PassWorkKey& key, const PassWork* work);
 hipError_t rtc_launch_nodes_nt(RtcModel* m, const NodeArgs<double>& a, hipStream_t s);
 
 struct KktWorkspace;
diff --git a/etol_amd/csrc/emi_pass_plan.hpp b/etol_amd/csrc/emi_pass_plan.hpp
--- a/etol_amd/csrc/emi_pass_plan.hpp
+++ b/etol_amd/csrc/emi_pass_plan.hpp
@@ -5,6 +5,7 @@
 #include <climits>
 
 #include "emi355x.h"
+#include "emi_pass_work.hpp"
 
 namespace emi {
 
@@ -293,6 +294,10 @@
     return p;
 }
 
+inline PassWorkKey pass_work_for(const SymPlan& sym, int ns, int B, int M, int order) {
+    return pass_work_key(ns, B, M, sym.sw, sym.ct, sym.ks, sym.hs, sym.cpart, sym.cx, order);
+}
+
 inline PassPlan plan_pass(const PassPolicyIn& in, int B, bool jac) {
     PassPlan p;
     p.tiles16 = pass_tiles16(in, B);
diff --git a/etol_amd/csrc/emi_pass_work.hpp b/etol_amd/csrc/emi_pass_work.hpp
--- /dev/null
+++ b/etol_amd/csrc/emi_pass_work.hpp
@@ -0,0 +1,154 @@
+#pragma once
+
+#if defined(__HIPCC__)
+#define EMI_WORK_HD __host__ __device__
+#else
+#define EMI_WORK_HD
+#endif
+
+namespace emi {
+
+struct RingTile { int ntile, grp; };
+EMI_WORK_HD inline RingTile ring_tile_of(int tl, int ntiles, int ngrp, int cpart, int cx, int nsg = 1) {
+    RingTile t;
+    if (cpart > 0) {
+        const int per_xcd = ngrp * ntiles / 8;
+        const int x = tl / per_xcd, m = tl - x * per_xcd;
+        const int pc = x % cpart, pg = x / cpart;
+        const int ncol = ntiles / cpart, ng = ngrp / (8 / cpart);
+        const int cb = m / (ng * cx), r = m - cb * ng * cx;
+        t.grp = pg * ng + r / cx;
+        t.ntile = pc * ncol + cb * cx + r % cx;
+    } else if (cpart < 0) {
+        const int G = -cpart, per_xcd = ngrp * ntiles / 8;
+        const int x = tl / per_xcd, m = tl - x * per_xcd;
+        const int per_sb = G * nsg * ntiles, sb = m / per_sb, r = m - sb * per_sb;
+        const int per_cb = G * nsg * cx, cb = r / per_cb, r2 = r - cb * per_cb;
+        const int g = r2 / (nsg * cx), r3 = r2 - g * (nsg * cx);
+        const int mt = x * (ngrp / nsg / 8) + sb * G + g;
+        t.grp = mt * nsg + r3 / cx;
+        t.ntile = cb * cx + r3 % cx;
+    } else {
+        t.ntile = tl % ntiles;
+        t.grp = tl / ntiles;
+    }
+    return t;
+}
+struct PassRole { int mfma, index; };
+EMI_WORK_HD inline PassRole pass_role_of(int j, int nm, int nn, int order) {
+    const long long t = (long long)nm + nn;
+    long long m0, m1;
+    const long long d = order >= 100 ? order : 100;
+    if (order == 1 || d * nm > 100 * t) {
+        m0 = j < nm ? j : nm;
+        m1 = j < nm ? j + 1 : nm;
+    } else {
+        m0 = ((long long)j * nm * d) / (100 * t);
+        m1 = ((long long)(j + 1) * nm * d) / (100 * t);
+        if (m0 > nm) m0 = nm;
+        if (m1 > nm) m1 = nm;
+    }
+    PassRole r;
+    r.mfma = m1 > m0;
+    r.index = (int)(r.mfma ? m0 : j - m0);
+    return r;
+}
+
+struct PassWork { unsigned w0, w1; };
+enum PassWorkRole { PASS_WORK_IDLE = 0, PASS_WORK_MFMA = 1, PASS_WORK_NODE = 2 };
+constexpr unsigned PASS_WORK_MAX_KSLICE = 1u << 8, PASS_WORK_MAX_NTILE = 1u << 22, PASS_WORK_MAX_BX = 1u << 14;
+
+EMI_WORK_HD inline long long pass_work_index(int g, int per_xcd) { return (long long)(g & 7) * per_xcd + (g >> 3); }
+EMI_WORK_HD inline int pass_work_role(PassWork e) { return (int)(e.w0 & 3u); }
+EMI_WORK_HD inline int pass_work_kslice(PassWork e) { return (int)((e.w0 >> 2) & 255u); }
+EMI_WORK_HD inline int pass_work_ntile(PassWork e) { return (int)(e.w0 >> 10); }
+EMI_WORK_HD inline int pass_work_grp(PassWork e) { return (int)e.w1; }
+EMI_WORK_HD inline bool pass_work_has_chunk(PassWork e, int half) { return half == 0 || (e.w0 & 4u) != 0; }
+EMI_WORK_HD inline int pass_work_bx(PassWork e, int half) { return (int)((e.w0 >> (half ? 18 : 4)) & 0x3FFFu); }
+EMI_WORK_HD inline int pass_work_b(PassWork e, int half) { return (int)e.w1 + (half ? (int)((e.w0 >> 3) & 1u) : 0); }
+
+}
+
+#ifndef __HIPCC_RTC__
+#include <vector>
+
+namespace emi {
+
+struct PassWorkKey {
+    int nm = 0, nn = 0;
+    int nm8 = 0, nn8 = 0;
+    int order = 0;
+    int ntiles = 0, ngrp = 0;
+    int nsg = 1;
+    int cpart = 0, cx = 0;
+    int ks = 1, hs = 1;
+    int nbx = 1;
+    bool operator==(const PassWorkKey& o) const {
+        return nm == o.nm && nn == o.nn && nm8 == o.nm8 && nn8 == o.nn8 && order == o.order && ntiles == o.ntiles && ngrp == o.ngrp && nsg == o.nsg &&
+               cpart == o.cpart && cx == o.cx && ks == o.ks && hs == o.hs && nbx == o.nbx;
+    }
+    int per_xcd() const { return nm8 + nn8; }
+    long long blocks() const { return 8LL * per_xcd(); }
+};
+
+inline PassWorkKey pass_work_key(int ns, int B, int M, int sw, int ct, int ks, int hs, int cpart, int cx, int order) {
+    PassWorkKey k;
+    const int mtiles = (B + 15) / 16;
+    k.ks = ks > 1 ? ks : 1;
+    k.hs = hs == 2 ? 2 : 1;
+    k.nsg = ns / sw;
+    k.ntiles = (M / 2) / (64 * ct);
+    k.ngrp = mtiles * k.nsg;
+    k.nm = k.ngrp * k.ntiles * k.ks;
+    k.nbx = (M + 511) / 512;
+    k.nn = k.nbx * B;
+    k.nm8 = (k.nm + 7) / 8;
+    k.nn8 = ((k.nn + k.hs - 1) / k.hs + 7) / 8;
+    k.order = order;
+    k.cpart = cpart;
+    k.cx = cx;
+    return k;
+}
+
+inline bool pass_work_build(const PassWorkKey& k, std::vector<PassWork>& out, const char** why = nullptr) {
+    const char* dummy;
+    const char*& w = why ? *why : dummy;
+    w = "";
+    if (k.nm < 0 || k.nn < 1 || k.nm8 < 0 || k.nn8 < 1 || k.ntiles < 1 || k.ngrp < 1 || k.nsg < 1 || k.nbx < 1 || k.ks < 1 || k.hs < 1 || k.hs > 2) {
+        w = "counts";
+        return false;
+    }
+    if ((long long)k.nm8 * 8 < k.nm || (long long)k.nn8 * 8 * k.hs < k.nn) { w = "workgroups per XCD"; return false; }
+    if (k.blocks() > 0x7FFFFFFFLL) { w = "grid"; return false; }
+    if ((unsigned)k.ks > PASS_WORK_MAX_KSLICE) { w = "K slices"; return false; }
+    if ((unsigned)k.ntiles > PASS_WORK_MAX_NTILE) { w = "column tiles"; return false; }
+    if ((unsigned)k.nbx > PASS_WORK_MAX_BX) { w = "node chunks per instance"; return false; }
+    if ((long long)k.ngrp * k.ntiles * k.ks != k.nm) { w = "tiles"; return false; }
+    out.assign((size_t)k.blocks(), PassWork{0u, 0u});
+    const int per = k.per_xcd();
+    for (int xcd = 0; xcd < 8; ++xcd)
+        for (int j = 0; j < per; ++j) {
+            PassWork& e = out[(size_t)xcd * per + j];
+            const PassRole role = pass_role_of(j, k.nm8, k.nn8, k.order);
+            if (role.index < 0 || role.index >= (role.mfma ? k.nm8 : k.nn8)) { w = "role index"; return false; }
+            if (role.mfma) {
+                const long long bid = (long long)xcd * k.nm8 + role.index;
+                if (bid >= k.nm) continue;
+                const RingTile rt = ring_tile_of((int)(bid / k.ks), k.ntiles, k.ngrp, k.cpart, k.cx, k.nsg);
+                if (rt.ntile < 0 || rt.ntile >= k.ntiles || rt.grp < 0 || rt.grp >= k.ngrp) { w = "tile"; return false; }
+                e.w0 = (unsigned)PASS_WORK_MFMA | (unsigned)(bid % k.ks) << 2 | (unsigned)rt.ntile << 10;
+                e.w1 = (unsigned)rt.grp;
+            } else {
+                const long long n0 = ((long long)xcd * k.nn8 + role.index) * k.hs;
+                if (n0 >= k.nn) continue;
+                e.w0 = (unsigned)PASS_WORK_NODE | (unsigned)(n0 % k.nbx) << 4;
+                e.w1 = (unsigned)(n0 / k.nbx);
+                if (k.hs == 2 && n0 + 1 < k.nn)
+                    e.w0 |= 4u | ((n0 + 1) / k.nbx != n0 / k.nbx ? 8u : 0u) | (unsigned)((n0 + 1) % k.nbx) << 18;
+            }
+        }
+    return true;
+}
+
+}
+#endif
diff --git a/etol_amd/csrc/emi_rtc.hip b/etol_amd/csrc/emi_rtc.hip
--- a/etol_amd/csrc/emi_rtc.hip
+++ b/etol_amd/csrc/emi_rtc.hip
@@ -267,7 +267,7 @@
 
 int rtc_pass_sw_large(const RtcModel* m) { return m ? pass_class_sw(SWC_LARGE, m->ns) : 0; }
 
-hipError_t rtc_launch_pass(RtcModel* m, const SymDefectArgs& sa, const NodeArgs<double>& na, int sw, hipStream_t s) {
+hipError_t rtc_launch_pass(RtcModel* m, const SymDefectArgs& sa, const NodeArgs<double>& na, int sw, hipStream_t s, const PassWorkKey& key, const PassWork* work) {
     PassShape shape;
     shape.ns = m->ns;
     shape.M = sa.M;
@@ -286,6 +286,10 @@
     a.nn = nn;
     a.nm8 = (nm + 7) / 8;
     a.nn8 = (nn + 7) / 8;
+    if (!work || key.nm != nm || key.nn != nn || key.nm8 != a.nm8 || key.nn8 != a.nn8 || key.nbx != a.nbx || key.hs != 1 || key.nsg != m->ns / sw ||
+        key.ntiles != ntiles || key.ks != (sa.ksplit > 1 ? sa.ksplit : 1) || key.order != sa.mfma_first || key.cpart != sa.cpart || key.cx != sa.cx)
+        return hipErrorInvalidValue;
+    a.work = work;
     const size_t lds = (size_t)f->nst * ((2 * sw * FUSED_TI + 2 * 64 + 63) / 64 * 64) * f->bk * sizeof(double);
     return launch(m->pass[f - PASS_FORMS_RTC], dim3(8 * (a.nm8 + a.nn8)), dim3(256), lds, s, &a, sizeof a);
 }
diff --git a/etol_amd/csrc/emi_symdefect.hip b/etol_amd/csrc/emi_symdefect.hip
--- a/etol_amd/csrc/emi_symdefect.hip
+++ b/etol_amd/csrc/emi_symdefect.hip
@@ -70,7 +70,7 @@
 }
 
 template <class Model, int SW, int NST, int BK = 8, int CT = 1, int HS = 1, bool DOP = false>
-static hipError_t launch_pass_model(const SymDefectArgs& sa, const NodeArgs<double>& na, hipStream_t s, int res) {
+static hipError_t launch_pass_model(const SymDefectArgs& sa, const NodeArgs<double>& na, hipStream_t s, int res, const PassWorkKey& key, const PassWork* work) {
     constexpr int NS = Model::NS;
     PassArgs a;
     a.s = sa;
@@ -83,6 +83,10 @@
     a.nn = nn;
     a.nm8 = (nm + 7) / 8;
     a.nn8 = ((nn + HS - 1) / HS + 7) / 8;
+    if (!work || key.nm != nm || key.nn != nn || key.nm8 != a.nm8 || key.nn8 != a.nn8 || key.nbx != a.nbx || key.hs != HS || key.nsg != NS / SW ||
+        key.ntiles != ntiles || key.ks != (sa.ksplit > 1 ? sa.ksplit : 1) || key.order != sa.mfma_first || key.cpart != sa.cpart || key.cx != sa.cx)
+        return hipErrorInvalidValue;
+    a.work = work;
     const size_t lds = DOP ? (size_t)NST * (2 * SW * FUSED_TI) * BK * sizeof(double)
                            : (size_t)HS * NST * ((2 * SW * FUSED_TI + 2 * 64 * CT + 63) / 64 * 64) * BK * sizeof(double);
     if (DOP && (!sa.Dfrag || sa.ksplit > 1)) return hipErrorInvalidValue;
@@ -120,12 +124,13 @@
 }
 
 template <class Model>
-static hipError_t launch_pass_planned(const SymDefectArgs& sa, const NodeArgs<double>& na, hipStream_t s, const SymPlan& p) {
+static hipError_t launch_pass_planned(const SymDefectArgs& sa, const NodeArgs<double>& na, hipStream_t s, const SymPlan& p, const PassWorkKey& key,
+                                      const PassWork* work) {
     constexpr int NS = Model::NS;
 #define EMI_PASS_FORM_LAUNCH(CLS, NST, BK, CT, HS, DOP, SLICES, STORES)                                                                   \
     if constexpr (pass_class_applies(CLS, NS)) {                                                                                          \
         if (p.sw == pass_class_sw(CLS, NS) && p.nst == NST && p.bk == BK && p.ct == CT && p.hs == HS && p.dop == DOP && (SLICES || p.ks == 1)) \
-            return launch_pass_model<Model, pass_class_sw(CLS, NS), NST, BK, CT, HS, DOP>(sa, na, s, p.res);                             \
+            return launch_pass_model<Model, pass_class_sw(CLS, NS), NST, BK, CT, HS, DOP>(sa, na, s, p.res, key, work);                  \
     }
     EMI_PASS_FORMS(EMI_PASS_FORM_LAUNCH)
 #undef EMI_PASS_FORM_LAUNCH
@@ -134,9 +139,10 @@
 
 bool pass_model_supported(int model) { return model == EMI_MODEL_POINTMASS2D || model == EMI_MODEL_QUADROTOR2D; }
 
-hipError_t launch_pass(int model, const SymDefectArgs& sa, const NodeArgs<double>& na, hipStream_t s, const SymPlan& p) {
-    if (model == EMI_MODEL_POINTMASS2D) return launch_pass_planned<PointMass2D<double>>(sa, na, s, p);
-    if (model == EMI_MODEL_QUADROTOR2D) return launch_pass_planned<Quadrotor2D<double>>(sa, na, s, p);
+hipError_t launch_pass(int model, const SymDefectArgs& sa, const NodeArgs<double>& na, hipStream_t s, const SymPlan& p, const PassWorkKey& key,
+                       const PassWork* work) {
+    if (model == EMI_MODEL_POINTMASS2D) return launch_pass_planned<PointMass2D<double>>(sa, na, s, p, key, work);
+    if (model == EMI_MODEL_QUADROTOR2D) return launch_pass_planned<Quadrotor2D<double>>(sa, na, s, p, key, work);
     return hipErrorInvalidValue;
 }
 
diff --git a/etol_amd/csrc/emi_symdefect_kernels.hpp b/etol_amd/csrc/emi_symdefect_kernels.hpp
--- a/etol_amd/csrc/emi_symdefect_kernels.hpp
+++ b/etol_amd/csrc/emi_symdefect_kernels.hpp
@@ -436,8 +436,17 @@
     ring_epilogue_pre<Model, SW, false>(a, acc_a, acc_b, inst0, i0, s0, wid, r16, kq, none);
 }
 
+struct RingWork { int ntile, grp, kslice; };
+template <class Model, int SW>
+EMI_DEV RingWork emi_ring2_tile_of(const SymDefectArgs& a, const int bid) {
+    constexpr int NSG = Model::NS / SW;
+    const int KS = a.ksplit > 1 ? a.ksplit : 1;
+    const RingTile rt = ring_tile_of(bid / KS, (a.M >> 1) / 64, (a.B + FUSED_TI - 1) / FUSED_TI * NSG, a.cpart, a.cx, NSG);
+    return RingWork{rt.ntile, rt.grp, bid % KS};
+}
+
 template <class Model, int SW, int NST = 3, int BK = 8, int CT = 1, int HS = 1, bool DOP = false>
-EMI_DEV void emi_ring2_body(const SymDefectArgs& a, const int bid ) {
+EMI_DEV void emi_ring2_body(const SymDefectArgs& a, const int ntile, const int grp, const int kslice ) {
     constexpr int NS = Model::NS;
     constexpr int TI = FUSED_TI, TM = SW * TI, TN = 64 * CT, CH = BK / 2, NSG = NS / SW;
     static_assert(CT == 1 || CT == 2, "one or two column sub-tiles per wave");
@@ -460,9 +469,6 @@
     const int M = a.M, Hh = M >> 1, B = a.B;
     const int ntiles = Hh / TN;
     const int KS = (HS == 1 && !DOP && a.ksplit > 1) ? a.ksplit : 1;
-    const int kslice = bid % KS;
-    const RingTile rt = ring_tile_of(bid / KS, ntiles, (B + TI - 1) / TI * NSG, a.cpart, a.cx, NSG);
-    const int ntile = rt.ntile, grp = rt.grp;
     const int tile = grp * ntiles + ntile;
     const int sg = grp % NSG, mtile = grp / NSG;
     const int inst0 = mtile * TI, i0 = ntile * TN, s0 = sg * SW;
@@ -775,7 +781,8 @@
         const int nwg = gridDim.x, xcd = bid & 7, q = nwg >> 3, rr = nwg & 7;
         bid = (xcd < rr ? xcd * (q + 1) : rr * (q + 1) + (xcd - rr) * q) + (bid >> 3);
     }
-    emi_ring2_body<Model, SW>(a, bid);
+    const RingWork w = emi_ring2_tile_of<Model, SW>(a, bid);
+    emi_ring2_body<Model, SW>(a, w.ntile, w.grp, w.kslice);
 }
 
 template <class Model, int SW>
@@ -824,19 +831,24 @@
 #ifdef EMI_ENTRY_PAD_NOPS
     asm volatile(".rept " EMI_STR(EMI_ENTRY_PAD_NOPS) "\n\ts_nop 0\n\t.endr" ::: "memory");
 #endif
-    const int g = blockIdx.x, xcd = g & 7, j = g >> 3;
-    const PassRole role = pass_role_of(j, a.nm8, a.nn8, a.s.mfma_first);
-    if (a.s.ablate & (role.mfma ? 16 : 32)) return;
-    if (role.mfma) {
-        const int tid = xcd * a.nm8 + role.index;
-        if (tid >= a.nm) return;
+    const int g = blockIdx.x;
+    const PassWork wk = a.work[pass_work_index(g, a.nm8 + a.nn8)];
+    {
+        const double *sx = a.s.X, *nx = a.n.X, *nu = a.n.U;
+        const int sm = a.s.M, sb = a.s.B, sab = a.s.ablate, nm = a.n.M;
+        asm volatile("" ::"s"(sx), "s"(nx), "s"(nu), "s"(sm), "s"(sb), "s"(sab), "s"(nm));
+    }
+    const int role = pass_work_role(wk);
+    if (role == PASS_WORK_IDLE) return;
+    if (a.s.ablate & (role == PASS_WORK_MFMA ? 16 : 32)) return;
+    if (role == PASS_WORK_MFMA) {
         __builtin_amdgcn_s_setprio(3);
-        emi_ring2_body<Model, SW, NST, BK, CT, HS, DOP>(a.s, tid);
+        emi_ring2_body<Model, SW, NST, BK, CT, HS, DOP>(a.s, pass_work_ntile(wk), pass_work_grp(wk), pass_work_kslice(wk));
     } else {
-        const int nid = (xcd * a.nn8 + role.index) * HS + (HS > 1 ? (int)(threadIdx.x >> 8) : 0);
-        if (nid >= a.nn) return;
-        emi_nodes_body<double, Model, VEC, true, false, ST, false, KEEP>(a.n, nid % a.nbx, nid / a.nbx, a.nbx);
-    }
-}
-
-}
+        const int half = HS > 1 ? (int)(threadIdx.x >> 8) : 0;
+        if (!pass_work_has_chunk(wk, half)) return;
+        emi_nodes_body<double, Model, VEC, true, false, ST, false, KEEP>(a.n, pass_work_bx(wk, half), pass_work_b(wk, half), a.nbx);
+    }
+}
+
+}
diff --git a/etol_amd/evaluator.py b/etol_amd/evaluator.py
--- a/etol_amd/evaluator.py
+++ b/etol_amd/evaluator.py
@@ -892,6 +892,12 @@
         return res.value
 
     @property
+    def pass_work_uploads(self):
+        n, held = C.c_ulonglong(0), C.c_int(0)
+        self._ck(self.lib.emi_debug_pass_work_uploads(self.ctx, C.byref(n), C.byref(held)), "emi_debug_pass_work_uploads")
+        return n.value, held.value
+
+    @property
     def last_defect_kernel(self):
         return self.lib.emi_last_defect_kernel(self.ctx).decode()
 
@@ -900,3 +906,20 @@
         f = C.c_int()
         self._ck(self.lib.emi_last_path(self.ctx, C.byref(f)), "emi_last_path")
         return bool(f.value)
+
+
+
+PASS_WORK_INFO = ("blocks", "nm", "nn", "nm8", "nn8", "nbx", "ntiles", "ngrp", "cpart", "cx", "ks", "nsg")
+
+
+def debug_pass_work(ns, B, M, sw, ctc=1, ksplit=1, hs=1, sym_cpart=0, sym_gblk=0, sym_cx=0, order=0):
+    lib = L.load()
+    info = (C.c_int * 12)()
+    args = [int(v) for v in (ns, B, M, sw, ctc, ksplit, hs, sym_cpart, sym_gblk, sym_cx, order)]
+    if lib.emi_debug_pass_work(*args, None, 0, info) != 0:
+        return None
+    table = np.zeros((info[0], 5), dtype=np.intc)
+    st = lib.emi_debug_pass_work(*args, table.ctypes.data_as(C.POINTER(C.c_int)), table.size, info)
+    if st != 0:
+        raise L.EmiError(f"emi_debug_pass_work: status {st}")
+    return table, dict(zip(PASS_WORK_INFO, info))
diff --git a/include/emi355x.h b/include/emi355x.h
--- a/include/emi355x.h
+++ b/include/emi355x.h
@@ -342,6 +342,9 @@
                           int* ntiles_total, int* cpart, int* cx);
 int emi_debug_operator_fragments(int M, const double* D, double* out);
 int emi_debug_pass_roles(int nm, int nn, int order, int* out_role, int out_cap);
+int emi_debug_pass_work(int ns, int B, int M, int sw, int ctc, int ksplit, int hs, int sym_cpart, int sym_gblk, int sym_cx, int order,
+                        int* out, int out_cap, int* info);
+int emi_debug_pass_work_uploads(emi_ctx_t ctx, unsigned long long* uploads, int* tables);
 const char* emi_last_defect_kernel(emi_ctx_t ctx);
 
 #define EMI_COMM_ID_BYTES 128
```

After: 5.966 billion (median of 6 runs). 1.3% higher.
